# wing02/MyLdpcCppApi

Measured on AMD Instinct MI355X. Metric: decoded Mbit/s (info bits), DVB-S2 N=64800 rate-1/2, 50 iters, higher is better.
Workload: dtype f32; 1 GPU; DVB-S2-profile (64800,32400) rate-1/2 (seeded IRA table with the standard's structure, E=226799), batch 4096 frames per GPU, 50 iterations, sum-product fp32 (probability domain), all-zero codeword + AWGN sigma=0.95 (no frame converges), early termination on, inputs resident in HBM; global_batch=4096, frames_per_gpu=4096, algo=sp, frames_per_launch=4096, parallelism=frames sharded over 1 GPU(s), all-gather of decoded bytes, frames_converged=0

## Files before the change

### include/ldpc_hip.h

```cpp
#ifndef LDPC_HIP_H_
#define LDPC_HIP_H_

#include <stddef.h>
#include <stdint.h>

#ifdef __cplusplus
extern "C" {
#endif

#define LDPC_HIP_ABI_VERSION 3

enum ldpc_status {
    LDPC_OK = 0,
    LDPC_ERR_ARG = 1,
    LDPC_ERR_HIP = 2,
    LDPC_ERR_NOMEM = 3,
    LDPC_ERR_UNSUPPORTED = 4,
    LDPC_ERR_STATE = 5
};

enum ldpc_algo {
    LDPC_ALGO_SP = 0,
    LDPC_ALGO_MS = 1,
    LDPC_ALGO_LAYERED = 2,
    LDPC_ALGO_MS_FUSED = 3,
    LDPC_ALGO_LAYERED_HOST = 4
};

enum ldpc_msg_dtype { LDPC_MSG_F32 = 0, LDPC_MSG_F16 = 1 };

enum ldpc_host_input { LDPC_HOST_INPUT_AUTO = 0, LDPC_HOST_INPUT_STAGED = 1, LDPC_HOST_INPUT_LOCK_PAGES = 2 };

enum ldpc_pack_mode {
    LDPC_PACK_BYTES = 0,
    LDPC_PACK_BITS = 1
};

typedef struct ldpc_graph ldpc_graph;
typedef struct ldpc_decoder ldpc_decoder;

typedef struct ldpc_decoder_config {
    uint32_t struct_size;
    int32_t K;
    int32_t max_batch;
    int32_t algo;
    int32_t msg_dtype;
    int32_t max_iter;
    float llr_scale;
    int32_t early_term;
    int32_t device;
    int32_t layer_rows;
    int32_t pack_mode;
    int32_t frames_per_lane;
    int32_t poll_interval;
    int32_t tune_flags;
    int32_t tune_rows_per_wave;
    int32_t tune_cols_per_wave;
    int32_t tune_link_rows;
    int32_t tune_compact;
    int32_t tune_ldsp_grid;
    int32_t tune_ldsp_shape;
    int32_t tune_place;
    int32_t host_input;
    int32_t host_copy_threads;
    int32_t tune_q_order;
    float ms_scale;
    float ms_offset;
} ldpc_decoder_config;

enum ldpc_tune_field {
    LDPC_TUNE_FUSED = 0,
    LDPC_TUNE_LDSP = 2,
    LDPC_TUNE_LDSP_EXT = 4,
    LDPC_TUNE_LDSP_PACK = 6,
    LDPC_TUNE_LINK_NARROW = 8,
    LDPC_TUNE_CHECK_WIDE = 10,
    LDPC_TUNE_SYN_XCD = 12,
    LDPC_TUNE_FUSED_PACK = 14,
    LDPC_TUNE_FUSED_LOOP = 16,
    LDPC_TUNE_DEVICE_TAIL = 18,
    LDPC_TUNE_MERGE = 20,
    LDPC_TUNE_LINK_DEEP = 22,
    LDPC_TUNE_LINK_HALF = 24,
    LDPC_TUNE_LINK_GUIDED = 26,
    LDPC_TUNE_TILES_FIRST = 28
};
#define LDPC_TUNE_ON(field) (1 << (field))
#define LDPC_TUNE_OFF(field) (2 << (field))

typedef struct ldpc_decode_stats {
    int32_t iterations_launched;
    int32_t batch_time;
    int64_t frames;
    int64_t frames_converged;
    float ms_total;
    float ms_check;
    float ms_var;
    float ms_other;
    int32_t launches_check;
    int32_t launches_var;
    int64_t frame_rounds;
} ldpc_decode_stats;

int ldpc_abi_version(void);
const char *ldpc_last_error(void);
int ldpc_device_count(int *count);

int ldpc_graph_create(const int32_t *rows, const int32_t *cols, int64_t E, int32_t M, int32_t N,
                      ldpc_graph **out);
int ldpc_graph_destroy(ldpc_graph *g);
int ldpc_graph_info(const ldpc_graph *g, int32_t *M, int32_t *N, int64_t *E, int32_t *max_row_deg,
                    int32_t *max_col_deg);

void ldpc_decoder_config_init(ldpc_decoder_config *cfg);
int ldpc_decoder_create(const ldpc_graph *g, const ldpc_decoder_config *cfg, ldpc_decoder **out);
int ldpc_decoder_create_multi(const ldpc_graph *g, const ldpc_decoder_config *cfg, const int32_t *devices,
                              int32_t n_devices, ldpc_decoder **out);
int ldpc_decoder_destroy(ldpc_decoder *d);
int ldpc_shard_range(int64_t frames, int32_t part, int32_t parts, int32_t unit, int64_t *lo, int64_t *hi);

int ldpc_decode(ldpc_decoder *d, const float *llr_host, int64_t frames, uint8_t *out_host,
                int64_t out_bytes, int32_t *iters);

int ldpc_decode_device(ldpc_decoder *d, const float *llr_dev, int64_t frames, uint8_t *out_dev,
                       int64_t out_bytes, int32_t *iters_dev, void *stream);

int64_t ldpc_out_bytes(int32_t K, int64_t frames, int32_t pack_mode);

int ldpc_decoder_set_timing(ldpc_decoder *d, int enable);
int ldpc_decoder_stats(ldpc_decoder *d, ldpc_decode_stats *stats);

typedef struct ldpc_kernel_time {
    int32_t phase;
    int32_t degree;
    int32_t launches;
    float ms_total;
    int64_t bytes_total;
    char name[64];
    int64_t bytes_moved;
} ldpc_kernel_time;
int ldpc_decoder_kernel_times(ldpc_decoder *d, ldpc_kernel_time *out, int32_t capacity,
                              int32_t *count);

int ldpc_decoder_link_form(ldpc_decoder *d, int32_t *form, int32_t *calibrated, float ms[3]);

int ldpc_decoder_placement(ldpc_decoder *d, int32_t *candidates, int32_t *kept, float ms[16]);
int ldpc_decoder_array_addresses(ldpc_decoder *d, uint64_t out[4]);

int ldpc_decoder_set_tap(ldpc_decoder *d, int32_t iter);
int ldpc_decoder_dump(ldpc_decoder *d, int32_t which, float *host_out, int64_t count);

int ldpc_awgn_device(float *llr_dev, int64_t frames, int32_t N, const uint8_t *bits_dev, float sd,
                     uint64_t seed, int64_t first_frame, int32_t device, void *stream);
int ldpc_count_errors_device(const uint8_t *out_dev, const uint8_t *ref_dev, int64_t frames,
                             int64_t bytes_per_frame, int64_t errors[3], int32_t device, void *stream);

typedef struct ldpc_encoder ldpc_encoder;
enum ldpc_code_format {
    LDPC_CODE_PACKED = 0,
    LDPC_CODE_BITS = 1
};
enum ldpc_parity_kind { LDPC_PARITY_DUAL_DIAGONAL = 1, LDPC_PARITY_STAIRCASE = 2 };
int ldpc_parity_structure(const ldpc_graph *g, int32_t K, int32_t block_rows, int32_t out[8]);
int ldpc_encoder_create(const ldpc_graph *g, int32_t K, int32_t block_rows, int32_t max_frames, int32_t device,
                        ldpc_encoder **out);
int ldpc_encoder_destroy(ldpc_encoder *e);
int ldpc_encode_device(ldpc_encoder *e, const uint8_t *src_dev, int64_t src_bytes, int64_t frames, uint8_t *code_dev,
                       int64_t code_bytes, int32_t format, void *stream);
int ldpc_encode(ldpc_encoder *e, const uint8_t *src_host, int64_t src_bytes, uint8_t *code_host, int64_t code_bytes);
int64_t ldpc_code_bytes(int32_t N, int64_t frames, int32_t format);

typedef struct ldpc_rate_spec {
    uint32_t struct_size;
    int32_t  N;
    int32_t  punctured;
    int32_t  filler_lo, filler_hi;
    float    fill_llr;
    float    erasure_llr;
} ldpc_rate_spec;
void ldpc_rate_spec_init(ldpc_rate_spec *spec, int32_t N);
int ldpc_rate_lengths(const ldpc_rate_spec *spec, int32_t *Ncb, int32_t *L);
int ldpc_rate_index(const ldpc_rate_spec *spec, int32_t k0, int32_t E, int32_t *index_out);
int ldpc_rate_match_device(const ldpc_rate_spec *spec, const uint8_t *code_dev, int32_t code_format, int64_t frames, int32_t k0,
                           int32_t E, uint8_t *tx_dev, int64_t tx_bytes, int32_t tx_format, int32_t device, void *stream);
int ldpc_rate_recover_device(const ldpc_rate_spec *spec, const float *rx_dev, int64_t frames, int32_t k0, int32_t E, float *soft_dev,
                             int32_t accumulate, float *y_dev, int32_t device, void *stream);
int ldpc_rate_match(const ldpc_rate_spec *spec, const uint8_t *code_host, int32_t code_format, int64_t frames, int32_t k0, int32_t E,
                    uint8_t *tx_host, int64_t tx_bytes, int32_t tx_format, int32_t device);
int ldpc_rate_recover(const ldpc_rate_spec *spec, const float *rx_host, int64_t frames, int32_t k0, int32_t E, float *soft_host,
                      int32_t accumulate, float *y_host, int32_t device);

typedef struct ldpc_modem_spec {
    uint32_t struct_size;
    int32_t  Qm;
    int32_t  interleave;
} ldpc_modem_spec;
void ldpc_modem_spec_init(ldpc_modem_spec *spec, int32_t Qm);
int64_t ldpc_modem_symbol_floats(const ldpc_modem_spec *spec, int32_t E);
int ldpc_modem_index(const ldpc_modem_spec *spec, int32_t E, int32_t *index_out);
int ldpc_modem_points(int32_t Qm, float *iq);
int ldpc_modem_transmit_device(const ldpc_modem_spec *spec, const uint8_t *tx_dev, int32_t tx_format, int64_t frames, int32_t E,
                               float sd, uint64_t seed, int64_t first_frame, float *sym_dev, int64_t sym_floats, int32_t device,
                               void *stream);
int ldpc_modem_demap_device(const ldpc_modem_spec *spec, const float *sym_dev, int64_t frames, int32_t E, float *rx_dev,
                            int32_t device, void *stream);
int ldpc_modem_transmit(const ldpc_modem_spec *spec, const uint8_t *tx_host, int32_t tx_format, int64_t frames, int32_t E, float sd,
                        uint64_t seed, int64_t first_frame, float *sym_host, int64_t sym_floats, int32_t device);
int ldpc_modem_demap(const ldpc_modem_spec *spec, const float *sym_host, int64_t frames, int32_t E, float *rx_host, int32_t device);

int ldpc_hbm_probe_device(int32_t device, int64_t bytes, int32_t reps, double *copy_gbs, double *by_policy);
int ldpc_hbm_sustained_device(int32_t device, int64_t bytes, int32_t milliseconds, double *copy_gbs);

int ldpc_host_block_plan(uint64_t base, int64_t frames, int32_t N, int32_t max_batch, int64_t group, uint64_t out[6]);
int ldpc_host_locked_ranges(int64_t *live, int64_t *stale);

#ifdef __cplusplus
}
#endif
#endif
```

### myldpccppapi_amd/capi.py

```python
import ctypes

import numpy as np

from . import _lib
from ._lib import DecoderConfig, DecodeStats, LdpcError

ALGO_SP, ALGO_MS, ALGO_LAYERED, ALGO_MS_FUSED, ALGO_LAYERED_HOST = 0, 1, 2, 3, 4
MSG_F32, MSG_F16 = 0, 1
PACK_BYTES, PACK_BITS = 0, 1
CODE_PACKED, CODE_BITS = 0, 1
CODE_FORMATS = {"packed": CODE_PACKED, "bits": CODE_BITS}
PARITY_KINDS = {1: "dual_diagonal", 2: "staircase"}
HOST_INPUT = {"auto": 0, "staged": 1, "lock_pages": 2}
ALGOS = {"sp": ALGO_SP, "ms": ALGO_MS, "layered": ALGO_LAYERED, "ms_fused": ALGO_MS_FUSED,
         "layered_host": ALGO_LAYERED_HOST}

TUNE_FIELDS = {"fused": 0, "ldsp": 2, "ldsp_ext": 4, "ldsp_pack": 6, "link_narrow": 8, "check_wide": 10,
               "syn_xcd": 12, "fused_pack": 14, "fused_loop": 16, "device_tail": 18, "merge": 20, "link_deep": 22, "link_half": 24,
               "link_guided": 26, "tiles_first": 28}
TUNE_INTS = ("rows_per_wave", "cols_per_wave", "link_rows", "compact", "ldsp_grid", "ldsp_per_cu", "ldsp_waves", "place", "q_order")


def apply_tune(cfg, tune):
    flags, shape = 0, 0
    for k, v in (tune or {}).items():
        if k in TUNE_FIELDS:
            if v is not None:
                flags |= (1 if v else 2) << TUNE_FIELDS[k]
        elif k == "ldsp_per_cu":
            shape |= int(v) & 255
        elif k == "ldsp_waves":
            shape |= (int(v) & 255) << 8
        elif k in TUNE_INTS:
            setattr(cfg, "tune_" + k, int(v))
        else:
            raise KeyError("unknown tuning field %r" % k)
    cfg.tune_flags, cfg.tune_ldsp_shape = flags, shape


def hbm_probe(device=0, nbytes=1 << 30, reps=5, by_policy=False):
    g = ctypes.c_double(0.0)
    two = (ctypes.c_double * 2)(0.0, 0.0)
    _lib.check(_lib.load().ldpc_hbm_probe_device(int(device), int(nbytes), int(reps), ctypes.byref(g), two))
    return (g.value, two[0], two[1]) if by_policy else g.value


def hbm_sustained(device=0, nbytes=1 << 30, milliseconds=300):
    g = ctypes.c_double(0.0)
    _lib.check(_lib.load().ldpc_hbm_sustained_device(int(device), int(nbytes), int(milliseconds), ctypes.byref(g)))
    return g.value


def tune_from_env(env=None):
    import os
    env = os.environ if env is None else env
    t = {}
    for name, key in (("FUSED", "fused"), ("LDSP", "ldsp"), ("LDSP_EXT", "ldsp_ext"), ("LDSP_PACK", "ldsp_pack"),
                      ("LINK_NARROW", "link_narrow"), ("CHECK_WIDE", "check_wide"), ("SYN_XCD", "syn_xcd"),
                      ("FUSED_LOOP", "fused_loop"), ("DEVICE_TAIL", "device_tail"), ("MERGE", "merge"), ("LINK_DEEP", "link_deep"), ("LINK_HALF", "link_half"),
                      ("LINK_GUIDED", "link_guided"), ("TILES_FIRST", "tiles_first")):
        if "LDPC_TUNE_" + name in env:
            t[key] = int(env["LDPC_TUNE_" + name]) != 0
    if "LDPC_TUNE_NO_PACK" in env:
        t["fused_pack"] = False
    for name, key in (("RPW", "rows_per_wave"), ("CPW", "cols_per_wave"), ("LDSP_GRID", "ldsp_grid"),
                      ("LDSP_PER_CU", "ldsp_per_cu"), ("LDSP_WAVES", "ldsp_waves")):
        if "LDPC_TUNE_" + name in env:
            t[key] = int(env["LDPC_TUNE_" + name])
    for name, key in (("LINK_RPW", "link_rows"), ("COMPACT", "compact")):
        if "LDPC_TUNE_" + name in env:
            v = int(env["LDPC_TUNE_" + name])
            t[key] = v if v > 0 else -1
    return t


def shard_range(frames, part, parts, unit=1):
    lo, hi = ctypes.c_int64(), ctypes.c_int64()
    _lib.check(_lib.load().ldpc_shard_range(int(frames), int(part), int(parts), int(unit),
                                            ctypes.byref(lo), ctypes.byref(hi)))
    return lo.value, hi.value


def host_block_plan(base, frames, N, max_batch, group):
    out = (ctypes.c_uint64 * 6)()
    _lib.check(_lib.load().ldpc_host_block_plan(int(base), int(frames), int(N), int(max_batch), int(group), out))
    return tuple(int(x) for x in out)


def host_locked_ranges():
    a, b = ctypes.c_int64(-1), ctypes.c_int64(-1)
    _lib.check(_lib.load().ldpc_host_locked_ranges(ctypes.byref(a), ctypes.byref(b)))
    return a.value, b.value


def device_count():
    n = ctypes.c_int(0)
    rc = _lib.load().ldpc_device_count(ctypes.byref(n))
    return n.value if rc == 0 else 0


def out_bytes(K, frames, pack_mode=PACK_BYTES):
    return int(_lib.load().ldpc_out_bytes(K, frames, pack_mode))


def code_bytes(N, frames, fmt="packed"):
    return int(_lib.load().ldpc_code_bytes(int(N), int(frames), CODE_FORMATS.get(fmt, fmt)))


def parity_structure(graph, K, block_rows=0):
    out = (ctypes.c_int32 * 8)()
    _lib.check(_lib.load().ldpc_parity_structure(graph._h, int(K), int(block_rows), out))
    return dict(kind=PARITY_KINDS[out[0]], c=out[1], x=out[2], a=out[3], b=out[4], ext_rows=out[5], z=out[6])


class Graph:

    def __init__(self, rows, cols, M, N):
        L = _lib.load()
        self.rows = np.ascontiguousarray(rows, np.int32)
        self.cols = np.ascontiguousarray(cols, np.int32)
        if self.rows.shape != self.cols.shape or self.rows.ndim != 1:
            raise ValueError("rows and cols must be 1-D arrays of equal length")
        self.M, self.N, self.E = int(M), int(N), int(self.rows.size)
        self._h = ctypes.c_void_p()
        i32p = ctypes.POINTER(ctypes.c_int32)
        _lib.check(L.ldpc_graph_create(self.rows.ctypes.data_as(i32p), self.cols.ctypes.data_as(i32p),
                                       self.E, self.M, self.N, ctypes.byref(self._h)))

    def info(self):
        L = _lib.load()
        M, N, rd, cd = (ctypes.c_int32() for _ in range(4))
        E = ctypes.c_int64()
        _lib.check(L.ldpc_graph_info(self._h, ctypes.byref(M), ctypes.byref(N), ctypes.byref(E),
                                     ctypes.byref(rd), ctypes.byref(cd)))
        return dict(M=M.value, N=N.value, E=E.value, max_row_deg=rd.value, max_col_deg=cd.value)

    def close(self):
        h, self._h = getattr(self, "_h", None), None
        if h and _lib is not None and _lib._lib is not None:
            _lib._lib.ldpc_graph_destroy(h)

    def __del__(self):
        try:
            self.close()
        except Exception:
            pass


class Decoder:

    def __init__(self, graph, K, max_batch, algo="sp", max_iter=40, llr_scale=8.0, early_term=True,
                 device=0, layer_rows=0, pack_mode=PACK_BYTES, frames_per_lane=0, poll_interval=0,
                 msg_dtype=MSG_F32, tune=None, devices=None, host_input="auto", host_copy_threads=0,
                 ms_scale=0.0, ms_offset=0.0):
        L = _lib.load()
        cfg = DecoderConfig()
        L.ldpc_decoder_config_init(ctypes.byref(cfg))
        cfg.K, cfg.max_batch = int(K), int(max_batch)
        cfg.algo = ALGOS[algo] if isinstance(algo, str) else int(algo)
        cfg.msg_dtype = {"f32": MSG_F32, "f16": MSG_F16}.get(msg_dtype, msg_dtype)
        cfg.max_iter, cfg.llr_scale = int(max_iter), float(llr_scale)
        cfg.early_term, cfg.device, cfg.layer_rows = int(bool(early_term)), int(device), int(layer_rows)
        cfg.pack_mode, cfg.frames_per_lane, cfg.poll_interval = int(pack_mode), int(frames_per_lane), int(poll_interval)
        apply_tune(cfg, tune)
        cfg.host_input = HOST_INPUT[host_input] if isinstance(host_input, str) else int(host_input)
        cfg.host_copy_threads = int(host_copy_threads)
        cfg.ms_scale, cfg.ms_offset = float(ms_scale), float(ms_offset)
        self.cfg = cfg
        self.graph = graph
        self.K, self.N, self.E = int(K), graph.N, graph.E
        self._h = ctypes.c_void_p()
        if devices is None:
            _lib.check(L.ldpc_decoder_create(graph._h, ctypes.byref(cfg), ctypes.byref(self._h)))
        else:
            devs = (ctypes.c_int32 * len(devices))(*[int(x) for x in devices])
            _lib.check(L.ldpc_decoder_create_multi(graph._h, ctypes.byref(cfg), devs, len(devices),
                                                   ctypes.byref(self._h)))

    def decode(self, llr, want_iters=True):
        L = _lib.load()
        llr = np.ascontiguousarray(llr, np.float32).reshape(-1, self.N)
        frames = llr.shape[0]
        out = np.zeros(out_bytes(self.K, frames, self.cfg.pack_mode), np.uint8)
        iters = np.zeros(frames, np.int32)
        _lib.check(L.ldpc_decode(self._h, llr.ctypes.data, frames, out.ctypes.data, out.size,
                                 iters.ctypes.data if want_iters else None))
        return out, iters

    def decode_device(self, llr_ptr, frames, out_ptr, out_nbytes, iters_ptr=None, stream=None):
        _lib.check(_lib.load().ldpc_decode_device(self._h, llr_ptr, frames, out_ptr, out_nbytes,
                                                  iters_ptr, stream))

    def set_timing(self, enable=True):
        _lib.check(_lib.load().ldpc_decoder_set_timing(self._h, int(enable)))

    def stats(self):
        st = DecodeStats()
        _lib.check(_lib.load().ldpc_decoder_stats(self._h, ctypes.byref(st)))
        return {f: getattr(st, f) for f, _ in st._fields_}

    def kernel_times(self):
        arr = (_lib.KernelTime * 64)()
        n = ctypes.c_int32(0)
        _lib.check(_lib.load().ldpc_decoder_kernel_times(self._h, arr, 64, ctypes.byref(n)))
        return [dict(name=arr[i].name.decode(), phase=arr[i].phase, degree=arr[i].degree,
                     launches=arr[i].launches, ms_total=arr[i].ms_total, bytes_total=arr[i].bytes_total,
                     bytes_moved=arr[i].bytes_moved)
                for i in range(n.value)]

    def link_form(self):
        form, cal = ctypes.c_int32(-1), ctypes.c_int32(0)
        ms = (ctypes.c_float * 3)()
        _lib.check(_lib.load().ldpc_decoder_link_form(self._h, ctypes.byref(form), ctypes.byref(cal), ms))
# ... 182 lines not shown
```

### myldpccppapi_amd/csrc/decoder.hpp

```cpp
#pragma once

#include <hip/hip_runtime.h>
#include <stdint.h>

#include <memory>
#include <type_traits>
#include <vector>

#include "../../include/ldpc_hip.h"
#include "flood_tables.hpp"
#include "layered_kernels.hpp"
#include "fused_kernels.hpp"
#include "ldsp_kernels.hpp"
#include "engines.hpp"
#include "tune.hpp"
#include "host_stage.hpp"
#include "hip_host.hpp"

#ifndef LDPC_IDLE_FAT
#define LDPC_IDLE_FAT 8
#endif

namespace ldpc {

template <typename Fn> inline int dispatch_v(int V, Fn &&fn)
{
    return V == 1 ? fn(std::integral_constant<int, 1>{})
                  : V == 2 ? fn(std::integral_constant<int, 2>{}) : fn(std::integral_constant<int, 4>{});
}

struct RowClass {
    int degree = 0;
    int count = 0;
    DevBuf<int32_t> e0;
    std::vector<int32_t> h_e0;
    DevBuf<int32_t> link_col, link_pos;
    int linked = 0;
    int n_big = 0, small_rows = 1;
};
struct ColClass {
    int degree = 0;
    int count = 0;
    DevBuf<int32_t> col, edge;
    int64_t q_base = -1;
};

struct ClassGroup {
    int bucket = 0, lo = 0, hi = 0;
    int blocks = 0;
    int blocks_fat = 0;
    std::vector<int> members;
    DevBuf<GroupClass> table, table_fat;
};

constexpr int kIdleFat = LDPC_IDLE_FAT;

struct FloodPlan {
    DevBuf<uint8_t> chan, Q, R;
    int msg_size = 4;
    DevBuf<int32_t> qpos, col_qedge;
    std::vector<int32_t> h_qpos;
    std::vector<RowClass> row_classes;
    std::vector<ColClass> col_classes;
    std::vector<ClassGroup> check_groups, var_groups;
    std::vector<int> check_solo, var_solo;
    DevBuf<int32_t> extra_e0, extra_deg;
    int n_extra = 0;
    int64_t extra_edges = 0;
    FloodFns fns;

    int link_form = 1;
    bool link_deep = false;
    bool syn_xcd = true;
    bool check_wide = false;
    int link_rpw = 16;
    int cus = 256;
    bool link_calibrated = false;
    float link_cal_ms[3] = {0, 0, 0};
    int place_candidates = 0, place_kept = 0;
    float place_ms[16] = {};

    bool tail_enabled = false;
    int TO = 0, TA = 0;
    DevBuf<int32_t> tail_state, tail_map, running;

    std::unique_ptr<ldpc_decoder> child;
    DevBuf<int32_t> cmap;
    DevBuf<int32_t> cinv;
    DevBuf<unsigned long long> cmoved;
    int child_capacity = kCompactCapacity;
    int compact_threshold = kCompactCapacity;
    bool is_child = false;
    ldpc_decoder *handed_to = nullptr;
    HostBuf<int32_t> h_active;

    HostBuf<int32_t> h_summary;
    Event ev_summary;
    bool summary_pending = false;
    int idle_after = 0;

    bool first_round_from_chan = false;
};

struct HostSlot {
    DevBuf<float> llr;
    DevBuf<uint8_t> out;
    DevBuf<int32_t> iters;
    HostBuf<uint8_t> h_out;
    HostBuf<int32_t> h_iters;
    HostBuf<uint8_t> h_head;
    Event h2d_done, all_done;
    bool busy = false;
    int64_t off = 0, n = 0, dst = 0, copy_bytes = 0;
    HostBuf<int32_t> h_sum;
    int g_iterations = 0, g_tiles = 0, g_children = 0, g_child_f[3] = {0, 0, 0};
};
struct RingChunk { HostBuf<uint8_t> h; Event ev; bool used = false; };
struct CallCounts { bool valid = false; int32_t iterations = 0, batch_time = 0; int64_t frames = 0, converged = 0, frame_rounds = 0; };

struct HostPath {
    Stream copy_stream;
    HostSlot slot[3];
    CallCounts call;
    bool suppress_poll = false;
    std::vector<RingChunk> ring;
    size_t ring_next = 0;
    std::unique_ptr<Worker> stager;
    std::vector<std::unique_ptr<Worker>> copy_helpers;
    std::vector<Job> copy_jobs;
    Job stage_job[3];
    bool stage_pending[3] = {false, false, false};
    std::vector<void *> locked_blocks, stuck_blocks;
};

struct TimedSpan {
    Event a, b;
    int kind = 0;
    int degree = 0;
    int64_t bytes = 0;
    int64_t moved = 0;
    int lo = 0;
};

struct Timing {
    bool timing = false;
    int timing_every = 0;
    int64_t timing_calls = 0;
    std::vector<TimedSpan> spans;
    size_t spans_used = 0;
    Event ev_begin, ev_end;
    hipStream_t last_stream = nullptr;
    bool have_last = false;
    int32_t tap_iter = 0;
};

}

struct ldpc_decoder {
    ldpc::Stream stream;
    ldpc_decoder_config cfg{};
    int32_t M = 0, N = 0;
    int64_t E = 0;
    int V = 1, F = 64, T = 0;
    std::vector<int32_t> h_cols;
    ldpc::Tune tune;

    ldpc::DevBuf<int32_t> row_ptr, edge_col, col_ptr, col_edge;
    ldpc::DevBuf<uint64_t> hard, failw, done;
    ldpc::DevBuf<int32_t> iters, active;
    ldpc::DevBuf<int32_t> summary;

    ldpc::LayeredPlan layered;
    ldpc::FusedPlan fused;
    bool use_fused = false;
    ldpc::LdspPlan ldsp;
    bool use_ldsp = false;
    bool ms_corr = false;
    float ms_scale = 1.0f, ms_offset = 0.0f;

    int32_t last_iterations = 0;
    int64_t last_frames = 0;
    int32_t last_tiles = 0;

    ldpc::FloodPlan flood;
    ldpc::HostPath host;
    ldpc::Timing tm;

    std::vector<ldpc_decoder *> shards;
    std::vector<std::unique_ptr<ldpc::Worker>> shard_workers;

    void wait_for_own_work()
    {
        if (!stream.s) return;
        if (flood.child) flood.child->wait_for_own_work();
        (void)hipSetDevice(cfg.device);
        if (tm.have_last && tm.ev_end.e) (void)hipEventSynchronize(tm.ev_end.e);
        (void)hipStreamSynchronize(stream.s);
        if (host.copy_stream.s) (void)hipStreamSynchronize(host.copy_stream.s);
    }

    ~ldpc_decoder()
    {
        for (auto &w : shard_workers) w->stop();
        if (host.stager) host.stager->stop();
        for (auto &w : host.copy_helpers) w->stop();
        for (ldpc_decoder *sh : shards) (void)ldpc_decoder_destroy(sh);
        wait_for_own_work();
    }
};

namespace ldpc {

inline hipError_t span_begin(ldpc_decoder *d, hipStream_t s, int kind, int degree = 0, int64_t bytes = 0, int64_t moved = -1,
                             int lo = 0)
{
    Timing &t = d->tm;
    if (!t.timing) return hipSuccess;
    if (t.spans_used == t.spans.size()) {
        TimedSpan sp;
        hipError_t e = sp.a.create();
        if (e == hipSuccess) e = sp.b.create();
        if (e != hipSuccess) return e;
        t.spans.push_back(std::move(sp));
    }
    TimedSpan &sp = t.spans[t.spans_used];
    sp.kind = kind;
    sp.degree = degree;
    sp.bytes = bytes;
    sp.moved = moved < 0 ? bytes : moved;
    sp.lo = lo;
    return hipEventRecord(sp.a.e, s);
}

inline hipError_t span_end(ldpc_decoder *d, hipStream_t s)
{
    if (!d->tm.timing) return hipSuccess;
    return hipEventRecord(d->tm.spans[d->tm.spans_used++].b.e, s);
}

}
```

### myldpccppapi_amd/csrc/engine_flood.hip

```cpp
#include <hip/hip_runtime.h>

#include <algorithm>
#include <map>
#include <vector>

#include "flood_kernels.hpp"
#include "decoder.hpp"
#include "graph.hpp"

using ldpc::set_error;

namespace {

using ldpc::DevBuf;
using ldpc::RowClass;
using ldpc::ColClass;
using ldpc::ClassGroup;
using ldpc::kIdleFat;
using ldpc::dispatch_v;
using ldpc::span_begin;
using ldpc::span_end;
using ldpc::kVarBuckets;
using ldpc::kCheckBuckets;
using ldpc::kVarBucketLo;
using ldpc::kVarBucketHi;
using ldpc::kCheckBucketLo;
using ldpc::kCheckBucketHi;

template <int V>
__global__ void summary_kernel(const int32_t *iters, const uint64_t *done, const uint64_t *fail,
                               int64_t frames, int32_t freeze, int32_t *summary)
{
    constexpr int F = 64 * V;
    const int64_t f = (int64_t)blockIdx.x * blockDim.x + threadIdx.x;
    if (f >= frames) return;
    const int64_t tile = f / F;
    const int fi = (int)(f % F);
    const int l = fi / V, v = fi % V;
    atomicMax(&summary[0], iters[f]);
    const uint64_t ok = freeze ? done[tile * V + v] : ~fail[tile * V + v];
    if ((ok >> l) & 1ull) atomicAdd(&summary[1], 1);
}

static inline dim3 flood_grid(const ldpc_decoder *d, unsigned blocks, unsigned tiles, int32_t *tiles_first, bool linked = false)
{
    const bool want = d->tune.tiles_first == 1 || (d->tune.tiles_first == 0 && linked);
    *tiles_first = (blocks <= 65535u && want) ? 1 : 0;
    return *tiles_first ? dim3(tiles, blocks) : dim3(blocks, tiles);
}

template <int V> int run_flooding(ldpc_decoder *d, const float *llr_dev, int64_t frames,
                                  uint8_t *out_dev, int64_t out_bytes, int32_t *iters_dev,
                                  hipStream_t s, int start_round = 1);

template <int V> int enqueue_check_phase(ldpc_decoder *d, hipStream_t s, int tiles, int64_t frames, int it, int max_iter,
                                         bool fat, const ldpc::TailRef &tr)
{
    using namespace ldpc;
    const int64_t msz = d->flood.msg_size;
    for (auto &rc : d->flood.row_classes) {
        if (!rc.linked) continue;
        LDPC_HIP_TRY(span_begin(d, s, 4, rc.degree,
                           (2 * msz * rc.degree * rc.count + msz * 5 * rc.linked + 2 * msz * d->flood.extra_edges) * frames,
                           msz * ((int64_t)rc.degree * rc.count + rc.linked +
                                  ((int64_t)rc.degree * rc.count - 2 * rc.linked) +
                                  (it < max_iter ? 2 * rc.linked : 0) + 2 * d->flood.extra_edges) * frames));
        CheckArgs a{d->flood.Q.p, d->flood.R.p, rc.e0.p, d->done.p, d->E, rc.count, 1, rc.degree, d->ms_scale, tr};
        a.ms_offset = d->ms_offset;
        a.qpos = d->flood.qpos.p;
        LinkArgs lk{rc.link_col.p, rc.link_pos.p, d->flood.chan.p, d->flood.Q.p, d->hard.p, d->N,
                    (it < max_iter) ? 1 : 0, d->tm.tap_iter ? 1 : 0, d->flood.extra_e0.p, d->flood.extra_deg.p, d->flood.n_extra, 0,
                    rc.n_big, rc.small_rows};
        a.rows_per_wave = d->flood.link_rpw;
        const int variant = (d->flood.link_form == 2 && !d->flood.fns.link_half[rc.degree]) ? 1 : d->flood.link_form;
        const int waves = link_chunk_count(d->flood.link_rpw, rc.n_big, rc.small_rows, rc.count) * (variant == 1 ? V : variant == 2 ? V / 2 : 1);
        lk.link_blocks = (waves + kWavesPerBlock - 1) / kWavesPerBlock;
        const dim3 grid = flood_grid(d, lk.link_blocks + (d->flood.n_extra + kWavesPerBlock - 1) / kWavesPerBlock, tiles, &a.tiles_first, true);
        (variant == 2 ? d->flood.fns.link_half : variant == 1 ? (d->flood.link_deep ? d->flood.fns.link_deep : d->flood.fns.link_narrow) : d->flood.fns.link)
            [rc.degree]<<<grid, kBlock, 0, s>>>(a, lk);
        LDPC_HIP_TRY(span_end(d, s));
    }
    for (auto &g : d->flood.check_groups) {
        int64_t edges = 0;
        for (int i : g.members) edges += (int64_t)d->flood.row_classes[i].degree * d->flood.row_classes[i].count;
        LDPC_HIP_TRY(span_begin(d, s, 5, g.hi, 2 * msz * edges * frames, -1, g.lo));
        CheckArgs a{d->flood.Q.p, d->flood.R.p, nullptr, d->done.p, d->E, 0, (d->tune.rows_per_wave ? d->tune.rows_per_wave : 2) * (fat ? kIdleFat : 1), 0, d->ms_scale, tr};
        a.ms_offset = d->ms_offset;
        a.qpos = d->flood.qpos.p;
        if (it == 1 && d->flood.first_round_from_chan) { a.first_chan = d->flood.chan.p; a.edge_col = d->edge_col.p; a.N = d->N; }
        const dim3 grid = flood_grid(d, fat ? g.blocks_fat : g.blocks, tiles, &a.tiles_first);
        d->flood.fns.check_group[g.bucket]<<<grid, kBlock, 0, s>>>(a, fat ? g.table_fat.p : g.table.p, (int)g.members.size());
        LDPC_HIP_TRY(span_end(d, s));
    }
    for (int ci : d->flood.check_solo) {
        RowClass &rc = d->flood.row_classes[ci];
        LDPC_HIP_TRY(span_begin(d, s, 0, rc.degree, 2 * msz * rc.degree * rc.count * frames));
        CheckArgs a{d->flood.Q.p, d->flood.R.p, rc.e0.p, d->done.p, d->E, rc.count, 1, rc.degree, d->ms_scale, tr};
        a.ms_offset = d->ms_offset;
        a.qpos = d->flood.qpos.p;
        if (it == 1 && d->flood.first_round_from_chan) { a.first_chan = d->flood.chan.p; a.edge_col = d->edge_col.p; a.N = d->N; }
        const int slotk = rc.degree <= d->flood.fns.max_check_unrolled ? rc.degree : 0;
        const bool narrow = slotk && (!d->flood.check_wide || rc.degree > kMaxUnrolledDegree);
        const int rpw = (d->tune.rows_per_wave ? d->tune.rows_per_wave : (narrow ? 2 : 1)) * (fat ? kIdleFat : 1);
        a.rows_per_wave = rpw;
        const int waves = ((rc.count + rpw - 1) / rpw) * (narrow ? V : 1);
        const dim3 grid = flood_grid(d, (waves + kWavesPerBlock - 1) / kWavesPerBlock, tiles, &a.tiles_first);
        (narrow ? d->flood.fns.check : d->flood.fns.check_wide)[slotk]<<<grid, kBlock, 0, s>>>(a);
        LDPC_HIP_TRY(span_end(d, s));
    }
    return LDPC_OK;
}

template <int V> int enqueue_var_phase(ldpc_decoder *d, hipStream_t s, int tiles, int64_t frames, int it, int max_iter,
                                       bool fat, const ldpc::TailRef &tr)
{
    using namespace ldpc;
    const int64_t msz = d->flood.msg_size;
    const int wq = (it < max_iter) ? 1 : 0;
    for (auto &g : d->flood.var_groups) {
        int64_t units = 0;
        for (int i : g.members) units += (int64_t)((wq ? 2 : 1) * d->flood.col_classes[i].degree + 1) * d->flood.col_classes[i].count;
        LDPC_HIP_TRY(span_begin(d, s, 6, g.hi, msz * units * frames, -1, g.lo));
        VarArgs a{d->flood.R.p, d->flood.Q.p, d->flood.chan.p, d->hard.p, d->done.p, nullptr, nullptr,
                  d->E, d->N, 0, (d->tune.cols_per_wave ? d->tune.cols_per_wave : 1) * (fat ? kIdleFat : 1), wq, 0, tr};
        const dim3 grid = flood_grid(d, fat ? g.blocks_fat : g.blocks, tiles, &a.tiles_first);
        d->flood.fns.var_group[g.bucket]<<<grid, kBlock, 0, s>>>(a, fat ? g.table_fat.p : g.table.p, (int)g.members.size());
        LDPC_HIP_TRY(span_end(d, s));
    }
    for (int ci : d->flood.var_solo) {
        ColClass &cc = d->flood.col_classes[ci];
        LDPC_HIP_TRY(span_begin(d, s, 1, cc.degree, msz * ((wq ? 2 : 1) * cc.degree + 1) * cc.count * frames));
        VarArgs a{d->flood.R.p, d->flood.Q.p, d->flood.chan.p, d->hard.p, d->done.p, cc.col.p, cc.edge.p,
                  d->E, d->N, cc.count, 1, wq, cc.degree, tr};
        const int cpw = (d->tune.cols_per_wave ? d->tune.cols_per_wave : 1) * (fat ? kIdleFat : 1);
        a.cols_per_wave = cpw;
        a.q_base = cc.q_base;
        const int slotk = cc.degree <= kMaxUnrolledDegree ? cc.degree : 0;
        const int waves = (cc.count + cpw - 1) / cpw;
        const dim3 grid = flood_grid(d, (waves + kWavesPerBlock - 1) / kWavesPerBlock, tiles, &a.tiles_first);
        d->flood.fns.var[slotk]<<<grid, kBlock, 0, s>>>(a);
        LDPC_HIP_TRY(span_end(d, s));
    }
    return LDPC_OK;
}

template <int V> int compact_and_finish(ldpc_decoder *d, int64_t frames, int count, int it, hipStream_t s)
{
    using namespace ldpc;
    ldpc_decoder *c = d->flood.child.get();
    while (c->flood.child && count <= c->flood.child->cfg.max_batch) c = c->flood.child.get();
    const int cv = c->V, cf = 64 * cv;
    const unsigned ct = (unsigned)((count + cf - 1) / cf);
    const unsigned cg = ct * (unsigned)cv;
    if (cg > (unsigned)kBackWords) return set_error(LDPC_ERR_STATE, "hand-over of %d frames: more than %d mask words per column", count, kBackWords);
    LDPC_HIP_TRY(hipMemsetAsync(d->active.p, 0, sizeof(int32_t), s));
    compact_list_kernel<V><<<(unsigned)((frames + kBlock - 1) / kBlock), kBlock, 0, s>>>(d->done.p, frames, d->flood.cmap.p,
                                                                                         d->active.p, d->flood.child_capacity);
    const dim3 ge((unsigned)((d->E + kWavesPerBlock - 1) / kWavesPerBlock), cg);
    const dim3 gn((unsigned)((d->N + kWavesPerBlock - 1) / kWavesPerBlock), cg);
    const bool rowwise = count >= 128;
    const int ptiles = (int)((frames + 64 * V - 1) / (64 * V));
    if (d->flood.msg_size == 2) {
        if (rowwise) {
            compact_gather_rows_kernel<V, _Float16><<<(unsigned)((d->E + gather_rows_per_block<_Float16>() - 1) / gather_rows_per_block<_Float16>()), kBlock, 0, s>>>((const _Float16 *)d->flood.Q.p, (_Float16 *)c->flood.Q.p, d->flood.cmap.p, count, d->E, ptiles, cf, d->flood.qpos.p, c->flood.qpos.p);
            compact_gather_rows_kernel<V, _Float16><<<(unsigned)((d->N + gather_rows_per_block<_Float16>() - 1) / gather_rows_per_block<_Float16>()), kBlock, 0, s>>>((const _Float16 *)d->flood.chan.p, (_Float16 *)c->flood.chan.p, d->flood.cmap.p, count, d->N, ptiles, cf);
        } else {
            compact_gather_kernel<V, _Float16><<<ge, kBlock, 0, s>>>((const _Float16 *)d->flood.Q.p, (_Float16 *)c->flood.Q.p, d->flood.cmap.p, count, d->E, cf, d->flood.qpos.p, c->flood.qpos.p);
            compact_gather_kernel<V, _Float16><<<gn, kBlock, 0, s>>>((const _Float16 *)d->flood.chan.p, (_Float16 *)c->flood.chan.p, d->flood.cmap.p, count, d->N, cf);
        }
    } else {
        if (rowwise) {
            compact_gather_rows_kernel<V, float><<<(unsigned)((d->E + gather_rows_per_block<float>() - 1) / gather_rows_per_block<float>()), kBlock, 0, s>>>((const float *)d->flood.Q.p, (float *)c->flood.Q.p, d->flood.cmap.p, count, d->E, ptiles, cf, d->flood.qpos.p, c->flood.qpos.p);
            compact_gather_rows_kernel<V, float><<<(unsigned)((d->N + gather_rows_per_block<float>() - 1) / gather_rows_per_block<float>()), kBlock, 0, s>>>((const float *)d->flood.chan.p, (float *)c->flood.chan.p, d->flood.cmap.p, count, d->N, ptiles, cf);
        } else {
            compact_gather_kernel<V, float><<<ge, kBlock, 0, s>>>((const float *)d->flood.Q.p, (float *)c->flood.Q.p, d->flood.cmap.p, count, d->E, cf, d->flood.qpos.p, c->flood.qpos.p);
            compact_gather_kernel<V, float><<<gn, kBlock, 0, s>>>((const float *)d->flood.chan.p, (float *)c->flood.chan.p, d->flood.cmap.p, count, d->N, cf);
        }
    }
    LDPC_HIP_TRY(hipMemsetAsync(c->hard.p, 0, (size_t)ct * d->N * cv * sizeof(uint64_t), s));
    if (d->cfg.algo == LDPC_ALGO_SP) {
        if (ptiles * V <= kGatherParentWords && count <= 2 * kCompactCapacity)
            compact_hard_lds_kernel<V><<<(unsigned)((d->N + 63) / 64), kBlock, 0, s>>>(d->hard.p, c->hard.p, d->flood.cmap.p, count, d->N, cv, ptiles, (int)cg);
        else
            compact_hard_kernel<V><<<gn, kBlock, 0, s>>>(d->hard.p, c->hard.p, d->flood.cmap.p, count, d->N, cv);
    }
    compact_child_state_kernel<0><<<ct, 64, 0, s>>>(c->done.p, c->iters.p, count, d->cfg.max_iter, cv);
    LDPC_HIP_TRY(hipGetLastError());
    c->tm.timing = false;
    c->tm.tap_iter = 0;
    const int rc = dispatch_v(cv, [&](auto v) { return run_flooding<decltype(v)::value>(c, nullptr, count, nullptr, 0, nullptr, s, it + 1); });
    if (rc) return rc;
    d->flood.handed_to = c;
    LDPC_HIP_TRY(hipMemsetAsync(d->flood.cmoved.p, 0, d->flood.cmoved.n * sizeof(unsigned long long), s));
    compact_inverse_kernel<V><<<(unsigned)((count + 255) / 256), 256, 0, s>>>(d->flood.cmap.p, count, d->flood.cinv.p, d->flood.cmoved.p, cv);
    compact_hard_back_kernel<V><<<dim3((unsigned)((d->N + kBlock - 1) / kBlock), (unsigned)ptiles), kBlock, 0, s>>>(
        d->hard.p, c->hard.p, d->flood.cinv.p, d->flood.cmoved.p, d->N, cv, (int)cg);
    compact_finish_kernel<V><<<(unsigned)((count + 63) / 64), 64, 0, s>>>(d->done.p, d->iters.p, c->done.p, c->iters.p, d->flood.cmap.p, count, cv);
    LDPC_HIP_TRY(hipGetLastError());
    return LDPC_OK;
}

template <int V> int run_flooding(ldpc_decoder *d, const float *llr_dev, int64_t frames,
                                  uint8_t *out_dev, int64_t out_bytes, int32_t *iters_dev,
                                  hipStream_t s, int start_round)
{
    using namespace ldpc;
    const int F = 64 * V;
    const int tiles = (int)((frames + F - 1) / F);
    const int64_t msz = d->flood.msg_size;
    const int max_iter = d->cfg.max_iter;
    const int rounds = d->tm.tap_iter ? std::min(d->tm.tap_iter, max_iter) : max_iter;
    const bool freeze = d->cfg.early_term != 0;
    const size_t slot = (size_t)d->flood.TA * V;

    const bool resume = start_round > 1;
    LDPC_HIP_TRY(hipMemsetAsync(d->failw.p, 0, d->failw.n * sizeof(uint64_t), s));
    LDPC_HIP_TRY(hipMemsetAsync(d->summary.p, 0, 4 * sizeof(int32_t), s));
    d->flood.handed_to = nullptr;
    if (!resume && d->flood.summary_pending) {
        if (hipEventQuery(d->flood.ev_summary.e) == hipSuccess) {
            d->flood.summary_pending = false;
            d->flood.idle_after = (d->flood.h_summary.p[0] > 0 && d->flood.h_summary.p[0] < max_iter) ? d->flood.h_summary.p[0] + 1 : 0;
        } else {
            (void)hipGetLastError();
        }
    }
    const int idle_after = (freeze && !resume && !d->tm.tap_iter && d->cfg.poll_interval == 0) ? d->flood.idle_after : 0;
    const bool use_tail = d->flood.tail_enabled && freeze && !resume && !d->tm.tap_iter && tiles >= 4 * d->flood.TO;
    const TailRef tr{use_tail ? d->flood.tail_state.p : nullptr, d->T, d->flood.TO};
    TailArgs ta{};
    if (use_tail) {
        LDPC_HIP_TRY(hipMemsetAsync(d->flood.tail_state.p, 0, 4 * sizeof(int32_t), s));
        LDPC_HIP_TRY(hipMemsetAsync(d->flood.running.p, 0, d->flood.running.n * sizeof(int32_t), s));
        ta = TailArgs{d->flood.tail_state.p, d->flood.tail_map.p, d->flood.running.p, d->done.p, d->iters.p, d->flood.Q.p, d->flood.chan.p, d->hard.p,
                      d->E, frames, d->N, tiles, d->T, d->flood.TO * F, std::min(d->flood.compact_threshold, d->flood.TO * F), 0, max_iter};
    }

    bool q_less = d->cfg.algo == LDPC_ALGO_MS && !resume && !d->tm.tap_iter && max_iter > 1 && d->flood.n_extra == 0;
    for (auto &rc : d->flood.row_classes) if (rc.linked) q_less = false;
    for (int ci : d->flood.check_solo) if (d->flood.row_classes[ci].degree > d->flood.fns.max_check_unrolled) q_less = false;
    d->flood.first_round_from_chan = q_less;
    if (!resume) {
        LDPC_HIP_TRY(span_begin(d, s, 3));
        InitArgs a{llr_dev, d->flood.chan.p, q_less ? nullptr : d->flood.Q.p, d->hard.p, d->col_ptr.p, d->flood.col_qedge.p,
                   d->E, frames, d->N, d->cfg.llr_scale};
        dim3 grid((d->N + kInitCols - 1) / kInitCols, tiles);
        d->flood.fns.init<<<grid, kBlock, 0, s>>>(a);
        StateArgs st{d->done.p, nullptr, d->iters.p, nullptr, frames, 0, max_iter, freeze ? 1 : 0};
        state_kernel<V><<<use_tail ? d->flood.TA : tiles, 64, 0, s>>>(st);
        LDPC_HIP_TRY(span_end(d, s));
    }

    int launched = start_round - 1;
    bool poll_dense = false;
    for (int it = start_round; it <= rounds; ++it) {
        const bool fat = idle_after > 0 && it > idle_after;
        {
            const int rcp = enqueue_check_phase<V>(d, s, tiles, frames, it, max_iter, fat, tr);
            if (rcp) return rcp;
        }
        {
            const int rcv = enqueue_var_phase<V>(d, s, tiles, frames, it, max_iter, fat, tr);
            if (rcv) return rcv;
        }
        launched = it;
        if (freeze || it == rounds) {
            LDPC_HIP_TRY(span_begin(d, s, 3));
            uint64_t *fw = d->failw.p + (size_t)it * slot;
            const int rbk = (d->M + kBlock - 1) / kBlock;
            SyndromeArgs sa{d->row_ptr.p, d->edge_col.p, d->hard.p, fw, d->done.p, d->M, d->N,
                            d->flood.syn_xcd ? tiles : 0, rbk, tr};
            dim3 sgrid = d->flood.syn_xcd ? dim3(8 * rbk * ((tiles + 7) / 8)) : dim3(rbk, tiles);
            syndrome_kernel<V><<<sgrid, kBlock, 0, s>>>(sa);
            StateArgs st{d->done.p, fw, d->iters.p, nullptr, frames, it, max_iter, 1, tr, use_tail ? d->flood.running.p : nullptr,
                         d->summary.p + 2};
            const bool poll = freeze && it < rounds && d->cfg.poll_interval > 0 && !d->host.suppress_poll &&
                              ((it % d->cfg.poll_interval) == 0 || poll_dense);
            if (poll) {
                LDPC_HIP_TRY(hipMemsetAsync(d->active.p, 0, sizeof(int32_t), s));
                st.active = d->active.p;
            }
            state_kernel<V><<<tiles, 64, 0, s>>>(st);
            if (use_tail && it < rounds) {
                ta.iter = it;
                const unsigned tg = (unsigned)std::min<int64_t>(1024, d->E + 2 * (int64_t)d->N);
                if (d->flood.msg_size == 2) tail_gather_kernel<V, _Float16><<<tg, kBlock, 0, s>>>(ta);
                else tail_gather_kernel<V, float><<<tg, kBlock, 0, s>>>(ta);
            }
            LDPC_HIP_TRY(span_end(d, s));
            if (poll) {
                LDPC_HIP_TRY(hipMemcpyAsync(d->flood.h_active.p, d->active.p, sizeof(int32_t),
                                       hipMemcpyDeviceToHost, s));
                LDPC_HIP_TRY(hipStreamSynchronize(s));
                const int running = *d->flood.h_active.p;
                if (running == 0) break;
                if ((int64_t)running * 10 <= frames * 9 && d->flood.child && tiles > 1 &&
                    (double)d->E * (double)frames * 4.0 * (double)msz > 1.5e9) poll_dense = true;
                if (d->flood.child && running <= d->flood.compact_threshold && (int64_t)running * 4 <= frames && tiles > 1 && !d->tm.tap_iter) {
                    const int rc = compact_and_finish<V>(d, frames, running, it, s);
                    if (rc) return rc;
                    launched = d->flood.handed_to->last_iterations;
                    break;
                }
            }
        }
    }
    d->last_iterations = launched;
    d->last_tiles = tiles;
    if (resume) return LDPC_OK;

    LDPC_HIP_TRY(span_begin(d, s, 3));
    if (use_tail) tail_scatter_kernel<V><<<2048, kBlock, 0, s>>>(ta);
    {
        PackArgs pa{d->hard.p, out_dev, d->iters.p, iters_dev, frames, out_bytes, d->N, d->cfg.K,
                    d->cfg.pack_mode};
        const bool pack = (out_dev || iters_dev) && frames;
        if (d->cfg.pack_mode == LDPC_PACK_BYTES) {
            if (pack) pack_kernel<V><<<pack_grid<V>(d->cfg.K, tiles), kBlock, 0, s>>>(pa);
        } else {
            const int64_t n = std::max<int64_t>(out_bytes, frames);
            dim3 grid((unsigned)((n + kBlock - 1) / kBlock));
            if (pack) pack_kernel<V><<<grid, kBlock, 0, s>>>(pa);
        }
        summary_kernel<V><<<(unsigned)((frames + 255) / 256), 256, 0, s>>>(
            d->iters.p, d->done.p, d->failw.p, frames, 1, d->summary.p);
        if (!d->flood.is_child && d->cfg.poll_interval == 0 && freeze && !d->flood.summary_pending) {
            LDPC_HIP_TRY(hipMemcpyAsync(d->flood.h_summary.p, d->summary.p, 2 * sizeof(int32_t), hipMemcpyDeviceToHost, s));
            LDPC_HIP_TRY(hipEventRecord(d->flood.ev_summary.e, s));
            d->flood.summary_pending = true;
        }
    }
    LDPC_HIP_TRY(span_end(d, s));
    LDPC_HIP_TRY(hipGetLastError());
    return LDPC_OK;
}

int build_classes(ldpc_decoder *d, const ldpc_graph *g)
{
    std::map<int, std::vector<int32_t>> rows_by_deg, cols_by_deg, rowids_by_deg;
    for (int32_t m = 0; m < g->M; ++m) {
        const int deg = g->row_ptr[m + 1] - g->row_ptr[m];
        if (deg > 0) { rows_by_deg[deg].push_back(g->row_ptr[m]); rowids_by_deg[deg].push_back(m); }
    }
    std::vector<char> fused_col((size_t)g->N, 0);
    d->flood.row_classes.resize(rows_by_deg.size());
    size_t i = 0;
    for (auto &kv : rows_by_deg) {
        RowClass &rc = d->flood.row_classes[i++];
        rc.degree = kv.first;
        rc.count = (int)kv.second.size();
        rc.h_e0 = kv.second;
        LDPC_HIP_TRY(rc.e0.upload(kv.second));
        const std::vector<int32_t> &ids = rowids_by_deg[kv.first];
        const int rpw = d->flood.link_rpw;
        if (rpw >= 2 && rc.degree >= 2 && rc.degree <= ldpc::kMaxUnrolledDegree) {
            rc.n_big = (rc.count + rpw - 1) / rpw;
            rc.small_rows = rpw;
            const int small = std::max(2, rpw / 4);
            const bool forced = ldpc::tune_forced_on(d->tune.link_guided);
            if ((d->T >= 4 || forced) && small < rpw && !ldpc::tune_forced_off(d->tune.link_guided)) {
                const int64_t last_generation = (int64_t)d->flood.cus * 16 / d->T;
                int64_t big = (int64_t)rc.n_big - last_generation;
                if (big <= 0 && forced) big = rc.n_big - std::max(1, rc.n_big / 3);
                if (big > 0) { rc.n_big = (int)big; rc.small_rows = small; }
            }
            std::vector<char> chunk_end((size_t)rc.count, 0);
            for (int c = 0, nc = ldpc::link_chunk_count(rpw, rc.n_big, rc.small_rows, rc.count); c < nc; ++c) {
                int rb, re;
                ldpc::link_chunk_rows(c, rpw, rc.n_big, rc.small_rows, rc.count, &rb, &re);
                if (re > rb) chunk_end[(size_t)re - 1] = 1;
            }
            std::vector<int32_t> lcol((size_t)rc.count, -1), lpos((size_t)rc.count, 0);
            for (int idx = 0; idx + 1 < rc.count; ++idx) {
                if (chunk_end[idx]) continue;
                const int32_t m = ids[idx], m2 = ids[idx + 1];
                for (int32_t p = g->row_ptr[m]; p < g->row_ptr[m + 1]; ++p) {
                    const int32_t c = g->cols[p];
                    if (g->col_ptr[c + 1] - g->col_ptr[c] != 2 || fused_col[c]) continue;
                    const int32_t ea = g->col_edge[g->col_ptr[c]], eb = g->col_edge[g->col_ptr[c] + 1];
                    if (ea != p || g->rows[eb] != m2) continue;
                    lcol[idx] = c;
                    lpos[idx] = (p - g->row_ptr[m]) | ((eb - g->row_ptr[m2]) << 8);
                    fused_col[c] = 1;
                    ++rc.linked;
                    break;
                }
            }
            if (rc.linked * 4 >= rc.count) {
                LDPC_HIP_TRY(rc.link_col.upload(lcol));
                LDPC_HIP_TRY(rc.link_pos.upload(lpos));
            } else {
                for (int idx = 0; idx < rc.count; ++idx)
                    if (lcol[idx] >= 0) fused_col[lcol[idx]] = 0;
                rc.linked = 0;
            }
        }
    }
    for (int32_t n = 0; n < g->N; ++n) {
        const int deg = g->col_ptr[n + 1] - g->col_ptr[n];
        if (!fused_col[n]) cols_by_deg[deg].push_back(n);
    }
    d->flood.col_classes.resize(cols_by_deg.size());
    i = 0;
    for (auto &kv : cols_by_deg) {
        ColClass &cc = d->flood.col_classes[i++];
        cc.degree = kv.first;
        cc.count = (int)kv.second.size();
        std::vector<int32_t> edges;
        edges.reserve((size_t)cc.count * std::max(cc.degree, 1));
        for (int32_t n : kv.second)
            for (int32_t p = g->col_ptr[n]; p < g->col_ptr[n + 1]; ++p) edges.push_back(g->col_edge[p]);
        if (edges.empty()) edges.push_back(0);
        LDPC_HIP_TRY(cc.col.upload(kv.second));
        LDPC_HIP_TRY(cc.edge.upload(edges));
    }
    {
        d->flood.h_qpos.assign((size_t)g->E, -1);
        int64_t slot = 0;
        if (d->tune.q_order >= 0)
            for (ColClass &cc : d->flood.col_classes) {
                cc.q_base = slot;
                const std::vector<int32_t> &members = cols_by_deg[cc.degree];
                for (size_t ci = 0; ci < members.size(); ++ci)
                    for (int k = 0; k < cc.degree; ++k)
                        d->flood.h_qpos[(size_t)g->col_edge[(size_t)g->col_ptr[members[ci]] + k]] = (int32_t)(slot + (int64_t)k * cc.count + (int64_t)ci);
                slot += (int64_t)cc.degree * cc.count;
            }
        for (int64_t e = 0; e < g->E; ++e)
            if (d->flood.h_qpos[(size_t)e] < 0) d->flood.h_qpos[(size_t)e] = d->tune.q_order >= 0 ? (int32_t)slot++ : (int32_t)e;
        std::vector<int32_t> cq((size_t)g->E);
        for (int64_t p = 0; p < g->E; ++p) cq[(size_t)p] = d->flood.h_qpos[(size_t)g->col_edge[(size_t)p]];
        LDPC_HIP_TRY(d->flood.qpos.upload(d->flood.h_qpos));
        LDPC_HIP_TRY(d->flood.col_qedge.upload(cq));
    }
    return LDPC_OK;
}

int plan_launches(ldpc_decoder *d)
{
    using ldpc::GroupClass;
    const int V = d->V;
    const bool merge = ldpc::tune_pick(d->tune.merge, true) && !d->flood.check_wide;
    d->flood.check_groups.clear(); d->flood.var_groups.clear(); d->flood.check_solo.clear(); d->flood.var_solo.clear();
    d->flood.n_extra = 0; d->flood.extra_edges = 0;
    int linked_classes = 0;
    int64_t unlinked_rows = 0;
    for (auto &rc : d->flood.row_classes) { if (rc.linked) ++linked_classes; else unlinked_rows += rc.count; }
    const bool as_extra = merge && linked_classes == 1 && unlinked_rows > 0 && unlinked_rows <= 64;
    std::vector<int> cb[kCheckBuckets], vb[kVarBuckets];
    std::vector<int32_t> xe0, xdeg;
    for (int i = 0; i < (int)d->flood.row_classes.size(); ++i) {
        RowClass &rc = d->flood.row_classes[i];
        if (rc.linked) continue;
        if (as_extra) {
            for (int32_t e : rc.h_e0) { xe0.push_back(e); xdeg.push_back(rc.degree); d->flood.extra_edges += rc.degree; }
            continue;
        }
        int b = -1;
        for (int k = 0; k < kCheckBuckets; ++k)
            if (rc.degree >= kCheckBucketLo[k] && rc.degree <= kCheckBucketHi[k] && rc.degree <= d->flood.fns.max_check_unrolled &&
                d->flood.fns.check_group[k]) b = k;
        if (merge && b >= 0) cb[b].push_back(i); else d->flood.check_solo.push_back(i);
    }
    if (as_extra) {
        d->flood.n_extra = (int)xe0.size();
        LDPC_HIP_TRY(d->flood.extra_e0.upload(xe0));
        LDPC_HIP_TRY(d->flood.extra_deg.upload(xdeg));
    }
    for (int i = 0; i < (int)d->flood.col_classes.size(); ++i) {
        const ColClass &cc = d->flood.col_classes[i];
        int b = -1;
        for (int k = 0; k < kVarBuckets; ++k)
            if (cc.degree >= kVarBucketLo[k] && cc.degree <= kVarBucketHi[k] && d->flood.fns.var_group[k]) b = k;
        if (merge && b >= 0) vb[b].push_back(i); else d->flood.var_solo.push_back(i);
    }
    const int rpw = d->tune.rows_per_wave ? d->tune.rows_per_wave : 2, cpw = d->tune.cols_per_wave ? d->tune.cols_per_wave : 1;
    auto make = [&](std::vector<ClassGroup> &groups, std::vector<int> &solo, const std::vector<int> &members, int bucket,
                    int lo, int hi, bool rows) -> hipError_t {
        if (members.size() < 2) { for (int i : members) solo.push_back(i); return hipSuccess; }
        groups.emplace_back();
        ClassGroup &g = groups.back();
        g.bucket = bucket; g.lo = lo; g.hi = hi; g.members = members;
        std::vector<GroupClass> tab, tabf;
        constexpr int fatk = kIdleFat;
        for (int i : members) {
            GroupClass gc{};
            if (rows) {
                const RowClass &rc = d->flood.row_classes[i];
                gc.degree = rc.degree; gc.count = rc.count; gc.ids = rc.e0.p; gc.edges = nullptr; gc.q_base = -1;
            } else {
                const ColClass &cc = d->flood.col_classes[i];
                gc.degree = cc.degree; gc.count = cc.count; gc.ids = cc.col.p; gc.edges = cc.edge.p; gc.q_base = cc.q_base;
            }
            auto blocks_of = [&](int per_wave) {
                const int waves = ((gc.count + per_wave - 1) / per_wave) * (rows ? V / d->flood.fns.check_group_width : 1);
                return (waves + ldpc::kWavesPerBlock - 1) / ldpc::kWavesPerBlock;
            };
            gc.block_begin = g.blocks;
            tab.push_back(gc);
            g.blocks += blocks_of(rows ? rpw : cpw);
            gc.block_begin = g.blocks_fat;
            tabf.push_back(gc);
            g.blocks_fat += blocks_of((rows ? rpw : cpw) * fatk);
        }
        const hipError_t e = g.table.upload(tab);
        return e != hipSuccess ? e : g.table_fat.upload(tabf);
    };
    for (int k = 0; k < kCheckBuckets; ++k) LDPC_HIP_TRY(make(d->flood.check_groups, d->flood.check_solo, cb[k], k, kCheckBucketLo[k], kCheckBucketHi[k], true));
    for (int k = 0; k < kVarBuckets; ++k) LDPC_HIP_TRY(make(d->flood.var_groups, d->flood.var_solo, vb[k], k, kVarBucketLo[k], kVarBucketHi[k], false));
    return LDPC_OK;
}

int setup_flooding(ldpc_decoder *d, const ldpc_graph *g, size_t TF)
{
    const ldpc_decoder_config *cfg = &d->cfg;
    d->flood.msg_size = cfg->msg_dtype == LDPC_MSG_F16 ? 2 : 4;
    LDPC_HIP_TRY(d->flood.chan.alloc(TF * d->N * d->flood.msg_size));
    LDPC_HIP_TRY(d->flood.Q.alloc(TF * (size_t)d->E * d->flood.msg_size));
    LDPC_HIP_TRY(d->flood.R.alloc(TF * (size_t)d->E * d->flood.msg_size));
    int rc = build_classes(d, g);
    if (rc) return rc;
    ldpc::FloodFns *fns = &d->flood.fns;
    if (cfg->algo == LDPC_ALGO_SP) ldpc::fill_flood_sp(d->V, fns);
    else if (d->ms_corr && cfg->msg_dtype == LDPC_MSG_F16) ldpc::fill_flood_msc16(d->V, fns);
    else if (d->ms_corr) ldpc::fill_flood_msc(d->V, fns);
    else if (cfg->msg_dtype == LDPC_MSG_F16) ldpc::fill_flood_ms16(d->V, fns);
    else ldpc::fill_flood_ms(d->V, fns);
    return plan_launches(d);
}

template <int V> int calibrate_link(ldpc_decoder *d)
{
    using namespace ldpc;
    RowClass *rcp = nullptr;
    for (auto &rc : d->flood.row_classes) if (rc.linked) rcp = &rc;
    if (!rcp || !d->flood.fns.link[rcp->degree] || !d->flood.fns.link_narrow[rcp->degree]) return LDPC_OK;
    RowClass &rc = *rcp;
    const int tiles = d->T;
    hipStream_t s = d->stream.s;
    LDPC_HIP_TRY(hipMemsetAsync(d->flood.Q.p, 0, d->flood.Q.n, s));
    LDPC_HIP_TRY(hipMemsetAsync(d->flood.chan.p, 0, d->flood.chan.n, s));
    LDPC_HIP_TRY(hipMemsetAsync(d->done.p, 0, d->done.n * sizeof(uint64_t), s));
    ldpc::Event ev[2];
    LDPC_HIP_TRY(ev[0].create());
    LDPC_HIP_TRY(ev[1].create());
    float best[3] = {1e30f, 1e30f, 1e30f};
    const int candidates = d->flood.fns.link_half[rc.degree] ? 3 : 2;
    hipError_t err = hipSuccess;
    for (int rep = 0; rep < 4 && err == hipSuccess; ++rep) {
        for (int nar = 0; nar < candidates && err == hipSuccess; ++nar) {
            CheckArgs a{d->flood.Q.p, d->flood.R.p, rc.e0.p, d->done.p, d->E, rc.count, d->flood.link_rpw, rc.degree, d->ms_scale,
                        TailRef{nullptr, 0, 0}};
            a.ms_offset = d->ms_offset;
            a.qpos = d->flood.qpos.p;
            LinkArgs lk{rc.link_col.p, rc.link_pos.p, d->flood.chan.p, d->flood.Q.p, d->hard.p, d->N, 1, 0, nullptr, nullptr, 0, 0,
                        rc.n_big, rc.small_rows};
            const int waves = link_chunk_count(d->flood.link_rpw, rc.n_big, rc.small_rows, rc.count) * (nar == 1 ? V : nar == 2 ? V / 2 : 1);
            lk.link_blocks = (waves + kWavesPerBlock - 1) / kWavesPerBlock;
            const dim3 grid = flood_grid(d, lk.link_blocks, tiles, &a.tiles_first, true);
            err = hipEventRecord(ev[0].e, s);
            (nar == 2 ? d->flood.fns.link_half : nar == 1 ? d->flood.fns.link_narrow : d->flood.fns.link)[rc.degree]<<<grid, kBlock, 0, s>>>(a, lk);
            if (err == hipSuccess) err = hipEventRecord(ev[1].e, s);
            if (err == hipSuccess) err = hipEventSynchronize(ev[1].e);
            float ms = 0;
            if (err == hipSuccess) err = hipEventElapsedTime(&ms, ev[0].e, ev[1].e);
            if (err == hipSuccess && rep > 0 && ms < best[nar]) best[nar] = ms;
        }
    }
    if (err != hipSuccess) return set_error(LDPC_ERR_HIP, "link calibration: %s", hipGetErrorString(err));
    LDPC_HIP_TRY(hipGetLastError());
    int pick = 0;
    for (int k = 0; k < candidates; ++k) { d->flood.link_cal_ms[k] = best[k]; if (best[k] < best[pick]) pick = k; }
    d->flood.link_form = pick;
    d->flood.link_calibrated = true;
    return LDPC_OK;
}

template <int V> int time_check_phase(ldpc_decoder *d, float *ms_out)
{
    hipStream_t s = d->stream.s;
    LDPC_HIP_TRY(hipMemsetAsync(d->flood.Q.p, 0, d->flood.Q.n, s));
    LDPC_HIP_TRY(hipMemsetAsync(d->flood.chan.p, 0, d->flood.chan.n, s));
    LDPC_HIP_TRY(hipMemsetAsync(d->done.p, 0, d->done.n * sizeof(uint64_t), s));
    ldpc::Event ev[2];
    LDPC_HIP_TRY(ev[0].create());
    LDPC_HIP_TRY(ev[1].create());
    float best = 1e30f;
    hipError_t err = hipSuccess;
    int rc = LDPC_OK;
    for (int rep = 0; rep < 4 && err == hipSuccess && rc == LDPC_OK; ++rep) {
        err = hipEventRecord(ev[0].e, s);
        rc = enqueue_check_phase<V>(d, s, d->T, (int64_t)d->T * d->F, 1, d->cfg.max_iter, false, ldpc::TailRef{nullptr, 0, 0});
        if (rc == LDPC_OK)
            rc = enqueue_var_phase<V>(d, s, d->T, (int64_t)d->T * d->F, 1, d->cfg.max_iter, false, ldpc::TailRef{nullptr, 0, 0});
        if (err == hipSuccess) err = hipEventRecord(ev[1].e, s);
        if (err == hipSuccess) err = hipEventSynchronize(ev[1].e);
        float ms = 0;
        if (err == hipSuccess) err = hipEventElapsedTime(&ms, ev[0].e, ev[1].e);
        if (err == hipSuccess && rep > 0 && ms < best) best = ms;
    }
    if (rc) return rc;
    if (err != hipSuccess) return set_error(LDPC_ERR_HIP, "placement search: %s", hipGetErrorString(err));
    *ms_out = best;
    return LDPC_OK;
}

template <int V> int placement_search(ldpc_decoder *d, size_t TF)
{
    const size_t bq = TF * (size_t)d->E * d->flood.msg_size, bc = TF * d->N * d->flood.msg_size;
    const int want = d->tune.place == 0 ? (2 * bq + bc >= ((size_t)256 << 20) ? 6 : 1) : d->tune.place;
    if (want <= 1) return LDPC_OK;
    float best_ms = 0.0f;
    int rc = time_check_phase<V>(d, &best_ms);
    if (rc) return rc;
    std::vector<DevBuf<uint8_t>> held;
    d->flood.place_ms[0] = best_ms;
    d->flood.place_candidates = 1;
    d->flood.place_kept = 0;
    float lo = best_ms, hi = best_ms;
    for (int stage = 0; stage < 2; ++stage) {
        DevBuf<uint8_t> &arr = stage == 0 ? d->flood.R : d->flood.Q;
        for (int c = 1; c < want; ++c) {
            if (lo < 0.91f * hi && best_ms <= lo && d->flood.place_candidates >= 4) break;
            size_t free_b = 0, total_b = 0;
            if (hipMemGetInfo(&free_b, &total_b) != hipSuccess || free_b < 2 * bq + ((size_t)2 << 30)) break;
            DevBuf<uint8_t> cand, spacer;
            const size_t period = (size_t)16 << 30;
            if (c == 1 && arr.n < period && free_b > period + 2 * bq + ((size_t)2 << 30)) {
                if (spacer.alloc(period - arr.n) != hipSuccess) (void)hipGetLastError();
            }
            if (cand.alloc(arr.n) != hipSuccess) { (void)hipGetLastError(); break; }
            spacer.release();
            std::swap(arr, cand);
            float ms = 0.0f;
            rc = time_check_phase<V>(d, &ms);
            if (rc) return rc;
            if (d->flood.place_candidates < 16) d->flood.place_ms[d->flood.place_candidates] = ms;
            lo = std::min(lo, ms); hi = std::max(hi, ms);
            if (ms < best_ms) {
                best_ms = ms;
                d->flood.place_kept = d->flood.place_candidates;
            } else {
                std::swap(arr, cand);
            }
            ++d->flood.place_candidates;
            held.push_back(std::move(cand));
        }
    }
    return LDPC_OK;
}

}

int ldpc::engine_flood_setup(ldpc_decoder *d, const ldpc_graph *g, size_t TF, bool top_level)
{
    int rc = setup_flooding(d, g, TF);
    if (rc || !top_level) return rc;
    const ldpc::Tune &tune = d->tune;
    if (tune.link_narrow == 0 && tune.link_half == 0 && !tune.link_deep && d->V >= 2) {
        rc = dispatch_v(d->V, [&](auto v) { return calibrate_link<decltype(v)::value>(d); });
        if (rc) return rc;
    }
// ... 9 lines not shown
```

### myldpccppapi_amd/csrc/flood_kernels.hpp

```cpp
#pragma once

#include <hip/hip_runtime.h>
#include <stdint.h>

#include "ldpc_expf.h"

namespace ldpc {

constexpr int kAlgoSP = 0;
constexpr int kAlgoMS = 1;
constexpr int kAlgoMSC = 2;
constexpr int kCompactCapacity = 512;
constexpr int kLastCapacity = 64;
constexpr int kBlock = 256;
constexpr int kWavesPerBlock = 4;
constexpr int kMaxUnrolledDegree = 16;
constexpr int kMaxUnrolledCheckDegreeMS = 32;

#ifndef LDPC_NT_LOAD
#define LDPC_NT_LOAD 1
#endif
#ifndef LDPC_NT_STORE
#define LDPC_NT_STORE 1
#endif
typedef float vf2 __attribute__((ext_vector_type(2)));
typedef float vf4 __attribute__((ext_vector_type(4)));

template <typename T> __device__ __forceinline__ T ld_stream(const T *p)
{
#if LDPC_NT_LOAD
    return __builtin_nontemporal_load(p);
#else
    return *p;
#endif
}
template <typename T> __device__ __forceinline__ void st_stream(T *p, T v)
{
#if LDPC_NT_STORE
    __builtin_nontemporal_store(v, p);
#else
    *p = v;
#endif
}

template <int V> __device__ __forceinline__ void vload(float (&d)[V], const float *p);
template <> __device__ __forceinline__ void vload<1>(float (&d)[1], const float *p) { d[0] = ld_stream(p); }
template <> __device__ __forceinline__ void vload<2>(float (&d)[2], const float *p)
{
    const vf2 t = ld_stream(reinterpret_cast<const vf2 *>(p));
    d[0] = t.x; d[1] = t.y;
}
template <> __device__ __forceinline__ void vload<4>(float (&d)[4], const float *p)
{
    const vf4 t = ld_stream(reinterpret_cast<const vf4 *>(p));
    d[0] = t.x; d[1] = t.y; d[2] = t.z; d[3] = t.w;
}
template <int V> __device__ __forceinline__ void vstore(float *p, const float (&s)[V]);
template <> __device__ __forceinline__ void vstore<1>(float *p, const float (&s)[1]) { st_stream(p, s[0]); }
template <> __device__ __forceinline__ void vstore<2>(float *p, const float (&s)[2])
{
    vf2 t; t.x = s[0]; t.y = s[1];
    st_stream(reinterpret_cast<vf2 *>(p), t);
}
template <> __device__ __forceinline__ void vstore<4>(float *p, const float (&s)[4])
{
    vf4 t; t.x = s[0]; t.y = s[1]; t.z = s[2]; t.w = s[3];
    st_stream(reinterpret_cast<vf4 *>(p), t);
}

typedef _Float16 hf;
typedef _Float16 vh2 __attribute__((ext_vector_type(2)));
typedef _Float16 vh4 __attribute__((ext_vector_type(4)));

template <int V> __device__ __forceinline__ void vload(float (&d)[V], const hf *p);
template <> __device__ __forceinline__ void vload<1>(float (&d)[1], const hf *p) { d[0] = (float)ld_stream(p); }
template <> __device__ __forceinline__ void vload<2>(float (&d)[2], const hf *p)
{
    const vh2 t = ld_stream(reinterpret_cast<const vh2 *>(p));
    d[0] = (float)t.x; d[1] = (float)t.y;
}
template <> __device__ __forceinline__ void vload<4>(float (&d)[4], const hf *p)
{
    const vh4 t = ld_stream(reinterpret_cast<const vh4 *>(p));
    d[0] = (float)t.x; d[1] = (float)t.y; d[2] = (float)t.z; d[3] = (float)t.w;
}
template <int V> __device__ __forceinline__ void vstore(hf *p, const float (&s)[V]);
template <> __device__ __forceinline__ void vstore<1>(hf *p, const float (&s)[1]) { st_stream(p, (hf)s[0]); }
template <> __device__ __forceinline__ void vstore<2>(hf *p, const float (&s)[2])
{
    vh2 t; t.x = (hf)s[0]; t.y = (hf)s[1];
    st_stream(reinterpret_cast<vh2 *>(p), t);
}
template <> __device__ __forceinline__ void vstore<4>(hf *p, const float (&s)[4])
{
    vh4 t; t.x = (hf)s[0]; t.y = (hf)s[1]; t.z = (hf)s[2]; t.w = (hf)s[3];
    st_stream(reinterpret_cast<vh4 *>(p), t);
}

__device__ __forceinline__ int wave_id_in_block()
{
    return __builtin_amdgcn_readfirstlane((int)(threadIdx.x >> 6));
}

template <int V> __device__ __forceinline__ bool tile_finished(const uint64_t *done, int tile)
{
    bool all = true;
#pragma unroll
    for (int v = 0; v < V; ++v) all = all && (done[(size_t)tile * V + v] == ~0ull);
    return all;
}

struct TailRef {
    const int32_t *state;
    int32_t base_tile;
    int32_t n_tiles;
};

template <int V> __device__ __forceinline__ int tile_select(const TailRef &t, const uint64_t *done, int row)
{
    int tile = row;
    if (t.state && __builtin_amdgcn_readfirstlane(t.state[0])) {
        if (row >= t.n_tiles) return -1;
        tile = t.base_tile + row;
    }
    return tile_finished<V>(done, tile) ? -1 : tile;
}


struct CheckArgs {
    const void *__restrict__ Q;
    void *__restrict__ R;
    const int32_t *__restrict__ cls_e0;
    const uint64_t *__restrict__ done;
    int64_t E;
    int32_t n_rows;
    int32_t rows_per_wave;
    int32_t degree;
    float ms_scale = 1.0f;
    TailRef tail;
    int32_t tiles_first = 0;
    float ms_offset = 0.0f;
    const void *__restrict__ first_chan = nullptr;
    const int32_t *__restrict__ edge_col = nullptr;
    int32_t N = 0;
    const int32_t *__restrict__ qpos = nullptr;
};

template <int D> __device__ __forceinline__ void row_slots(const int32_t *__restrict__ qpos, int e0, int lane, int (&slot)[D])
{
    static_assert(D <= 64, "one lane per edge");
    const int mine = qpos[e0 + (lane < D ? lane : D - 1)];
#pragma unroll
    for (int k = 0; k < D; ++k) slot[k] = __builtin_amdgcn_readlane(mine, k);
}
__device__ __forceinline__ int edge_slot(const int32_t *__restrict__ qpos, int e)
{
    return __builtin_amdgcn_readfirstlane(qpos[e]);
}

struct GridPos { int row, block; };
__device__ __forceinline__ GridPos grid_pos(int tiles_first)
{
    return tiles_first ? GridPos{(int)blockIdx.x, (int)blockIdx.y} : GridPos{(int)blockIdx.y, (int)blockIdx.x};
}

template <int D, int V>
__device__ __forceinline__ void check_sp(const float (&x)[D][V], float (&out)[D][V])
{
#pragma unroll
    for (int v = 0; v < V; ++v) {
        if (D == 1) { out[0][v] = 1.0f; continue; }
        {
            float p = x[1][v];
#pragma unroll
            for (int j = 2; j < D; ++j) p *= x[j][v];
            out[0][v] = p;
        }
        float pre = x[0][v];
#pragma unroll
        for (int k = 1; k < D; ++k) {
            float p = pre;
#pragma unroll
            for (int j = k + 1; j < D; ++j) p *= x[j][v];
            out[k][v] = p;
            pre *= x[k][v];
        }
    }
}

struct MsCorr {
    float scale, offset;
};
template <typename T> __device__ __forceinline__ float ms_corr(float m, const MsCorr &c)
{
    const float r = fmaxf(m - c.offset, 0.0f) * c.scale;
    return sizeof(T) == 2 ? (float)(hf)r : r;
}

template <int D, int V, bool CORR = false, typename T = float>
__device__ __forceinline__ void check_ms(const float (&x)[D][V], float (&out)[D][V], MsCorr c = MsCorr{1.0f, 0.0f})
{
#pragma unroll
    for (int v = 0; v < V; ++v) {
        float m1 = 1000.0f, m2 = 1000.0f;
        int idx = -1;
        unsigned par = 0;
#pragma unroll
        for (int j = 0; j < D; ++j) {
            const float a = __builtin_fabsf(x[j][v]);
            par ^= (x[j][v] < 0.0f) ? 1u : 0u;
            if (a < m1) { m2 = m1; m1 = a; idx = j; }
            else if (a < m2) { m2 = a; }
        }
        if (CORR) { m1 = ms_corr<T>(m1, c); m2 = ms_corr<T>(m2, c); }
#pragma unroll
        for (int k = 0; k < D; ++k) {
            const float b = (k == idx) ? m2 : m1;
            const unsigned s = par ^ ((x[k][v] < 0.0f) ? 1u : 0u);
            out[k][v] = s ? -b : b;
        }
    }
}

__device__ __forceinline__ MsCorr ms_corr_of(const CheckArgs &a) { return MsCorr{a.ms_scale, a.ms_offset}; }

template <int ALGO, int D, int V, int W, typename T>
__global__ __launch_bounds__(kBlock) void check_kernel(const CheckArgs a)
{
    constexpr size_t F = 64 * V;
    constexpr int SUB = V / W;
    const int lane = threadIdx.x & 63;
    const GridPos gp = grid_pos(a.tiles_first);
    const int tile = tile_select<V>(a.tail, a.done, gp.row);
    if (tile < 0) return;
    const int wave = gp.block * kWavesPerBlock + wave_id_in_block();
    const int sub = wave % SUB;
    const int r_begin = (wave / SUB) * a.rows_per_wave;
    const int r_end = min(r_begin + a.rows_per_wave, a.n_rows);
    const unsigned lane_off = (unsigned)sub * 64 * W + (unsigned)lane * W;
    const T *Qu = static_cast<const T *>(a.Q) + (size_t)tile * (size_t)a.E * F;
    T *Rt = static_cast<T *>(a.R) + (size_t)tile * (size_t)a.E * F + lane_off;

    const T *Ct = (ALGO != kAlgoSP && a.first_chan)
                      ? static_cast<const T *>(a.first_chan) + (size_t)tile * (size_t)a.N * F + lane_off : nullptr;
    for (int r = r_begin; r < r_end; ++r) {
        const int e0 = a.cls_e0[r];
        float x[D][W], out[D][W];
        if (ALGO != kAlgoSP && Ct) {
#pragma unroll
            for (int k = 0; k < D; ++k) vload<W>(x[k], Ct + (size_t)a.edge_col[e0 + k] * F);
        } else {
            int sl[D];
            row_slots<D>(a.qpos, e0, lane, sl);
#pragma unroll
            for (int k = 0; k < D; ++k) vload<W>(x[k], Qu + (size_t)sl[k] * F + lane_off);
        }
        if (ALGO == kAlgoSP) check_sp<D, W>(x, out); else if (ALGO == kAlgoMS) check_ms<D, W>(x, out); else check_ms<D, W, true, T>(x, out, ms_corr_of(a));
#pragma unroll
        for (int k = 0; k < D; ++k) vstore<W>(Rt + (size_t)(e0 + k) * F, out[k]);
    }
}

template <int ALGO, int V, typename T>
__device__ __forceinline__ void check_row_generic(const T *Qu, unsigned lane_off, T *Rt, int e0, int D,
                                                  const int32_t *__restrict__ qpos, const MsCorr &c)
{
    constexpr size_t F = 64 * V;
    if (ALGO != kAlgoSP) {
        float m1[V], m2[V];
        int idx[V];
        unsigned par[V];
#pragma unroll
        for (int v = 0; v < V; ++v) { m1[v] = 1000.0f; m2[v] = 1000.0f; idx[v] = -1; par[v] = 0; }
        for (int j = 0; j < D; ++j) {
            float xj[V];
            vload<V>(xj, Qu + (size_t)edge_slot(qpos, e0 + j) * F + lane_off);
#pragma unroll
            for (int v = 0; v < V; ++v) {
                const float m = __builtin_fabsf(xj[v]);
                par[v] ^= (xj[v] < 0.0f) ? 1u : 0u;
                if (m < m1[v]) { m2[v] = m1[v]; m1[v] = m; idx[v] = j; }
                else if (m < m2[v]) { m2[v] = m; }
            }
        }
        if (ALGO == kAlgoMSC) {
#pragma unroll
            for (int v = 0; v < V; ++v) { m1[v] = ms_corr<T>(m1[v], c); m2[v] = ms_corr<T>(m2[v], c); }
        }
        for (int k = 0; k < D; ++k) {
            float xk[V], o[V];
            vload<V>(xk, Qu + (size_t)edge_slot(qpos, e0 + k) * F + lane_off);
#pragma unroll
            for (int v = 0; v < V; ++v) {
                const float b = (k == idx[v]) ? m2[v] : m1[v];
                const unsigned sg = par[v] ^ ((xk[v] < 0.0f) ? 1u : 0u);
                o[v] = sg ? -b : b;
            }
            vstore<V>(Rt + (size_t)(e0 + k) * F, o);
        }
        return;
    }
    for (int k = 0; k < D; ++k) {
        float o[V];
        float p[V];
#pragma unroll
        for (int v = 0; v < V; ++v) p[v] = 1.0f;
        for (int j = 0; j < D; ++j) {
            if (j == k) continue;
            float xj[V];
            vload<V>(xj, Qu + (size_t)edge_slot(qpos, e0 + j) * F + lane_off);
#pragma unroll
            for (int v = 0; v < V; ++v) p[v] *= xj[v];
        }
#pragma unroll
        for (int v = 0; v < V; ++v) o[v] = p[v];
        vstore<V>(Rt + (size_t)(e0 + k) * F, o);
    }
}

template <int ALGO, int V, typename T>
__global__ __launch_bounds__(kBlock) void check_kernel_generic(const CheckArgs a)
{
    constexpr size_t F = 64 * V;
    const int lane = threadIdx.x & 63;
    const GridPos gp = grid_pos(a.tiles_first);
    const int tile = tile_select<V>(a.tail, a.done, gp.row);
    if (tile < 0) return;
    const int wave = gp.block * kWavesPerBlock + wave_id_in_block();
    const int r_begin = wave * a.rows_per_wave;
    const int r_end = min(r_begin + a.rows_per_wave, a.n_rows);
    const T *Qu = static_cast<const T *>(a.Q) + (size_t)tile * (size_t)a.E * F;
    T *Rt = static_cast<T *>(a.R) + (size_t)tile * (size_t)a.E * F + (size_t)lane * V;
    for (int r = r_begin; r < r_end; ++r) check_row_generic<ALGO, V, T>(Qu, (unsigned)lane * V, Rt, a.cls_e0[r], a.degree, a.qpos, ms_corr_of(a));
}

struct GroupClass {
    int32_t block_begin;
    int32_t degree;
    int32_t count;
    int32_t pad;
    const int32_t *ids;
    const int32_t *edges;
    int64_t q_base;
};

template <int ALGO, int D, int V, int W, typename T>
__device__ __forceinline__ void check_rows(const T *Qu, unsigned lane_off, T *Rt, const int32_t *__restrict__ e0s, int r_begin, int r_end,
                                           const T *Ct, const int32_t *__restrict__ edge_col,
                                           const int32_t *__restrict__ qpos, const MsCorr &c)
{
    const int lane = threadIdx.x & 63;
    constexpr size_t F = 64 * V;
    for (int r = r_begin; r < r_end; ++r) {
        const int e0 = e0s[r];
        float x[D][W], out[D][W];
        if (ALGO != kAlgoSP && Ct) {
#pragma unroll
            for (int k = 0; k < D; ++k) vload<W>(x[k], Ct + (size_t)edge_col[e0 + k] * F);
        } else {
            int sl[D];
            row_slots<D>(qpos, e0, lane, sl);
#pragma unroll
            for (int k = 0; k < D; ++k) vload<W>(x[k], Qu + (size_t)sl[k] * F + lane_off);
        }
        if (ALGO == kAlgoSP) check_sp<D, W>(x, out); else if (ALGO == kAlgoMS) check_ms<D, W>(x, out); else check_ms<D, W, true, T>(x, out, c);
#pragma unroll
        for (int k = 0; k < D; ++k) vstore<W>(Rt + (size_t)(e0 + k) * F, out[k]);
    }
}

template <int ALGO, int V, typename T, int D, int DLO, int W = 1> struct CheckDispatch {
    static __device__ __forceinline__ void run(int deg, const T *Qu, unsigned lane_off, T *Rt, const int32_t *e0s, int rb, int re,
                                               const T *Ct, const int32_t *edge_col, const int32_t *qpos, const MsCorr &c)
    {
        if (deg == D) check_rows<ALGO, D, V, W, T>(Qu, lane_off, Rt, e0s, rb, re, Ct, edge_col, qpos, c);
        else CheckDispatch<ALGO, V, T, D - 1, DLO, W>::run(deg, Qu, lane_off, Rt, e0s, rb, re, Ct, edge_col, qpos, c);
    }
};
template <int ALGO, int V, typename T, int DLO, int W> struct CheckDispatch<ALGO, V, T, DLO, DLO, W> {
    static __device__ __forceinline__ void run(int, const T *Qu, unsigned lane_off, T *Rt, const int32_t *e0s, int rb, int re,
                                               const T *Ct, const int32_t *edge_col, const int32_t *qpos, const MsCorr &c)
    {
        check_rows<ALGO, DLO, V, W, T>(Qu, lane_off, Rt, e0s, rb, re, Ct, edge_col, qpos, c);
    }
};

template <int ALGO, int V, typename T, int DLO, int DHI, int W = 1>
__global__ __launch_bounds__(kBlock) void check_group_kernel(const CheckArgs a, const GroupClass *__restrict__ cls, int n_classes)
{
    constexpr size_t F = 64 * V;
    constexpr int SUB = V / W;
    const int lane = threadIdx.x & 63;
    const GridPos gp = grid_pos(a.tiles_first);
    const int tile = tile_select<V>(a.tail, a.done, gp.row);
    if (tile < 0) return;
    int c = 0;
    while (c + 1 < n_classes && gp.block >= cls[c + 1].block_begin) ++c;
    const int wave = (gp.block - cls[c].block_begin) * kWavesPerBlock + wave_id_in_block();
    const int sub = wave % SUB;
    const int r_begin = (wave / SUB) * a.rows_per_wave;
    const int r_end = min(r_begin + a.rows_per_wave, cls[c].count);
    const unsigned lane_off = (unsigned)sub * 64 * W + (unsigned)lane * W;
    const T *Qu = static_cast<const T *>(a.Q) + (size_t)tile * (size_t)a.E * F;
    T *Rt = static_cast<T *>(a.R) + (size_t)tile * (size_t)a.E * F + lane_off;
    const T *Ct = (ALGO != kAlgoSP && a.first_chan)
                      ? static_cast<const T *>(a.first_chan) + (size_t)tile * (size_t)a.N * F + lane_off : nullptr;
    CheckDispatch<ALGO, V, T, DHI, DLO, W>::run(cls[c].degree, Qu, lane_off, Rt, cls[c].ids, r_begin, r_end, Ct, a.edge_col, a.qpos, ms_corr_of(a));
}

struct SyndromeArgs {
    const int32_t *__restrict__ row_ptr;
    const int32_t *__restrict__ edge_col;
    const uint64_t *__restrict__ hard;
    uint64_t *__restrict__ fail;
    const uint64_t *__restrict__ done;
    int32_t M, N;
    int32_t tiles;
    int32_t row_blocks;
    TailRef tail;
};

template <int V> __global__ __launch_bounds__(kBlock) void syndrome_kernel(const SyndromeArgs a)
{
    int tile, rb;
    if (a.tiles > 0) {
        const int xcd = blockIdx.x & 7, j = blockIdx.x >> 3;
        tile = xcd + 8 * (j / a.row_blocks);
        rb = j % a.row_blocks;
        if (tile >= a.tiles) return;
    } else {
        tile = blockIdx.y;
        rb = blockIdx.x;
    }
    tile = tile_select<V>(a.tail, a.done, tile);
    if (tile < 0) return;
    const int m = rb * kBlock + threadIdx.x;
    const uint64_t *hard_t = a.hard + (size_t)tile * (size_t)a.N * V;
    uint64_t s[V];
#pragma unroll
    for (int v = 0; v < V; ++v) s[v] = 0;
    if (m < a.M) {
        for (int p = a.row_ptr[m]; p < a.row_ptr[m + 1]; ++p) {
            const int c = a.edge_col[p];
#pragma unroll
            for (int v = 0; v < V; ++v) s[v] ^= hard_t[(size_t)c * V + v];
        }
    }
    __shared__ uint64_t part[kWavesPerBlock][V];
#pragma unroll
    for (int v = 0; v < V; ++v) {
        uint64_t x = s[v];
#pragma unroll
        for (int off = 32; off >= 1; off >>= 1) {
            const uint32_t lo = __shfl_xor((uint32_t)x, off);
            const uint32_t hi = __shfl_xor((uint32_t)(x >> 32), off);
            x |= ((uint64_t)hi << 32) | lo;
        }
        if ((threadIdx.x & 63) == 0) part[threadIdx.x >> 6][v] = x;
    }
    __syncthreads();
    if (threadIdx.x < V) {
        uint64_t x = 0;
#pragma unroll
        for (int w = 0; w < kWavesPerBlock; ++w) x |= part[w][threadIdx.x];
        unsigned long long *dst = reinterpret_cast<unsigned long long *>(&a.fail[(size_t)tile * V + threadIdx.x]);
        const uint64_t seen = __hip_atomic_load(dst, __ATOMIC_RELAXED, __HIP_MEMORY_SCOPE_AGENT);
        if (x & ~seen) atomicOr(dst, (unsigned long long)x);
    }
}


struct VarArgs {
    const void *__restrict__ R;
    void *__restrict__ Q;
    const void *__restrict__ chan;
    uint64_t *hard;
    const uint64_t *__restrict__ done;
    const int32_t *__restrict__ cls_col;
    const int32_t *__restrict__ cls_edge;
    int64_t E;
    int32_t N;
    int32_t n_cols;
    int32_t cols_per_wave;
    int32_t write_q;
    int32_t degree;
    TailRef tail;
    int32_t tiles_first = 0;
    int64_t q_base = -1;
};

template <int D, int V>
__device__ __forceinline__ void var_sp(const float (&t)[V], const float (&d)[D][V],
                                       float (&outq)[D][V], float (&full0)[V], float (&full1)[V])
{
#pragma unroll
    for (int v = 0; v < V; ++v) {
        const float den = 1.0f + t[v];
        float pre0 = t[v] / den;
        float pre1 = 1.0f / den;
        float r0[D], r1[D];
#pragma unroll
        for (int k = 0; k < D; ++k) {
            r0[k] = (1.0f + d[k][v]) * 0.5f;
            r1[k] = (1.0f - d[k][v]) * 0.5f;
        }
#pragma unroll
        for (int k = 0; k < D; ++k) {
            float t0 = pre0, t1 = pre1;
#pragma unroll
            for (int j = k + 1; j < D; ++j) { t0 *= r0[j]; t1 *= r1[j]; }
            const float s = t0 + t1;
            const float q0 = t0 / s;
            const float q1 = t1 / s;
            outq[k][v] = q0 - q1;
            pre0 *= r0[k];
            pre1 *= r1[k];
        }
        full0[v] = pre0;
        full1[v] = pre1;
    }
}

struct LinkArgs {
    const int32_t *__restrict__ link_col;
    const int32_t *__restrict__ link_pos;
    const void *__restrict__ chan;
    void *Qw;
    uint64_t *hard;
    int32_t N;
    int32_t write_q;
    int32_t store_all;
    const int32_t *__restrict__ extra_e0;
    const int32_t *__restrict__ extra_deg;
    int32_t n_extra;
    int32_t link_blocks;
    int32_t n_big, small_rows;
};

__host__ __device__ inline void link_chunk_rows(int c, int rows_per_wave, int n_big, int small_rows, int n_rows,
                                               int *rb, int *re)
{
    int b, e;
    if (c < n_big) { b = c * rows_per_wave; e = b + rows_per_wave; }
    else { b = n_big * rows_per_wave + (c - n_big) * small_rows; e = b + small_rows; }
    *rb = b < n_rows ? b : n_rows;
    *re = e < n_rows ? e : n_rows;
}
__host__ __device__ inline int link_chunk_count(int rows_per_wave, int n_big, int small_rows, int n_rows)
{
    const int rest = n_rows - n_big * rows_per_wave;
    return n_big + (rest > 0 ? (rest + small_rows - 1) / small_rows : 0);
}

template <int ALGO, int V, typename T>
__device__ __forceinline__ void link_extra_rows(const CheckArgs &a, const LinkArgs &g, int tile, int block)
{
    constexpr size_t F = 64 * V;
    const int lane = threadIdx.x & 63;
    const int w = (block - g.link_blocks) * kWavesPerBlock + wave_id_in_block();
    if (w >= g.n_extra) return;
    const T *Qu = static_cast<const T *>(a.Q) + (size_t)tile * (size_t)a.E * F;
    T *Rt = static_cast<T *>(a.R) + (size_t)tile * (size_t)a.E * F + (size_t)lane * V;
    check_row_generic<ALGO, V, T>(Qu, (unsigned)lane * V, Rt, g.extra_e0[w], g.extra_deg[w], a.qpos, ms_corr_of(a));
}

#ifdef LDPC_LINK_WIDE_WAVES
#define LDPC_LINK_WIDE_ATTR __attribute__((amdgpu_waves_per_eu(LDPC_LINK_WIDE_WAVES, LDPC_LINK_WIDE_WAVES)))
#else
#define LDPC_LINK_WIDE_ATTR
#endif
template <int ALGO, int D, int V, typename T>
__global__ __launch_bounds__(kBlock) LDPC_LINK_WIDE_ATTR void check_link_kernel(const CheckArgs a, const LinkArgs g)
{
    constexpr size_t F = 64 * V;
    const int lane = threadIdx.x & 63;
    const GridPos gp = grid_pos(a.tiles_first);
    const int tile = tile_select<V>(a.tail, a.done, gp.row);
    if (tile < 0) return;
    if (gp.block >= g.link_blocks) { link_extra_rows<ALGO, V, T>(a, g, tile, gp.block); return; }
    const int wave = gp.block * kWavesPerBlock + wave_id_in_block();
    int r_begin, r_end;
    link_chunk_rows(wave, a.rows_per_wave, g.n_big, g.small_rows, a.n_rows, &r_begin, &r_end);
    const size_t lane_off = (size_t)lane * V;
    const unsigned lane_q = (unsigned)lane * V;
    const T *Qt = static_cast<const T *>(a.Q) + (size_t)tile * (size_t)a.E * F;
    T *Qwt = static_cast<T *>(g.Qw) + (size_t)tile * (size_t)a.E * F;
    T *Rt = static_cast<T *>(a.R) + (size_t)tile * (size_t)a.E * F + lane_off;
    const T *chan_t = static_cast<const T *>(g.chan) + (size_t)tile * (size_t)g.N * F + lane_off;
    uint64_t *hard_t = g.hard + (size_t)tile * (size_t)g.N * V;
    uint64_t frozen[V];
#pragma unroll
    for (int v = 0; v < V; ++v) frozen[v] = a.done[(size_t)tile * V + v];

    int pend_col = -1, pend_edge = 0, pend_kb = 0;
    float pend_r[V];
#pragma unroll
    for (int v = 0; v < V; ++v) pend_r[v] = 0.0f;

    float x[D][V];
    int qc[D], qn[D];
#pragma unroll
    for (int k = 0; k < D; ++k) qc[k] = qn[k] = 0;
    if (r_begin < r_end) {
        row_slots<D>(a.qpos, a.cls_e0[r_begin], lane, qc);
#pragma unroll
        for (int k = 0; k < D; ++k) vload<V>(x[k], Qt + (size_t)qc[k] * F + lane_q);
    }
    for (int r = r_begin; r < r_end; ++r) {
        const int e0 = a.cls_e0[r];
        const int next_col = (r + 1 < r_end) ? g.link_col[r] : -1;
        const int pos = g.link_pos[r];
        const int ka = next_col >= 0 ? (pos & 255) : -1;
        const int kb = pend_col >= 0 ? pend_kb : -1;
        if (r + 1 < r_end) row_slots<D>(a.qpos, a.cls_e0[r + 1], lane, qn);
        float ch[V];
        uint64_t old_w[V];
        if (pend_col >= 0) {
            vload<V>(ch, chan_t + (size_t)pend_col * F);
#pragma unroll
            for (int v = 0; v < V; ++v) old_w[v] = hard_t[(size_t)pend_col * V + v];
        }
        float out[D][V];
        if (ALGO == kAlgoSP) check_sp<D, V>(x, out); else if (ALGO == kAlgoMS) check_ms<D, V>(x, out); else check_ms<D, V, true, T>(x, out, ms_corr_of(a));
        if (r + 1 < r_end) {
#pragma unroll
            for (int k = 0; k < D; ++k) vload<V>(x[k], Qt + (size_t)qn[k] * F + lane_q);
        }
#pragma unroll
        for (int k = 0; k < D; ++k)
            if ((k != ka && k != kb) || g.store_all) vstore<V>(Rt + (size_t)(e0 + k) * F, out[k]);

        if (pend_col >= 0) {
            float rr[2][V], q[2][V];
#pragma unroll
            for (int v = 0; v < V; ++v) {
                rr[0][v] = pend_r[v];
                float t = out[0][v];
#pragma unroll
                for (int k = 1; k < D; ++k) t = (k == kb) ? out[k][v] : t;
                rr[1][v] = t;
            }
            uint64_t new_w[V];
            if (ALGO == kAlgoSP) {
                float f0[V], f1[V];
                var_sp<2, V>(ch, rr, q, f0, f1);
#pragma unroll
                for (int v = 0; v < V; ++v) {
                    const bool oldb = (old_w[v] >> lane) & 1ull;
                    const bool b = (f0[v] > f1[v]) ? false : ((f0[v] < f1[v]) ? true : oldb);
                    new_w[v] = __ballot(b);
                }
            } else {
#pragma unroll
                for (int v = 0; v < V; ++v) {
                    float p = ch[v];
                    p += rr[0][v];
                    p += rr[1][v];
                    q[0][v] = p - rr[0][v];
                    q[1][v] = p - rr[1][v];
                    new_w[v] = __ballot(!(p > 0.0f));
                }
            }
            if (lane == 0) {
#pragma unroll
                for (int v = 0; v < V; ++v)
                    hard_t[(size_t)pend_col * V + v] = (old_w[v] & frozen[v]) | (new_w[v] & ~frozen[v]);
            }
            if (g.write_q) {
                int qw1 = qc[0];
#pragma unroll
                for (int k = 1; k < D; ++k) qw1 = (k == kb) ? qc[k] : qw1;
                vstore<V>(Qwt + (size_t)pend_edge * F + lane_q, q[0]);
                vstore<V>(Qwt + (size_t)qw1 * F + lane_q, q[1]);
            }
        }
        pend_col = next_col;
        if (next_col >= 0) {
            pend_edge = qc[0];
#pragma unroll
            for (int k = 1; k < D; ++k) pend_edge = (k == ka) ? qc[k] : pend_edge;
            pend_kb = (pos >> 8) & 255;
#pragma unroll
            for (int v = 0; v < V; ++v) {
                float t = out[0][v];
#pragma unroll
                for (int k = 1; k < D; ++k) t = (k == ka) ? out[k][v] : t;
                pend_r[v] = t;
            }
        }
#pragma unroll
        for (int k = 0; k < D; ++k) qc[k] = qn[k];
    }
}

template <int V> __device__ __forceinline__ uint64_t compress_stride(uint64_t x)
{
    if (V == 1) return x;
    if (V == 2) {
        x &= 0x5555555555555555ull;
        x = (x | (x >> 1)) & 0x3333333333333333ull;
        x = (x | (x >> 2)) & 0x0f0f0f0f0f0f0f0full;
        x = (x | (x >> 4)) & 0x00ff00ff00ff00ffull;
        x = (x | (x >> 8)) & 0x0000ffff0000ffffull;
        x = (x | (x >> 16)) & 0x00000000ffffffffull;
        return x;
    }
    x &= 0x1111111111111111ull;
    x = (x | (x >> 3)) & 0x0303030303030303ull;
    x = (x | (x >> 6)) & 0x000f000f000f000full;
    x = (x | (x >> 12)) & 0x000000ff000000ffull;
    x = (x | (x >> 24)) & 0x000000000000ffffull;
    return x;
}

template <int ALGO, int D, int V, typename T, int W = 1>
__global__ __launch_bounds__(kBlock) void check_link_narrow_kernel(const CheckArgs a, const LinkArgs g)
{
    constexpr size_t F = 64 * V;
    constexpr int SUBS = V / W;
    constexpr int FB = 64 / SUBS;
    const int lane = threadIdx.x & 63;
    const GridPos gp = grid_pos(a.tiles_first);
    const int tile = tile_select<V>(a.tail, a.done, gp.row);
    if (tile < 0) return;
    if (gp.block >= g.link_blocks) { link_extra_rows<ALGO, V, T>(a, g, tile, gp.block); return; }
    const int wave = gp.block * kWavesPerBlock + wave_id_in_block();
    const int sub = wave % SUBS;
    int r_begin, r_end;
    link_chunk_rows(wave / SUBS, a.rows_per_wave, g.n_big, g.small_rows, a.n_rows, &r_begin, &r_end);
    const size_t lane_off = (size_t)sub * 64 * W + (size_t)lane * W;
    const unsigned lane_q = (unsigned)lane_off;
    const T *Qt = static_cast<const T *>(a.Q) + (size_t)tile * (size_t)a.E * F;
    T *Qwt = static_cast<T *>(g.Qw) + (size_t)tile * (size_t)a.E * F;
    T *Rt = static_cast<T *>(a.R) + (size_t)tile * (size_t)a.E * F + lane_off;
    const T *chan_t = static_cast<const T *>(g.chan) + (size_t)tile * (size_t)g.N * F + lane_off;
    uint8_t *hard_b = reinterpret_cast<uint8_t *>(g.hard + (size_t)tile * (size_t)g.N * V) + (size_t)sub * (FB / 8);
    const uint64_t frozen_field = (a.done[(size_t)tile * V + (lane < V ? lane : 0)] >> (sub * FB)) &
                                  (FB == 64 ? ~0ull : ((1ull << (FB & 63)) - 1ull));

    auto load_field = [&](int col, int word) -> uint64_t {
        const uint8_t *p = hard_b + ((size_t)col * V + word) * 8;
        if (FB == 64) return *reinterpret_cast<const uint64_t *>(p);
        if (FB == 32) return *reinterpret_cast<const uint32_t *>(p);
        return *reinterpret_cast<const uint16_t *>(p);
    };

    int pend_col = -1, pend_edge = 0, pend_kb = 0;
    float pend_r[W];
#pragma unroll
    for (int w = 0; w < W; ++w) pend_r[w] = 0.0f;
    float x[D][W];
    int qc[D], qn[D];
#pragma unroll
    for (int k = 0; k < D; ++k) qc[k] = qn[k] = 0;
    if (r_begin < r_end) {
        row_slots<D>(a.qpos, a.cls_e0[r_begin], lane, qc);
#pragma unroll
        for (int k = 0; k < D; ++k) vload<W>(x[k], Qt + (size_t)qc[k] * F + lane_q);
    }
    for (int r = r_begin; r < r_end; ++r) {
        const int e0 = a.cls_e0[r];
        const int next_col = (r + 1 < r_end) ? g.link_col[r] : -1;
        const int pos = g.link_pos[r];
        const int ka = next_col >= 0 ? (pos & 255) : -1;
        const int kb = pend_col >= 0 ? pend_kb : -1;
        if (r + 1 < r_end) row_slots<D>(a.qpos, a.cls_e0[r + 1], lane, qn);
        float ch[W];
        uint64_t old_mine[W];
#pragma unroll
        for (int w = 0; w < W; ++w) { ch[w] = 0.0f; old_mine[w] = 0; }
        if (pend_col >= 0) {
            vload<W>(ch, chan_t + (size_t)pend_col * F);
#pragma unroll
            for (int w = 0; w < W; ++w) old_mine[w] = load_field(pend_col, (W * lane + w) % V);
        }
        float out[D][W];
        if (ALGO == kAlgoSP) check_sp<D, W>(x, out); else if (ALGO == kAlgoMS) check_ms<D, W>(x, out); else check_ms<D, W, true, T>(x, out, ms_corr_of(a));
        if (r + 1 < r_end) {
#pragma unroll
            for (int k = 0; k < D; ++k) vload<W>(x[k], Qt + (size_t)qn[k] * F + lane_q);
        }
#pragma unroll
        for (int k = 0; k < D; ++k)
            if ((k != ka && k != kb) || g.store_all) vstore<W>(Rt + (size_t)(e0 + k) * F, out[k]);

        if (pend_col >= 0) {
            float rr[2][W], q[2][W];
#pragma unroll
            for (int w = 0; w < W; ++w) {
                rr[0][w] = pend_r[w];
                float t = out[0][w];
#pragma unroll
                for (int k = 1; k < D; ++k) t = (k == kb) ? out[k][w] : t;
                rr[1][w] = t;
            }
            uint64_t ballot[W];
            if (ALGO == kAlgoSP) {
                float f0[W], f1[W];
                var_sp<2, W>(ch, rr, q, f0, f1);
#pragma unroll
                for (int w = 0; w < W; ++w) {
                    const bool oldb = (old_mine[w] >> ((W * lane + w) / V)) & 1ull;
                    const bool bit = (f0[w] > f1[w]) ? false : ((f0[w] < f1[w]) ? true : oldb);
                    ballot[w] = __ballot(bit);
                }
            } else {
#pragma unroll
                for (int w = 0; w < W; ++w) {
                    float p = ch[w];
                    p += rr[0][w];
                    p += rr[1][w];
                    q[0][w] = p - rr[0][w];
                    q[1][w] = p - rr[1][w];
                    ballot[w] = __ballot(!(p > 0.0f));
                }
            }
            if (lane < V) {
                uint64_t bw = ballot[0];
#pragma unroll
                for (int w = 1; w < W; ++w) bw = (lane % W == w) ? ballot[w] : bw;
                const uint64_t nf = compress_stride<SUBS>(bw >> (lane / W));
                const uint64_t of = load_field(pend_col, lane);
                const uint64_t res = (of & frozen_field) | (nf & ~frozen_field);
                uint8_t *p = hard_b + ((size_t)pend_col * V + lane) * 8;
                if (FB == 64) *reinterpret_cast<uint64_t *>(p) = res;
                else if (FB == 32) *reinterpret_cast<uint32_t *>(p) = (uint32_t)res;
                else *reinterpret_cast<uint16_t *>(p) = (uint16_t)res;
            }
            if (g.write_q) {
                int qw1 = qc[0];
#pragma unroll
                for (int k = 1; k < D; ++k) qw1 = (k == kb) ? qc[k] : qw1;
                vstore<W>(Qwt + (size_t)pend_edge * F + lane_q, q[0]);
                vstore<W>(Qwt + (size_t)qw1 * F + lane_q, q[1]);
            }
        }
        pend_col = next_col;
        if (next_col >= 0) {
            pend_edge = qc[0];
#pragma unroll
            for (int k = 1; k < D; ++k) pend_edge = (k == ka) ? qc[k] : pend_edge;
            pend_kb = (pos >> 8) & 255;
#pragma unroll
            for (int w = 0; w < W; ++w) {
                float t = out[0][w];
#pragma unroll
                for (int k = 1; k < D; ++k) t = (k == ka) ? out[k][w] : t;
                pend_r[w] = t;
            }
        }
#pragma unroll
        for (int k = 0; k < D; ++k) qc[k] = qn[k];
    }
}

template <int ALGO, int D, int V, typename T>
__global__ __launch_bounds__(kBlock) void check_link_narrow2_kernel(const CheckArgs a, const LinkArgs g)
{
    constexpr size_t F = 64 * V;
    constexpr int FB = 64 / V;
    const int lane = threadIdx.x & 63;
    const GridPos gp = grid_pos(a.tiles_first);
    const int tile = tile_select<V>(a.tail, a.done, gp.row);
    if (tile < 0) return;
    if (gp.block >= g.link_blocks) { link_extra_rows<ALGO, V, T>(a, g, tile, gp.block); return; }
    const int wave = gp.block * kWavesPerBlock + wave_id_in_block();
    const int sub = wave % V;
    int r_begin, r_end;
    link_chunk_rows(wave / V, a.rows_per_wave, g.n_big, g.small_rows, a.n_rows, &r_begin, &r_end);
    const size_t lane_off = (size_t)sub * 64 + lane;
    const T *Qt = static_cast<const T *>(a.Q) + (size_t)tile * (size_t)a.E * F + lane_off;
    T *Qwt = static_cast<T *>(g.Qw) + (size_t)tile * (size_t)a.E * F + lane_off;
    T *Rt = static_cast<T *>(a.R) + (size_t)tile * (size_t)a.E * F + lane_off;
    const T *chan_t = static_cast<const T *>(g.chan) + (size_t)tile * (size_t)g.N * F + lane_off;
    const int my_word = lane % V, my_bit = lane / V;
    uint8_t *hard_b = reinterpret_cast<uint8_t *>(g.hard + (size_t)tile * (size_t)g.N * V) + (size_t)sub * (FB / 8);
    const uint64_t frozen_field = (a.done[(size_t)tile * V + (lane < V ? lane : 0)] >> (sub * FB)) &
                                  (FB == 64 ? ~0ull : ((1ull << FB) - 1ull));

    auto load_field = [&](int col, int word) -> uint64_t {
        const uint8_t *p = hard_b + ((size_t)col * V + word) * 8;
        if (V == 1) return *reinterpret_cast<const uint64_t *>(p);
        if (V == 2) return *reinterpret_cast<const uint32_t *>(p);
        return *reinterpret_cast<const uint16_t *>(p);
    };

    int pend_col = -1, pend_edge = 0, pend_kb = 0;
    float pend_r = 0.0f;
    float b0[D], b1[D], b2[D];
    auto load_row = [&](float (&dst)[D], int r) {
        const int e = a.cls_e0[r];
#pragma unroll
        for (int k = 0; k < D; ++k) { float t[1]; vload<1>(t, Qt + (size_t)edge_slot(a.qpos, e + k) * F); dst[k] = t[0]; }
    };
    if (r_begin < r_end) load_row(b0, r_begin);
    if (r_begin + 1 < r_end) load_row(b1, r_begin + 1);
    auto step = [&](int r, float (&x)[D], float (&pre)[D]) {
        const int e0 = a.cls_e0[r];
        const int next_col = (r + 1 < r_end) ? g.link_col[r] : -1;
        const int pos = g.link_pos[r];
        const int ka = next_col >= 0 ? (pos & 255) : -1;
        const int kb = pend_col >= 0 ? pend_kb : -1;
        float ch[1] = {0.0f};
        uint64_t old_mine = 0;
        if (pend_col >= 0) {
            vload<1>(ch, chan_t + (size_t)pend_col * F);
            old_mine = load_field(pend_col, my_word);
        }
        if (r + 2 < r_end) load_row(pre, r + 2);
        float xx[D][1], out[D][1];
#pragma unroll
        for (int k = 0; k < D; ++k) xx[k][0] = x[k];
        if (ALGO == kAlgoSP) check_sp<D, 1>(xx, out); else if (ALGO == kAlgoMS) check_ms<D, 1>(xx, out); else check_ms<D, 1, true, T>(xx, out, ms_corr_of(a));
#pragma unroll
        for (int k = 0; k < D; ++k)
            if ((k != ka && k != kb) || g.store_all) vstore<1>(Rt + (size_t)(e0 + k) * F, out[k]);

        if (pend_col >= 0) {
            float rr[2][1], q[2][1];
            rr[0][0] = pend_r;
            float t = out[0][0];
#pragma unroll
            for (int k = 1; k < D; ++k) t = (k == kb) ? out[k][0] : t;
            rr[1][0] = t;
            bool bit;
            if (ALGO == kAlgoSP) {
                float f0[1], f1[1];
                var_sp<2, 1>(ch, rr, q, f0, f1);
                const bool oldb = (old_mine >> my_bit) & 1ull;
                bit = (f0[0] > f1[0]) ? false : ((f0[0] < f1[0]) ? true : oldb);
            } else {
                float p = ch[0];
                p += rr[0][0];
                p += rr[1][0];
                q[0][0] = p - rr[0][0];
                q[1][0] = p - rr[1][0];
                bit = !(p > 0.0f);
            }
            const uint64_t ballot = __ballot(bit);
            if (lane < V) {
                const uint64_t nf = compress_stride<V>(ballot >> lane);
                const uint64_t of = load_field(pend_col, lane);
                const uint64_t res = (of & frozen_field) | (nf & ~frozen_field);
                uint8_t *p = hard_b + ((size_t)pend_col * V + lane) * 8;
                if (V == 1) *reinterpret_cast<uint64_t *>(p) = res;
                else if (V == 2) *reinterpret_cast<uint32_t *>(p) = (uint32_t)res;
                else *reinterpret_cast<uint16_t *>(p) = (uint16_t)res;
            }
            if (g.write_q) {
                vstore<1>(Qwt + (size_t)edge_slot(a.qpos, pend_edge) * F, q[0]);
                vstore<1>(Qwt + (size_t)edge_slot(a.qpos, e0 + kb) * F, q[1]);
            }
        }
        pend_col = next_col;
        if (next_col >= 0) {
            pend_edge = e0 + ka;
            pend_kb = (pos >> 8) & 255;
            float t = out[0][0];
#pragma unroll
            for (int k = 1; k < D; ++k) t = (k == ka) ? out[k][0] : t;
            pend_r = t;
        }
    };
    for (int r = r_begin; r < r_end; r += 3) {
        step(r, b0, b2);
        if (r + 1 < r_end) step(r + 1, b1, b0);
        if (r + 2 < r_end) step(r + 2, b2, b1);
    }
}

template <int ALGO, int D, int V, typename T>
__device__ __forceinline__ void var_columns(const T *Rt, T *Qt, const T *chan_t, uint64_t *hard_t, const uint64_t (&frozen)[V],
                                            const int32_t *__restrict__ cls_col, const int32_t *__restrict__ cls_edge,
                                            int c_begin, int c_end, int write_q, int lane, int64_t q_base, int n_cls)
{
    constexpr size_t F = 64 * V;
    for (int ci = c_begin; ci < c_end; ++ci) {
        const int n = cls_col[ci];
        int e[D];
#pragma unroll
        for (int k = 0; k < D; ++k) e[k] = cls_edge[(size_t)ci * D + k];
        float ch[V], r[D][V], q[D][V];
        vload<V>(ch, chan_t + (size_t)n * F);
#pragma unroll
        for (int k = 0; k < D; ++k) vload<V>(r[k], Rt + (size_t)e[k] * F);
        uint64_t old_w[V], new_w[V];
#pragma unroll
        for (int v = 0; v < V; ++v) old_w[v] = hard_t[(size_t)n * V + v];

        if (ALGO == kAlgoSP) {
            float f0[V], f1[V];
            var_sp<D, V>(ch, r, q, f0, f1);
#pragma unroll
            for (int v = 0; v < V; ++v) {
                const bool oldb = (old_w[v] >> lane) & 1ull;
                const bool b = (f0[v] > f1[v]) ? false : ((f0[v] < f1[v]) ? true : oldb);
                new_w[v] = __ballot(b);
            }
        } else {
#pragma unroll
            for (int v = 0; v < V; ++v) {
                float p = ch[v];
#pragma unroll
                for (int k = 0; k < D; ++k) p += r[k][v];
#pragma unroll
                for (int k = 0; k < D; ++k) q[k][v] = p - r[k][v];
                new_w[v] = __ballot(!(p > 0.0f));
            }
        }
        if (lane == 0) {
#pragma unroll
            for (int v = 0; v < V; ++v)
                hard_t[(size_t)n * V + v] = (old_w[v] & frozen[v]) | (new_w[v] & ~frozen[v]);
        }
        if (write_q) {
            if (q_base >= 0) {
                T *Qc = Qt + ((size_t)q_base + (size_t)ci) * F;
#pragma unroll
                for (int k = 0; k < D; ++k) vstore<V>(Qc + (size_t)k * (size_t)n_cls * F, q[k]);
            } else {
#pragma unroll
                for (int k = 0; k < D; ++k) vstore<V>(Qt + (size_t)e[k] * F, q[k]);
            }
        }
    }
}

#ifdef LDPC_VAR_WAVES
#define LDPC_VAR_ATTR __attribute__((amdgpu_waves_per_eu(LDPC_VAR_WAVES, LDPC_VAR_WAVES)))
#else
#define LDPC_VAR_ATTR
#endif
template <int ALGO, int D, int V, typename T>
__global__ __launch_bounds__(kBlock) LDPC_VAR_ATTR void var_kernel(const VarArgs a)
{
    constexpr size_t F = 64 * V;
    const int lane = threadIdx.x & 63;
    const GridPos gp = grid_pos(a.tiles_first);
    const int tile = tile_select<V>(a.tail, a.done, gp.row);
    if (tile < 0) return;
    const int wave = gp.block * kWavesPerBlock + wave_id_in_block();
    const int c_begin = wave * a.cols_per_wave;
    const int c_end = min(c_begin + a.cols_per_wave, a.n_cols);
    const T *Rt = static_cast<const T *>(a.R) + (size_t)tile * (size_t)a.E * F + (size_t)lane * V;
    T *Qt = static_cast<T *>(a.Q) + (size_t)tile * (size_t)a.E * F + (size_t)lane * V;
    const T *chan_t = static_cast<const T *>(a.chan) + (size_t)tile * (size_t)a.N * F + (size_t)lane * V;
    uint64_t *hard_t = a.hard + (size_t)tile * (size_t)a.N * V;
    uint64_t frozen[V];
#pragma unroll
    for (int v = 0; v < V; ++v) frozen[v] = a.done[(size_t)tile * V + v];
    var_columns<ALGO, D, V, T>(Rt, Qt, chan_t, hard_t, frozen, a.cls_col, a.cls_edge, c_begin, c_end, a.write_q, lane, a.q_base, a.n_cols);
}

template <int ALGO, int V, typename T, int D, int DLO> struct VarDispatch {
    static __device__ __forceinline__ void run(int deg, const T *Rt, T *Qt, const T *chan_t, uint64_t *hard_t,
                                               const uint64_t (&frozen)[V], const int32_t *col, const int32_t *edge,
                                               int cb, int ce, int write_q, int lane, int64_t q_base, int n_cls)
    {
        if (deg == D) var_columns<ALGO, D, V, T>(Rt, Qt, chan_t, hard_t, frozen, col, edge, cb, ce, write_q, lane, q_base, n_cls);
        else VarDispatch<ALGO, V, T, D - 1, DLO>::run(deg, Rt, Qt, chan_t, hard_t, frozen, col, edge, cb, ce, write_q, lane, q_base, n_cls);
    }
};
template <int ALGO, int V, typename T, int DLO> struct VarDispatch<ALGO, V, T, DLO, DLO> {
    static __device__ __forceinline__ void run(int, const T *Rt, T *Qt, const T *chan_t, uint64_t *hard_t,
                                               const uint64_t (&frozen)[V], const int32_t *col, const int32_t *edge,
// ... 713 lines not shown
```

### myldpccppapi_amd/csrc/flood_tables.hpp

```cpp
#pragma once

#include "flood_kernels.hpp"

namespace ldpc {

using CheckFn = void (*)(const CheckArgs);
using VarFn = void (*)(const VarArgs);
using LinkFn = void (*)(const CheckArgs, const LinkArgs);
using CheckGroupFn = void (*)(const CheckArgs, const GroupClass *, int);
using VarGroupFn = void (*)(const VarArgs, const GroupClass *, int);
using InitFn = void (*)(const InitArgs);

constexpr int kVarBuckets = 3, kCheckBuckets = 4;
constexpr int kVarBucketLo[kVarBuckets] = {1, 5, 9}, kVarBucketHi[kVarBuckets] = {4, 8, 16};
constexpr int kCheckBucketLo[kCheckBuckets] = {1, 9, 17, 25}, kCheckBucketHi[kCheckBuckets] = {8, 16, 24, 32};

struct FloodFns {
    CheckFn check[kMaxUnrolledCheckDegreeMS + 1] = {};
    CheckFn check_wide[kMaxUnrolledCheckDegreeMS + 1] = {};
    LinkFn link[kMaxUnrolledDegree + 1] = {};
    LinkFn link_narrow[kMaxUnrolledDegree + 1] = {};
    LinkFn link_deep[kMaxUnrolledDegree + 1] = {};
    LinkFn link_half[kMaxUnrolledDegree + 1] = {};
    VarFn var[kMaxUnrolledDegree + 1] = {};
    CheckGroupFn check_group[kCheckBuckets] = {};
    int check_group_width = 1;
    VarGroupFn var_group[kVarBuckets] = {};
    InitFn init = nullptr;
    int max_check_unrolled = kMaxUnrolledDegree;
};

void fill_flood_sp(int V, FloodFns *f);
void fill_flood_ms(int V, FloodFns *f);
void fill_flood_ms16(int V, FloodFns *f);
void fill_flood_msc(int V, FloodFns *f);
void fill_flood_msc16(int V, FloodFns *f);

}
```

### myldpccppapi_amd/csrc/flood_tables_impl.hpp

```cpp
#pragma once

#include "flood_tables.hpp"

namespace ldpc {
namespace tables {

template <int ALGO, int V, typename T, int D> struct FloodTable {
    static void fill(CheckFn *c, CheckFn *cw, VarFn *v)
    {
        c[D] = check_kernel<ALGO, D, V, 1, T>;
        cw[D] = check_kernel<ALGO, D, V, V, T>;
        v[D] = var_kernel<ALGO, D, V, T>;
        FloodTable<ALGO, V, T, D - 1>::fill(c, cw, v);
    }
};
template <int ALGO, int V, typename T> struct FloodTable<ALGO, V, T, 0> {
    static void fill(CheckFn *c, CheckFn *cw, VarFn *v)
    {
        c[0] = cw[0] = check_kernel_generic<ALGO, V, T>;
        v[0] = var_kernel_generic<ALGO, V, T>;
    }
};

template <int ALGO, int V, typename T, int D> struct CheckTableMS {
    static void fill(CheckFn *c, CheckFn *cw)
    {
        c[D] = cw[D] = check_kernel<ALGO, D, V, 1, T>;
        CheckTableMS<ALGO, V, T, D - 1>::fill(c, cw);
    }
};
template <int ALGO, int V, typename T> struct CheckTableMS<ALGO, V, T, kMaxUnrolledDegree> {
    static void fill(CheckFn *, CheckFn *) {}
};

template <int ALGO, int V, typename T, int D> struct LinkHalf {
    static LinkFn get() { return nullptr; }
};
template <int ALGO, typename T, int D> struct LinkHalf<ALGO, 4, T, D> {
    static LinkFn get() { return check_link_narrow_kernel<ALGO, D, 4, T, 2>; }
};
template <int ALGO, int V, typename T, int D> struct LinkTable {
    static void fill(LinkFn *t, LinkFn *tn, LinkFn *td, LinkFn *th)
    {
        t[D] = check_link_kernel<ALGO, D, V, T>;
        tn[D] = check_link_narrow_kernel<ALGO, D, V, T>;
        td[D] = check_link_narrow2_kernel<ALGO, D, V, T>;
        th[D] = LinkHalf<ALGO, V, T, D>::get();
        LinkTable<ALGO, V, T, D - 1>::fill(t, tn, td, th);
    }
};
template <int ALGO, int V, typename T> struct LinkTable<ALGO, V, T, 1> {
    static void fill(LinkFn *, LinkFn *, LinkFn *, LinkFn *) {}
};

template <int ALGO, int V, typename T> void fill_v(FloodFns *f)
{
    constexpr int DM = kMaxUnrolledDegree;
    FloodTable<ALGO, V, T, DM>::fill(f->check, f->check_wide, f->var);
    LinkTable<ALGO, V, T, DM>::fill(f->link, f->link_narrow, f->link_deep, f->link_half);
    constexpr int GW = (sizeof(T) == 2 && V == 4) ? 2 : 1;
    f->check_group_width = GW;
    f->check_group[0] = check_group_kernel<ALGO, V, T, 1, 8, GW>;
    f->check_group[1] = check_group_kernel<ALGO, V, T, 9, 16, GW>;
    f->check_group[2] = f->check_group[3] = nullptr;
    f->var_group[0] = var_group_kernel<ALGO, V, T, 1, 4>;
    f->var_group[1] = var_group_kernel<ALGO, V, T, 5, 8>;
    f->var_group[2] = var_group_kernel<ALGO, V, T, 9, 16>;
    f->init = init_kernel<ALGO, V, T>;
    f->max_check_unrolled = DM;
    if (ALGO != kAlgoSP) {
        CheckTableMS<ALGO, V, T, kMaxUnrolledCheckDegreeMS>::fill(f->check, f->check_wide);
        f->check_group[2] = check_group_kernel<ALGO, V, T, 17, 24, GW>;
        f->check_group[3] = check_group_kernel<ALGO, V, T, 25, 32, GW>;
        f->max_check_unrolled = kMaxUnrolledCheckDegreeMS;
    }
}

template <int ALGO, typename T> void fill(int V, FloodFns *f)
{
    *f = FloodFns();
    if (V == 1) fill_v<ALGO, 1, T>(f);
    else if (V == 2) fill_v<ALGO, 2, T>(f);
    else fill_v<ALGO, 4, T>(f);
}

}
}
```

### myldpccppapi_amd/csrc/ldpc_hip.hip

```cpp
#include <hip/hip_runtime.h>

#include <algorithm>
#include <cstdarg>
#include <cstdio>
#include <cstdlib>
#include <cstring>
#include <memory>
#include <new>
#include <string>
#include <vector>

#include "decoder.hpp"
#include "graph.hpp"

using ldpc::set_error;

namespace {

thread_local std::string g_err;

int pick_frames_per_lane(const ldpc_decoder_config &cfg, int32_t max_row_deg, int32_t max_col_deg)
{
    if (cfg.frames_per_lane) return cfg.frames_per_lane;
    int deg = cfg.algo == LDPC_ALGO_LAYERED ? max_row_deg : max_col_deg;
// ... 39 lines not shown
    *count = n;
    return LDPC_OK;
}

int64_t ldpc_out_bytes(int32_t K, int64_t frames, int32_t pack_mode)
{
    if (frames <= 0 || K <= 0) return 0;
    if (pack_mode == LDPC_PACK_BYTES) return (frames - 1) * (int64_t)K / 8 + K / 8;
    return (frames * (int64_t)K + 7) / 8;
}

int ldpc_graph_create(const int32_t *rows, const int32_t *cols, int64_t E, int32_t M, int32_t N,
                      ldpc_graph **out)
{
    if (!out) return set_error(LDPC_ERR_ARG, "out is NULL");
    *out = nullptr;
    if (!rows || !cols) return set_error(LDPC_ERR_ARG, "rows/cols is NULL");
    if (M <= 0 || N <= 0 || E <= 0) return set_error(LDPC_ERR_ARG, "M, N, E must be positive");
    if (E > 0x7fffffffLL) return set_error(LDPC_ERR_ARG, "E does not fit int32 edge ids");
    for (int64_t e = 0; e < E; ++e) {
        if (rows[e] < 0 || rows[e] >= M || cols[e] < 0 || cols[e] >= N)
            return set_error(LDPC_ERR_ARG, "edge %lld = (%d, %d) outside %d x %d", (long long)e, rows[e],
                        cols[e], M, N);
        if (e && (rows[e] < rows[e - 1] || (rows[e] == rows[e - 1] && cols[e] <= cols[e - 1])))
            return set_error(LDPC_ERR_ARG, "edges must be in strictly ascending row-major order (edge %lld)",
                        (long long)e);
    }
    ldpc_graph *g = new (std::nothrow) ldpc_graph;
    if (!g) return set_error(LDPC_ERR_NOMEM, "out of memory");
    g->M = M; g->N = N; g->E = E;
    g->rows.assign(rows, rows + E);
    g->cols.assign(cols, cols + E);
    g->row_ptr.assign((size_t)M + 1, 0);
    g->col_ptr.assign((size_t)N + 1, 0);
    for (int64_t e = 0; e < E; ++e) { ++g->row_ptr[rows[e] + 1]; ++g->col_ptr[cols[e] + 1]; }
    for (int32_t m = 0; m < M; ++m) {
        g->max_row_deg = std::max(g->max_row_deg, g->row_ptr[m + 1]);
        g->row_ptr[m + 1] += g->row_ptr[m];
    }
    for (int32_t n = 0; n < N; ++n) {
        g->max_col_deg = std::max(g->max_col_deg, g->col_ptr[n + 1]);
        g->col_ptr[n + 1] += g->col_ptr[n];
    }
    g->col_edge.assign((size_t)E, 0);
    std::vector<int32_t> fill(g->col_ptr.begin(), g->col_ptr.end() - 1);
    for (int64_t e = 0; e < E; ++e) g->col_edge[fill[cols[e]]++] = (int32_t)e;
    *out = g;
    return LDPC_OK;
}

int ldpc_graph_destroy(ldpc_graph *g)
{
    delete g;
    return LDPC_OK;
}

int ldpc_graph_info(const ldpc_graph *g, int32_t *M, int32_t *N, int64_t *E, int32_t *max_row_deg,
                    int32_t *max_col_deg)
{
    if (!g) return set_error(LDPC_ERR_ARG, "graph is NULL");
    if (M) *M = g->M;
    if (N) *N = g->N;
    if (E) *E = g->E;
    if (max_row_deg) *max_row_deg = g->max_row_deg;
    if (max_col_deg) *max_col_deg = g->max_col_deg;
    return LDPC_OK;
}

void ldpc_decoder_config_init(ldpc_decoder_config *cfg)
{
    if (!cfg) return;
    memset(cfg, 0, sizeof *cfg);
    cfg->struct_size = sizeof *cfg;
    cfg->max_batch = 1;
    cfg->algo = LDPC_ALGO_SP;
    cfg->msg_dtype = LDPC_MSG_F32;
    cfg->max_iter = 40;
    cfg->llr_scale = 8.0f;
    cfg->early_term = 1;
    cfg->pack_mode = LDPC_PACK_BYTES;
}

static int config_in(const ldpc_decoder_config *cfg, ldpc_decoder_config *full)
{
    constexpr size_t kSizeBeforeMsCorr = offsetof(ldpc_decoder_config, ms_scale);
    if (cfg->struct_size != sizeof(ldpc_decoder_config) && cfg->struct_size != kSizeBeforeMsCorr)
        return set_error(LDPC_ERR_ARG, "config struct_size %u is neither %zu nor %zu (ABI mismatch)", cfg->struct_size,
                    sizeof(ldpc_decoder_config), kSizeBeforeMsCorr);
    memset(full, 0, sizeof *full);
    memcpy(full, cfg, cfg->struct_size);
    full->struct_size = sizeof *full;
    return LDPC_OK;
}

int ldpc_decoder_create(const ldpc_graph *g, const ldpc_decoder_config *cfg_in, ldpc_decoder **out)
{
    if (!out) return set_error(LDPC_ERR_ARG, "out is NULL");
    *out = nullptr;
    if (!g || !cfg_in) return set_error(LDPC_ERR_ARG, "graph/config is NULL");
    ldpc_decoder_config cfg_full;
    if (int rc = config_in(cfg_in, &cfg_full)) return rc;
    const ldpc_decoder_config *cfg = &cfg_full;
    if (cfg->K <= 0 || cfg->K > g->N) return set_error(LDPC_ERR_ARG, "K=%d out of range", cfg->K);
    if (cfg->max_batch <= 0) return set_error(LDPC_ERR_ARG, "max_batch must be positive");
    if (cfg->max_iter <= 0 || cfg->max_iter > 100000) return set_error(LDPC_ERR_ARG, "max_iter out of range");
    if (cfg->algo != LDPC_ALGO_SP && cfg->algo != LDPC_ALGO_MS && cfg->algo != LDPC_ALGO_LAYERED &&
        cfg->algo != LDPC_ALGO_MS_FUSED && cfg->algo != LDPC_ALGO_LAYERED_HOST)
        return set_error(LDPC_ERR_ARG, "unknown algo %d", cfg->algo);
    if (!(cfg->ms_scale >= 0.0f && cfg->ms_scale <= 1.0f))
        return set_error(LDPC_ERR_ARG, "ms_scale must be 0 (off) or in (0, 1]");
    if (!(cfg->ms_offset >= 0.0f && cfg->ms_offset < 1000.0f))
        return set_error(LDPC_ERR_ARG, "ms_offset must be 0 (off) or in (0, 1000)");
    const bool ms_corr = cfg->ms_scale != 0.0f || cfg->ms_offset != 0.0f;
    if (ms_corr && cfg->algo != LDPC_ALGO_MS && cfg->algo != LDPC_ALGO_LAYERED)
        return set_error(LDPC_ERR_UNSUPPORTED, "ms_scale / ms_offset apply to LDPC_ALGO_MS and LDPC_ALGO_LAYERED only "
                    "(SP has no minimum to correct; MS_FUSED and LAYERED_HOST reproduce reference kernels)");
    if (cfg->algo == LDPC_ALGO_LAYERED_HOST) {
        for (int32_t m = 1; m < g->M; ++m)
            if (g->row_ptr[m + 1] - g->row_ptr[m] != g->row_ptr[1] - g->row_ptr[0])
                return set_error(LDPC_ERR_UNSUPPORTED, "LAYERED_HOST follows the reference's host-layered path, which sizes its "
                            "layers correctly only when every row of H has the same weight (MyLdpc.cpp:907,958)");
        if (g->max_row_deg > ldpc::kMaxUnrolledLayerDegree)
            return set_error(LDPC_ERR_UNSUPPORTED, "LAYERED_HOST: row weight %d > %d", g->max_row_deg, ldpc::kMaxUnrolledLayerDegree);
    }
    if (cfg->pack_mode != LDPC_PACK_BYTES && cfg->pack_mode != LDPC_PACK_BITS)
        return set_error(LDPC_ERR_ARG, "unknown pack_mode %d", cfg->pack_mode);
    if (cfg->frames_per_lane != 0 && cfg->frames_per_lane != 1 && cfg->frames_per_lane != 2 &&
        cfg->frames_per_lane != 4)
        return set_error(LDPC_ERR_ARG, "frames_per_lane must be 0, 1, 2 or 4");
    if (cfg->msg_dtype != LDPC_MSG_F32 && cfg->msg_dtype != LDPC_MSG_F16)
        return set_error(LDPC_ERR_ARG, "unknown msg_dtype %d", cfg->msg_dtype);
    if (cfg->msg_dtype == LDPC_MSG_F16 && cfg->algo != LDPC_ALGO_MS)
        return set_error(LDPC_ERR_UNSUPPORTED, "fp16 messages are built for flooding min-sum only "
                    "(the probability-domain SP needs fp32 range; layered: not yet)");
    if (!ldpc::tune_valid(*cfg)) return set_error(LDPC_ERR_ARG, "tuning / streams config fields out of range");

    int ndev = 0;
    LDPC_HIP_TRY(hipGetDeviceCount(&ndev));
    if (cfg->device < 0 || cfg->device >= ndev)
        return set_error(LDPC_ERR_HIP, "device %d not present (%d HIP devices)", cfg->device, ndev);
    LDPC_HIP_TRY(hipSetDevice(cfg->device));

    ldpc_decoder *d = new (std::nothrow) ldpc_decoder;
    if (!d) return set_error(LDPC_ERR_NOMEM, "out of memory");
    std::unique_ptr<ldpc_decoder> guard(d);
    d->cfg = *cfg;
    d->ms_corr = ms_corr;
    d->ms_scale = cfg->ms_scale != 0.0f ? cfg->ms_scale : 1.0f;
    d->ms_offset = cfg->ms_offset;
    d->M = g->M; d->N = g->N; d->E = g->E;
    d->h_cols = g->cols;
    const ldpc::Tune tune = d->tune = ldpc::tune_from_config(*cfg);
    d->flood.syn_xcd = ldpc::tune_pick(tune.syn_xcd, true);
    d->flood.check_wide = ldpc::tune_pick(tune.check_wide, false);
    d->flood.link_form = ldpc::tune_pick(tune.link_half, false) ? 2 : (ldpc::tune_pick(tune.link_narrow, true) ? 1 : 0);
    d->flood.link_deep = ldpc::tune_pick(tune.link_deep, false);
    if (tune.link_rows) d->flood.link_rpw = tune.link_rows < 0 ? 0 : tune.link_rows;
    LDPC_HIP_TRY(hipDeviceGetAttribute(&d->flood.cus, hipDeviceAttributeMultiprocessorCount, cfg->device));
    d->V = pick_frames_per_lane(*cfg, g->max_row_deg, g->max_col_deg);
    d->F = 64 * d->V;
    d->T = (cfg->max_batch + d->F - 1) / d->F;
    if (d->T == 1 && !tune.link_rows) d->flood.link_rpw = 4;

    LDPC_HIP_TRY(d->stream.create());
    LDPC_HIP_TRY(d->tm.ev_begin.create());
    LDPC_HIP_TRY(d->tm.ev_end.create());
    LDPC_HIP_TRY(d->flood.h_active.alloc(1));
    LDPC_HIP_TRY(d->flood.h_summary.alloc(2));
    LDPC_HIP_TRY(d->flood.ev_summary.create(false));
    LDPC_HIP_TRY(d->row_ptr.upload(g->row_ptr));
    LDPC_HIP_TRY(d->edge_col.upload(g->cols));
    LDPC_HIP_TRY(d->col_ptr.upload(g->col_ptr));
    LDPC_HIP_TRY(d->col_edge.upload(g->col_edge));
    d->flood.TO = (ldpc::kCompactCapacity + d->F - 1) / d->F;
    d->flood.tail_enabled = cfg->early_term && cfg->poll_interval == 0 && ldpc::tune_pick(tune.device_tail, true) &&
                      (cfg->algo == LDPC_ALGO_SP || cfg->algo == LDPC_ALGO_MS) && d->T >= 4 * d->flood.TO && t_child_depth == 0;
    if (!d->flood.tail_enabled) d->flood.TO = 0;
    d->flood.TA = d->T + d->flood.TO;
    const size_t TF = (size_t)d->flood.TA * d->F;
    LDPC_HIP_TRY(d->hard.alloc((size_t)d->flood.TA * d->N * d->V));
    LDPC_HIP_TRY(d->failw.alloc((size_t)(cfg->max_iter + 2) * d->flood.TA * d->V));
    LDPC_HIP_TRY(d->done.alloc((size_t)d->flood.TA * d->V));
    LDPC_HIP_TRY(d->iters.alloc(TF));
    LDPC_HIP_TRY(d->active.alloc(1));
    LDPC_HIP_TRY(d->summary.alloc(4));

    if (cfg->algo == LDPC_ALGO_MS_FUSED) {
        if (cfg->pack_mode != LDPC_PACK_BYTES && cfg->K % 8)
            return set_error(LDPC_ERR_UNSUPPORTED, "MS_FUSED packs whole bytes per frame only");
        if (!ldpc::tune_forced_off(tune.ldsp)) {
            LDPC_HIP_TRY(ldpc::engine_ldsp_plan_create(&d->ldsp, g->M, g->N, g->E, g->row_ptr, g->cols, cfg->layer_rows, cfg->K,
                                           cfg->max_batch, cfg->device, tune, 2));
            if (d->ldsp.eligible && (ldpc::tune_forced_on(tune.ldsp) || d->ldsp.lds_bytes <= 80 * 1024)) d->use_ldsp = true;
            else d->ldsp = ldpc::LdspPlan();
        }
        if (!d->use_ldsp) {
            LDPC_HIP_TRY(ldpc::fused_plan_create(&d->fused, g->M, g->N, g->E, g->row_ptr, g->cols, cfg->layer_rows));
            if (!d->fused.eligible)
                return set_error(LDPC_ERR_UNSUPPORTED, "MS_FUSED needs a quasi-cyclic H (circulant size = layer_rows) whose "
                            "posteriors fit in LDS");
        }
        d->use_fused = true;
    } else if (cfg->algo == LDPC_ALGO_LAYERED_HOST) {
        d->layered.host_arith = 1;
        int rc = ldpc::layered_plan_create(&d->layered, g->M, g->N, g->E, g->row_ptr, g->cols, cfg->layer_rows, d->T, d->V);
        if (rc == -1) return set_error(LDPC_ERR_ARG, "layer_rows=%d must divide M=%d and rows of a layer "
                                  "must not share a column", cfg->layer_rows, g->M);
        if (rc) return set_error(LDPC_ERR_HIP, "layered plan allocation failed: %s", hipGetErrorString(hipGetLastError()));
    } else if (cfg->algo == LDPC_ALGO_LAYERED) {
        if (d->ms_corr && ldpc::tune_forced_on(tune.fused) && ldpc::tune_forced_off(tune.ldsp))
            return set_error(LDPC_ERR_UNSUPPORTED, "ms_scale / ms_offset: the LDS-resident layered kernel (LDPC_TUNE_FUSED on, "
                        "LDPC_TUNE_LDSP off) carries no correction; the record or the streaming kernels do");
        if (!ldpc::tune_forced_off(tune.fused) && (cfg->pack_mode == LDPC_PACK_BYTES || cfg->K % 8 == 0)) {
            if (!d->ms_corr) {
                LDPC_HIP_TRY(ldpc::fused_plan_create(&d->fused, g->M, g->N, g->E, g->row_ptr, g->cols, cfg->layer_rows));
                d->use_fused = d->fused.eligible;
            }
            if (!ldpc::tune_forced_off(tune.ldsp)) {
                d->ldsp.corr = d->ms_corr;
                d->ldsp.mc = ldpc::MsCorr{d->ms_scale, d->ms_offset};
                LDPC_HIP_TRY(ldpc::engine_ldsp_plan_create(&d->ldsp, g->M, g->N, g->E, g->row_ptr, g->cols, cfg->layer_rows,
                                               cfg->K, cfg->max_batch, cfg->device, tune, 0));
                if (d->ldsp.eligible) d->use_fused = d->use_ldsp = true;
            }
        }
        d->layered.corr = d->ms_corr;
        d->layered.ms_scale = d->ms_scale;
        d->layered.ms_offset = d->ms_offset;
        int rc = d->use_fused ? 0 : ldpc::layered_plan_create(&d->layered, g->M, g->N, g->E, g->row_ptr, g->cols,
                                                              cfg->layer_rows, d->T, d->V);
        if (rc == -1) return set_error(LDPC_ERR_ARG, "layer_rows=%d must divide M=%d and rows of a layer "
                                  "must not share a column", cfg->layer_rows, g->M);
        if (rc) return set_error(LDPC_ERR_HIP, "layered plan allocation failed: %s",
                            hipGetErrorString(hipGetLastError()));
    } else {
        if (d->ms_corr && ldpc::tune_forced_on(tune.fused) && ldpc::tune_forced_off(tune.ldsp))
            return set_error(LDPC_ERR_UNSUPPORTED, "ms_scale / ms_offset: the LDS-resident flooding kernel (LDPC_TUNE_FUSED on, "
                        "LDPC_TUNE_LDSP off) carries no correction; the record or the streaming kernels do");
        if (cfg->msg_dtype == LDPC_MSG_F32 && cfg->layer_rows > 0 && cfg->frames_per_lane == 0 &&
            (cfg->pack_mode == LDPC_PACK_BYTES || cfg->K % 8 == 0)) {
            const bool small = (int64_t)cfg->max_batch * g->E <= (int64_t)1 << 23;
            if (!d->ms_corr && ldpc::tune_pick(tune.fused, small)) {
                LDPC_HIP_TRY(ldpc::fused_plan_create(&d->fused, g->M, g->N, g->E, g->row_ptr, g->cols, cfg->layer_rows));
                d->use_fused = d->fused.eligible && (cfg->algo == LDPC_ALGO_MS || d->fused.eligible_sp);
            }
            if (cfg->algo == LDPC_ALGO_MS && !ldpc::tune_forced_off(tune.fused) && !ldpc::tune_forced_off(tune.ldsp)) {
                d->ldsp.corr = d->ms_corr;
                d->ldsp.mc = ldpc::MsCorr{d->ms_scale, d->ms_offset};
                LDPC_HIP_TRY(ldpc::engine_ldsp_plan_create(&d->ldsp, g->M, g->N, g->E, g->row_ptr, g->cols, cfg->layer_rows,
                                               cfg->K, cfg->max_batch, cfg->device, tune, 1));
                if (d->ldsp.eligible && (ldpc::tune_forced_on(tune.ldsp) || d->ldsp.lds_bytes <= 80 * 1024))
                    d->use_fused = d->use_ldsp = true;
                else
                    d->ldsp = ldpc::LdspPlan();
            }
        }
        if (!d->use_fused) {
            int rc = ldpc::engine_flood_setup(d, g, TF, t_child_depth == 0);
            if (rc) return rc;
            if (d->flood.tail_enabled) {
                LDPC_HIP_TRY(d->flood.tail_state.alloc(4));
                LDPC_HIP_TRY(d->flood.tail_map.alloc((size_t)d->flood.TO * d->F));
                LDPC_HIP_TRY(d->flood.running.alloc((size_t)cfg->max_iter + 2));
            }
            if (t_child_depth == 0) d->flood.child_capacity = cfg->max_batch >= 4096 ? 2 * ldpc::kCompactCapacity : ldpc::kCompactCapacity;
            else d->flood.child_capacity = cfg->max_batch > ldpc::kCompactCapacity ? ldpc::kCompactCapacity : ldpc::kLastCapacity;
            d->flood.compact_threshold = d->flood.child_capacity;
            if (tune.compact) d->flood.compact_threshold = tune.compact < 0 ? 0 : std::min(d->flood.child_capacity, tune.compact);
            const bool may_have_child = t_child_depth == 0 || cfg->max_batch > ldpc::kLastCapacity;
            if (cfg->early_term && cfg->poll_interval > 0 && d->T > 1 && d->flood.compact_threshold > 0 && may_have_child) {
                ldpc_decoder_config cc = *cfg;
                cc.max_batch = d->flood.child_capacity;
                cc.frames_per_lane = (d->flood.child_capacity > ldpc::kCompactCapacity && d->V == 4) ? 4 : 1;
                cc.layer_rows = 0;
                cc.tune_compact = d->flood.child_capacity > ldpc::kLastCapacity ? 0 : -1;
                ++t_child_depth;
                ldpc_decoder *child = nullptr;
                rc = ldpc_decoder_create(g, &cc, &child);
                --t_child_depth;
                if (rc) return rc;
                d->flood.child.reset(child);
                d->flood.child->flood.is_child = true;
                LDPC_HIP_TRY(hipSetDevice(cfg->device));
                LDPC_HIP_TRY(d->flood.cmap.alloc((size_t)d->flood.child_capacity));
                LDPC_HIP_TRY(d->flood.cinv.alloc((size_t)d->T * d->F));
                LDPC_HIP_TRY(d->flood.cmoved.alloc((size_t)d->T * d->V));
            }
        }
    }
    *out = guard.release();
    return LDPC_OK;
}

int ldpc_decoder_destroy(ldpc_decoder *d)
{
    if (!d) return LDPC_OK;
    size_t stuck = d->host.stuck_blocks.size() + d->host.locked_blocks.size();
    for (ldpc_decoder *sh : d->shards) stuck += sh->host.stuck_blocks.size() + sh->host.locked_blocks.size();
    delete d;
    if (stuck) {
        fprintf(stderr, "ldpc_decoder_destroy: %zu page-locked block(s) of caller memory were never released\n", stuck);
        return set_error(LDPC_ERR_STATE, "%zu page-locked block(s) of caller memory could not be released "
                    "(hipHostUnregister failed in an earlier ldpc_decode)", stuck);
    }
    return LDPC_OK;
}

int ldpc_shard_range(int64_t frames, int32_t part, int32_t parts, int32_t unit, int64_t *lo, int64_t *hi)
{
    if (!lo || !hi) return set_error(LDPC_ERR_ARG, "lo/hi is NULL");
    if (frames < 0 || parts <= 0 || part < 0 || part >= parts || unit <= 0)
        return set_error(LDPC_ERR_ARG, "shard_range(frames=%lld, part=%d, parts=%d, unit=%d)", (long long)frames, part, parts, unit);
    const int64_t nu = (frames + unit - 1) / unit, base = nu / parts, rem = nu % parts;
    const int64_t lo_u = part * base + std::min<int64_t>(part, rem);
    const int64_t hi_u = lo_u + base + (part < rem ? 1 : 0);
    *lo = std::min(lo_u * unit, frames);
    *hi = std::min(hi_u * unit, frames);
    return LDPC_OK;
}

int ldpc_decoder_create_multi(const ldpc_graph *g, const ldpc_decoder_config *cfg, const int32_t *devices,
                              int32_t n_devices, ldpc_decoder **out)
{
    if (!out) return set_error(LDPC_ERR_ARG, "out is NULL");
    *out = nullptr;
    if (!g || !cfg) return set_error(LDPC_ERR_ARG, "graph/config is NULL");
    if (!devices || n_devices <= 0 || n_devices > 64) return set_error(LDPC_ERR_ARG, "devices[] must hold 1..64 ordinals");
    ldpc_decoder_config cfg_full;
    if (int rc = config_in(cfg, &cfg_full)) return rc;
    cfg = &cfg_full;
    ldpc_decoder *grp = new (std::nothrow) ldpc_decoder;
    if (!grp) return set_error(LDPC_ERR_NOMEM, "out of memory");
    std::unique_ptr<ldpc_decoder> guard(grp);
    for (int32_t i = 0; i < n_devices; ++i) {
// ... 82 lines not shown
```

### myldpccppapi_amd/csrc/tune.hpp

```cpp
#pragma once

#include "../../include/ldpc_hip.h"

namespace ldpc {

struct Tune {
    int fused = 0, ldsp = 0, ldsp_ext = 0, ldsp_pack = 0, link_narrow = 0, check_wide = 0, syn_xcd = 0,
        fused_pack = 0, fused_loop = 0, device_tail = 0, merge = 0, link_deep = 0, link_half = 0, link_guided = 0, tiles_first = 0;
    int rows_per_wave = 0, cols_per_wave = 0;
    int link_rows = 0;
    int compact = 0;
    int ldsp_grid = 0, ldsp_per_cu = 0, ldsp_waves = 0;
    int place = 0;
    int q_order = 0;
};

inline Tune tune_from_config(const ldpc_decoder_config &c)
{
    Tune t;
    auto f = [&](int field) { return (c.tune_flags >> field) & 3; };
    t.fused = f(LDPC_TUNE_FUSED);
    t.ldsp = f(LDPC_TUNE_LDSP);
    t.ldsp_ext = f(LDPC_TUNE_LDSP_EXT);
    t.ldsp_pack = f(LDPC_TUNE_LDSP_PACK);
    t.link_narrow = f(LDPC_TUNE_LINK_NARROW);
    t.check_wide = f(LDPC_TUNE_CHECK_WIDE);
    t.syn_xcd = f(LDPC_TUNE_SYN_XCD);
    t.fused_pack = f(LDPC_TUNE_FUSED_PACK);
    t.fused_loop = f(LDPC_TUNE_FUSED_LOOP);
    t.device_tail = f(LDPC_TUNE_DEVICE_TAIL);
    t.merge = f(LDPC_TUNE_MERGE);
    t.link_deep = f(LDPC_TUNE_LINK_DEEP);
    t.link_half = f(LDPC_TUNE_LINK_HALF);
    t.link_guided = f(LDPC_TUNE_LINK_GUIDED);
    t.tiles_first = f(LDPC_TUNE_TILES_FIRST);
    t.rows_per_wave = c.tune_rows_per_wave;
    t.cols_per_wave = c.tune_cols_per_wave;
    t.link_rows = c.tune_link_rows;
    t.compact = c.tune_compact;
    t.ldsp_grid = c.tune_ldsp_grid;
    t.ldsp_per_cu = c.tune_ldsp_shape & 255;
    t.ldsp_waves = (c.tune_ldsp_shape >> 8) & 255;
    t.place = c.tune_place;
    t.q_order = c.tune_q_order;
    return t;
}

inline bool tune_pick(int tri, bool dflt) { return tri == 1 ? true : (tri == 2 ? false : dflt); }
inline bool tune_forced_on(int tri) { return tri == 1; }
inline bool tune_forced_off(int tri) { return tri == 2; }

inline bool tune_valid(const ldpc_decoder_config &c)
{
    for (int field = 0; field <= LDPC_TUNE_TILES_FIRST; field += 2)
        if (((c.tune_flags >> field) & 3) == 3) return false;
    if (c.tune_flags >> (LDPC_TUNE_TILES_FIRST + 2)) return false;
    return c.tune_rows_per_wave >= 0 && c.tune_rows_per_wave <= 4096 && c.tune_cols_per_wave >= 0 &&
           c.tune_cols_per_wave <= 4096 && c.tune_link_rows >= -1 && c.tune_link_rows <= 4096 &&
           c.tune_compact >= -1 && c.tune_ldsp_grid >= 0 && c.tune_ldsp_shape >= 0 && c.tune_ldsp_shape < 65536 &&
           c.tune_place >= 0 && c.tune_place <= 8 && c.host_input >= 0 && c.host_input <= 2 && c.host_copy_threads >= 0 && c.host_copy_threads <= 16 &&
           c.tune_q_order >= -1 && c.tune_q_order <= 1;
}

}
```

Baseline: 1128 Mbit/s.

## Read channel LLRs directly in first round and fuse syndrome with state update

Adds FIRST-templated check and link kernels that read channel values through edge_col and convert them to the sum-product probability form in registers. This lets the first iteration skip the separate Q initialisation pass, and it now also applies to SP and to linked rows. Separately, a lean syndrome kernel driven by a per-row-class table folds the state/termination update into the syndrome launch using per-tile counters. The aim is to cut one full-E memory pass and one kernel launch per checked iteration, at the cost of many more kernel instantiations and a new termination path that can be switched off by a tune flag.

```diff
diff --git a/include/ldpc_hip.h b/include/ldpc_hip.h
--- a/include/ldpc_hip.h
+++ b/include/ldpc_hip.h
@@ -83,10 +83,11 @@
     LDPC_TUNE_LINK_DEEP = 22,
     LDPC_TUNE_LINK_HALF = 24,
     LDPC_TUNE_LINK_GUIDED = 26,
-    LDPC_TUNE_TILES_FIRST = 28
-};
-#define LDPC_TUNE_ON(field) (1 << (field))
-#define LDPC_TUNE_OFF(field) (2 << (field))
+    LDPC_TUNE_TILES_FIRST = 28,
+    LDPC_TUNE_LEAN_ROUNDS = 30
+};
+#define LDPC_TUNE_ON(field) ((int32_t)(1u << (field)))
+#define LDPC_TUNE_OFF(field) ((int32_t)(2u << (field)))
 
 typedef struct ldpc_decode_stats {
     int32_t iterations_launched;
diff --git a/myldpccppapi_amd/capi.py b/myldpccppapi_amd/capi.py
--- a/myldpccppapi_amd/capi.py
+++ b/myldpccppapi_amd/capi.py
@@ -18,6 +18,7 @@
 TUNE_FIELDS = {"fused": 0, "ldsp": 2, "ldsp_ext": 4, "ldsp_pack": 6, "link_narrow": 8, "check_wide": 10,
                "syn_xcd": 12, "fused_pack": 14, "fused_loop": 16, "device_tail": 18, "merge": 20, "link_deep": 22, "link_half": 24,
                "link_guided": 26, "tiles_first": 28}
+TUNE_OFF_ONLY = {"lean_rounds": 30}
 TUNE_INTS = ("rows_per_wave", "cols_per_wave", "link_rows", "compact", "ldsp_grid", "ldsp_per_cu", "ldsp_waves", "place", "q_order")
 
 
@@ -27,6 +28,9 @@
         if k in TUNE_FIELDS:
             if v is not None:
                 flags |= (1 if v else 2) << TUNE_FIELDS[k]
+        elif k in TUNE_OFF_ONLY:
+            if v is not None and not v:
+                flags |= 2 << TUNE_OFF_ONLY[k]
         elif k == "ldsp_per_cu":
             shape |= int(v) & 255
         elif k == "ldsp_waves":
@@ -35,7 +39,7 @@
             setattr(cfg, "tune_" + k, int(v))
         else:
             raise KeyError("unknown tuning field %r" % k)
-    cfg.tune_flags, cfg.tune_ldsp_shape = flags, shape
+    cfg.tune_flags, cfg.tune_ldsp_shape = flags - (1 << 32 if flags >> 31 else 0), shape
 
 
 def hbm_probe(device=0, nbytes=1 << 30, reps=5, by_policy=False):
@@ -58,7 +62,7 @@
     for name, key in (("FUSED", "fused"), ("LDSP", "ldsp"), ("LDSP_EXT", "ldsp_ext"), ("LDSP_PACK", "ldsp_pack"),
                       ("LINK_NARROW", "link_narrow"), ("CHECK_WIDE", "check_wide"), ("SYN_XCD", "syn_xcd"),
                       ("FUSED_LOOP", "fused_loop"), ("DEVICE_TAIL", "device_tail"), ("MERGE", "merge"), ("LINK_DEEP", "link_deep"), ("LINK_HALF", "link_half"),
-                      ("LINK_GUIDED", "link_guided"), ("TILES_FIRST", "tiles_first")):
+                      ("LINK_GUIDED", "link_guided"), ("TILES_FIRST", "tiles_first"), ("LEAN_ROUNDS", "lean_rounds")):
         if "LDPC_TUNE_" + name in env:
             t[key] = int(env["LDPC_TUNE_" + name]) != 0
     if "LDPC_TUNE_NO_PACK" in env:
diff --git a/myldpccppapi_amd/csrc/decoder.hpp b/myldpccppapi_amd/csrc/decoder.hpp
--- a/myldpccppapi_amd/csrc/decoder.hpp
+++ b/myldpccppapi_amd/csrc/decoder.hpp
@@ -98,6 +98,10 @@
     Event ev_summary;
     bool summary_pending = false;
     int idle_after = 0;
+
+    bool lean = true;
+    DevBuf<GroupClass> syn_table;
+    int syn_blocks = 0;
 
     bool first_round_from_chan = false;
 };
diff --git a/myldpccppapi_amd/csrc/engine_flood.hip b/myldpccppapi_amd/csrc/engine_flood.hip
--- a/myldpccppapi_amd/csrc/engine_flood.hip
+++ b/myldpccppapi_amd/csrc/engine_flood.hip
@@ -58,6 +58,8 @@
 {
     using namespace ldpc;
     const int64_t msz = d->flood.msg_size;
+    const bool first = it == 1 && d->flood.first_round_from_chan;
+    const FloodFns &fn = d->flood.fns;
     for (auto &rc : d->flood.row_classes) {
         if (!rc.linked) continue;
         LDPC_HIP_TRY(span_begin(d, s, 4, rc.degree,
@@ -68,6 +70,7 @@
         CheckArgs a{d->flood.Q.p, d->flood.R.p, rc.e0.p, d->done.p, d->E, rc.count, 1, rc.degree, d->ms_scale, tr};
         a.ms_offset = d->ms_offset;
         a.qpos = d->flood.qpos.p;
+        if (first) { a.edge_col = d->edge_col.p; a.N = d->N; }
         LinkArgs lk{rc.link_col.p, rc.link_pos.p, d->flood.chan.p, d->flood.Q.p, d->hard.p, d->N,
                     (it < max_iter) ? 1 : 0, d->tm.tap_iter ? 1 : 0, d->flood.extra_e0.p, d->flood.extra_deg.p, d->flood.n_extra, 0,
                     rc.n_big, rc.small_rows};
@@ -76,8 +79,10 @@
         const int waves = link_chunk_count(d->flood.link_rpw, rc.n_big, rc.small_rows, rc.count) * (variant == 1 ? V : variant == 2 ? V / 2 : 1);
         lk.link_blocks = (waves + kWavesPerBlock - 1) / kWavesPerBlock;
         const dim3 grid = flood_grid(d, lk.link_blocks + (d->flood.n_extra + kWavesPerBlock - 1) / kWavesPerBlock, tiles, &a.tiles_first, true);
-        (variant == 2 ? d->flood.fns.link_half : variant == 1 ? (d->flood.link_deep ? d->flood.fns.link_deep : d->flood.fns.link_narrow) : d->flood.fns.link)
-            [rc.degree]<<<grid, kBlock, 0, s>>>(a, lk);
+        const LinkFn *forms = variant == 2 ? (first ? fn.link_half_first : fn.link_half)
+                              : variant == 1 ? (d->flood.link_deep ? (first ? fn.link_deep_first : fn.link_deep) : (first ? fn.link_narrow_first : fn.link_narrow))
+                                             : (first ? fn.link_first : fn.link);
+        forms[rc.degree]<<<grid, kBlock, 0, s>>>(a, lk);
         LDPC_HIP_TRY(span_end(d, s));
     }
     for (auto &g : d->flood.check_groups) {
@@ -87,9 +92,9 @@
         CheckArgs a{d->flood.Q.p, d->flood.R.p, nullptr, d->done.p, d->E, 0, (d->tune.rows_per_wave ? d->tune.rows_per_wave : 2) * (fat ? kIdleFat : 1), 0, d->ms_scale, tr};
         a.ms_offset = d->ms_offset;
         a.qpos = d->flood.qpos.p;
-        if (it == 1 && d->flood.first_round_from_chan) { a.first_chan = d->flood.chan.p; a.edge_col = d->edge_col.p; a.N = d->N; }
+        if (first) { a.first_chan = d->flood.chan.p; a.edge_col = d->edge_col.p; a.N = d->N; }
         const dim3 grid = flood_grid(d, fat ? g.blocks_fat : g.blocks, tiles, &a.tiles_first);
-        d->flood.fns.check_group[g.bucket]<<<grid, kBlock, 0, s>>>(a, fat ? g.table_fat.p : g.table.p, (int)g.members.size());
+        (first ? fn.check_group_first : fn.check_group)[g.bucket]<<<grid, kBlock, 0, s>>>(a, fat ? g.table_fat.p : g.table.p, (int)g.members.size());
         LDPC_HIP_TRY(span_end(d, s));
     }
     for (int ci : d->flood.check_solo) {
@@ -98,14 +103,14 @@
         CheckArgs a{d->flood.Q.p, d->flood.R.p, rc.e0.p, d->done.p, d->E, rc.count, 1, rc.degree, d->ms_scale, tr};
         a.ms_offset = d->ms_offset;
         a.qpos = d->flood.qpos.p;
-        if (it == 1 && d->flood.first_round_from_chan) { a.first_chan = d->flood.chan.p; a.edge_col = d->edge_col.p; a.N = d->N; }
+        if (first) { a.first_chan = d->flood.chan.p; a.edge_col = d->edge_col.p; a.N = d->N; }
         const int slotk = rc.degree <= d->flood.fns.max_check_unrolled ? rc.degree : 0;
         const bool narrow = slotk && (!d->flood.check_wide || rc.degree > kMaxUnrolledDegree);
         const int rpw = (d->tune.rows_per_wave ? d->tune.rows_per_wave : (narrow ? 2 : 1)) * (fat ? kIdleFat : 1);
         a.rows_per_wave = rpw;
         const int waves = ((rc.count + rpw - 1) / rpw) * (narrow ? V : 1);
         const dim3 grid = flood_grid(d, (waves + kWavesPerBlock - 1) / kWavesPerBlock, tiles, &a.tiles_first);
-        (narrow ? d->flood.fns.check : d->flood.fns.check_wide)[slotk]<<<grid, kBlock, 0, s>>>(a);
+        (narrow ? (first ? fn.check_first : fn.check) : (first ? fn.check_wide_first : fn.check_wide))[slotk]<<<grid, kBlock, 0, s>>>(a);
         LDPC_HIP_TRY(span_end(d, s));
     }
     return LDPC_OK;
@@ -236,9 +241,18 @@
                       d->E, frames, d->N, tiles, d->T, d->flood.TO * F, std::min(d->flood.compact_threshold, d->flood.TO * F), 0, max_iter};
     }
 
-    bool q_less = d->cfg.algo == LDPC_ALGO_MS && !resume && !d->tm.tap_iter && max_iter > 1 && d->flood.n_extra == 0;
-    for (auto &rc : d->flood.row_classes) if (rc.linked) q_less = false;
-    for (int ci : d->flood.check_solo) if (d->flood.row_classes[ci].degree > d->flood.fns.max_check_unrolled) q_less = false;
+    bool q_less = !resume && !d->tm.tap_iter && max_iter > 1;
+    {
+        const FloodFns &fn = d->flood.fns;
+        if (!d->flood.lean && (d->cfg.algo != LDPC_ALGO_MS || d->flood.n_extra != 0)) q_less = false;
+        for (auto &rc : d->flood.row_classes)
+            if (rc.linked && (!d->flood.lean || rc.degree > kMaxUnrolledDegree || !fn.link_first[rc.degree])) q_less = false;
+        for (auto &g : d->flood.check_groups) if (!fn.check_group_first[g.bucket]) q_less = false;
+        for (int ci : d->flood.check_solo) {
+            const int deg = d->flood.row_classes[ci].degree;
+            if (deg > fn.max_check_unrolled || !fn.check_first[deg] || !fn.check_wide_first[deg]) q_less = false;
+        }
+    }
     d->flood.first_round_from_chan = q_less;
     if (!resume) {
         LDPC_HIP_TRY(span_begin(d, s, 3));
@@ -267,20 +281,27 @@
         if (freeze || it == rounds) {
             LDPC_HIP_TRY(span_begin(d, s, 3));
             uint64_t *fw = d->failw.p + (size_t)it * slot;
-            const int rbk = (d->M + kBlock - 1) / kBlock;
-            SyndromeArgs sa{d->row_ptr.p, d->edge_col.p, d->hard.p, fw, d->done.p, d->M, d->N,
-                            d->flood.syn_xcd ? tiles : 0, rbk, tr};
-            dim3 sgrid = d->flood.syn_xcd ? dim3(8 * rbk * ((tiles + 7) / 8)) : dim3(rbk, tiles);
-            syndrome_kernel<V><<<sgrid, kBlock, 0, s>>>(sa);
-            StateArgs st{d->done.p, fw, d->iters.p, nullptr, frames, it, max_iter, 1, tr, use_tail ? d->flood.running.p : nullptr,
-                         d->summary.p + 2};
             const bool poll = freeze && it < rounds && d->cfg.poll_interval > 0 && !d->host.suppress_poll &&
                               ((it % d->cfg.poll_interval) == 0 || poll_dense);
-            if (poll) {
-                LDPC_HIP_TRY(hipMemsetAsync(d->active.p, 0, sizeof(int32_t), s));
-                st.active = d->active.p;
-            }
-            state_kernel<V><<<tiles, 64, 0, s>>>(st);
+            if (poll) LDPC_HIP_TRY(hipMemsetAsync(d->active.p, 0, sizeof(int32_t), s));
+            if (d->flood.lean) {
+                const int rbk = d->flood.syn_blocks;
+                int32_t *counters = reinterpret_cast<int32_t *>(d->failw.p + (size_t)(max_iter + 2) * slot) + (size_t)it * d->flood.TA;
+                SyndromeLeanArgs sa{d->edge_col.p, d->hard.p, fw, d->done.p, d->flood.syn_table.p, (int)d->flood.row_classes.size(), d->N,
+                                    d->flood.syn_xcd ? tiles : 0, rbk, tr, counters, d->iters.p, poll ? d->active.p : nullptr,
+                                    use_tail ? d->flood.running.p : nullptr, d->summary.p + 2, it};
+                dim3 sgrid = d->flood.syn_xcd ? dim3(8 * rbk * ((tiles + 7) / 8)) : dim3(rbk, tiles);
+                syndrome_lean_kernel<V><<<sgrid, kBlock, 0, s>>>(sa);
+            } else {
+                const int rbk = (d->M + kBlock - 1) / kBlock;
+                SyndromeArgs sa{d->row_ptr.p, d->edge_col.p, d->hard.p, fw, d->done.p, d->M, d->N,
+                                d->flood.syn_xcd ? tiles : 0, rbk, tr};
+                dim3 sgrid = d->flood.syn_xcd ? dim3(8 * rbk * ((tiles + 7) / 8)) : dim3(rbk, tiles);
+                syndrome_kernel<V><<<sgrid, kBlock, 0, s>>>(sa);
+                StateArgs st{d->done.p, fw, d->iters.p, poll ? d->active.p : nullptr, frames, it, max_iter, 1, tr,
+                             use_tail ? d->flood.running.p : nullptr, d->summary.p + 2};
+                state_kernel<V><<<tiles, 64, 0, s>>>(st);
+            }
             if (use_tail && it < rounds) {
                 ta.iter = it;
                 const unsigned tg = (unsigned)std::min<int64_t>(1024, d->E + 2 * (int64_t)d->N);
@@ -508,6 +529,18 @@
     };
     for (int k = 0; k < kCheckBuckets; ++k) LDPC_HIP_TRY(make(d->flood.check_groups, d->flood.check_solo, cb[k], k, kCheckBucketLo[k], kCheckBucketHi[k], true));
     for (int k = 0; k < kVarBuckets; ++k) LDPC_HIP_TRY(make(d->flood.var_groups, d->flood.var_solo, vb[k], k, kVarBucketLo[k], kVarBucketHi[k], false));
+    {
+        std::vector<GroupClass> tab;
+        d->flood.syn_blocks = 0;
+        for (const RowClass &rc : d->flood.row_classes) {
+            GroupClass gc{};
+            gc.block_begin = d->flood.syn_blocks; gc.degree = rc.degree; gc.count = rc.count; gc.ids = rc.e0.p; gc.edges = nullptr; gc.q_base = -1;
+            tab.push_back(gc);
+            d->flood.syn_blocks += (rc.count + ldpc::kBlock - 1) / ldpc::kBlock;
+        }
+        if (tab.empty()) d->flood.lean = false;
+        else LDPC_HIP_TRY(d->flood.syn_table.upload(tab));
+    }
     return LDPC_OK;
 }
 
diff --git a/myldpccppapi_amd/csrc/flood_kernels.hpp b/myldpccppapi_amd/csrc/flood_kernels.hpp
--- a/myldpccppapi_amd/csrc/flood_kernels.hpp
+++ b/myldpccppapi_amd/csrc/flood_kernels.hpp
@@ -158,6 +158,19 @@
     return __builtin_amdgcn_readfirstlane(qpos[e]);
 }
 
+template <int ALGO> __device__ __forceinline__ float first_q(float c)
+{
+    if (ALGO == kAlgoSP) return c / (1.0f + c) - 1.0f / (1.0f + c);
+    return c;
+}
+template <int ALGO, int D, int W> __device__ __forceinline__ void first_inputs(float (&x)[D][W])
+{
+#pragma unroll
+    for (int k = 0; k < D; ++k)
+#pragma unroll
+        for (int w = 0; w < W; ++w) x[k][w] = first_q<ALGO>(x[k][w]);
+}
+
 struct GridPos { int row, block; };
 __device__ __forceinline__ GridPos grid_pos(int tiles_first)
 {
@@ -224,7 +237,7 @@
 
 __device__ __forceinline__ MsCorr ms_corr_of(const CheckArgs &a) { return MsCorr{a.ms_scale, a.ms_offset}; }
 
-template <int ALGO, int D, int V, int W, typename T>
+template <int ALGO, int D, int V, int W, typename T, bool FIRST = false>
 __global__ __launch_bounds__(kBlock) void check_kernel(const CheckArgs a)
 {
     constexpr size_t F = 64 * V;
@@ -241,12 +254,16 @@
     const T *Qu = static_cast<const T *>(a.Q) + (size_t)tile * (size_t)a.E * F;
     T *Rt = static_cast<T *>(a.R) + (size_t)tile * (size_t)a.E * F + lane_off;
 
-    const T *Ct = (ALGO != kAlgoSP && a.first_chan)
+    const T *Ct = ((FIRST || ALGO != kAlgoSP) && a.first_chan)
                       ? static_cast<const T *>(a.first_chan) + (size_t)tile * (size_t)a.N * F + lane_off : nullptr;
     for (int r = r_begin; r < r_end; ++r) {
         const int e0 = a.cls_e0[r];
         float x[D][W], out[D][W];
-        if (ALGO != kAlgoSP && Ct) {
+        if (FIRST) {
+#pragma unroll
+            for (int k = 0; k < D; ++k) vload<W>(x[k], Ct + (size_t)a.edge_col[e0 + k] * F);
+            first_inputs<ALGO, D, W>(x);
+        } else if (ALGO != kAlgoSP && Ct) {
 #pragma unroll
             for (int k = 0; k < D; ++k) vload<W>(x[k], Ct + (size_t)a.edge_col[e0 + k] * F);
         } else {
@@ -261,7 +278,7 @@
     }
 }
 
-template <int ALGO, int V, typename T>
+template <int ALGO, int V, typename T, bool FIRST = false>
 __device__ __forceinline__ void check_row_generic(const T *Qu, unsigned lane_off, T *Rt, int e0, int D,
                                                   const int32_t *__restrict__ qpos, const MsCorr &c)
 {
@@ -275,6 +292,10 @@
         for (int j = 0; j < D; ++j) {
             float xj[V];
             vload<V>(xj, Qu + (size_t)edge_slot(qpos, e0 + j) * F + lane_off);
+            if (FIRST) {
+#pragma unroll
+                for (int v = 0; v < V; ++v) xj[v] = first_q<ALGO>(xj[v]);
+            }
 #pragma unroll
             for (int v = 0; v < V; ++v) {
                 const float m = __builtin_fabsf(xj[v]);
@@ -290,6 +311,10 @@
         for (int k = 0; k < D; ++k) {
             float xk[V], o[V];
             vload<V>(xk, Qu + (size_t)edge_slot(qpos, e0 + k) * F + lane_off);
+            if (FIRST) {
+#pragma unroll
+                for (int v = 0; v < V; ++v) xk[v] = first_q<ALGO>(xk[v]);
+            }
 #pragma unroll
             for (int v = 0; v < V; ++v) {
                 const float b = (k == idx[v]) ? m2[v] : m1[v];
@@ -309,6 +334,10 @@
             if (j == k) continue;
             float xj[V];
             vload<V>(xj, Qu + (size_t)edge_slot(qpos, e0 + j) * F + lane_off);
+            if (FIRST) {
+#pragma unroll
+                for (int v = 0; v < V; ++v) xj[v] = first_q<ALGO>(xj[v]);
+            }
 #pragma unroll
             for (int v = 0; v < V; ++v) p[v] *= xj[v];
         }
@@ -344,7 +373,7 @@
     int64_t q_base;
 };
 
-template <int ALGO, int D, int V, int W, typename T>
+template <int ALGO, int D, int V, int W, typename T, bool FIRST = false>
 __device__ __forceinline__ void check_rows(const T *Qu, unsigned lane_off, T *Rt, const int32_t *__restrict__ e0s, int r_begin, int r_end,
                                            const T *Ct, const int32_t *__restrict__ edge_col,
                                            const int32_t *__restrict__ qpos, const MsCorr &c)
@@ -354,7 +383,11 @@
     for (int r = r_begin; r < r_end; ++r) {
         const int e0 = e0s[r];
         float x[D][W], out[D][W];
-        if (ALGO != kAlgoSP && Ct) {
+        if (FIRST) {
+#pragma unroll
+            for (int k = 0; k < D; ++k) vload<W>(x[k], Ct + (size_t)edge_col[e0 + k] * F);
+            first_inputs<ALGO, D, W>(x);
+        } else if (ALGO != kAlgoSP && Ct) {
 #pragma unroll
             for (int k = 0; k < D; ++k) vload<W>(x[k], Ct + (size_t)edge_col[e0 + k] * F);
         } else {
@@ -369,23 +402,23 @@
     }
 }
 
-template <int ALGO, int V, typename T, int D, int DLO, int W = 1> struct CheckDispatch {
+template <int ALGO, int V, typename T, int D, int DLO, int W = 1, bool FIRST = false> struct CheckDispatch {
     static __device__ __forceinline__ void run(int deg, const T *Qu, unsigned lane_off, T *Rt, const int32_t *e0s, int rb, int re,
                                                const T *Ct, const int32_t *edge_col, const int32_t *qpos, const MsCorr &c)
     {
-        if (deg == D) check_rows<ALGO, D, V, W, T>(Qu, lane_off, Rt, e0s, rb, re, Ct, edge_col, qpos, c);
-        else CheckDispatch<ALGO, V, T, D - 1, DLO, W>::run(deg, Qu, lane_off, Rt, e0s, rb, re, Ct, edge_col, qpos, c);
+        if (deg == D) check_rows<ALGO, D, V, W, T, FIRST>(Qu, lane_off, Rt, e0s, rb, re, Ct, edge_col, qpos, c);
+        else CheckDispatch<ALGO, V, T, D - 1, DLO, W, FIRST>::run(deg, Qu, lane_off, Rt, e0s, rb, re, Ct, edge_col, qpos, c);
     }
 };
-template <int ALGO, int V, typename T, int DLO, int W> struct CheckDispatch<ALGO, V, T, DLO, DLO, W> {
+template <int ALGO, int V, typename T, int DLO, int W, bool FIRST> struct CheckDispatch<ALGO, V, T, DLO, DLO, W, FIRST> {
     static __device__ __forceinline__ void run(int, const T *Qu, unsigned lane_off, T *Rt, const int32_t *e0s, int rb, int re,
                                                const T *Ct, const int32_t *edge_col, const int32_t *qpos, const MsCorr &c)
     {
-        check_rows<ALGO, DLO, V, W, T>(Qu, lane_off, Rt, e0s, rb, re, Ct, edge_col, qpos, c);
+        check_rows<ALGO, DLO, V, W, T, FIRST>(Qu, lane_off, Rt, e0s, rb, re, Ct, edge_col, qpos, c);
     }
 };
 
-template <int ALGO, int V, typename T, int DLO, int DHI, int W = 1>
+template <int ALGO, int V, typename T, int DLO, int DHI, int W = 1, bool FIRST = false>
 __global__ __launch_bounds__(kBlock) void check_group_kernel(const CheckArgs a, const GroupClass *__restrict__ cls, int n_classes)
 {
     constexpr size_t F = 64 * V;
@@ -403,9 +436,9 @@
     const unsigned lane_off = (unsigned)sub * 64 * W + (unsigned)lane * W;
     const T *Qu = static_cast<const T *>(a.Q) + (size_t)tile * (size_t)a.E * F;
     T *Rt = static_cast<T *>(a.R) + (size_t)tile * (size_t)a.E * F + lane_off;
-    const T *Ct = (ALGO != kAlgoSP && a.first_chan)
+    const T *Ct = ((FIRST || ALGO != kAlgoSP) && a.first_chan)
                       ? static_cast<const T *>(a.first_chan) + (size_t)tile * (size_t)a.N * F + lane_off : nullptr;
-    CheckDispatch<ALGO, V, T, DHI, DLO, W>::run(cls[c].degree, Qu, lane_off, Rt, cls[c].ids, r_begin, r_end, Ct, a.edge_col, a.qpos, ms_corr_of(a));
+    CheckDispatch<ALGO, V, T, DHI, DLO, W, FIRST>::run(cls[c].degree, Qu, lane_off, Rt, cls[c].ids, r_begin, r_end, Ct, a.edge_col, a.qpos, ms_corr_of(a));
 }
 
 struct SyndromeArgs {
@@ -467,6 +500,160 @@
         const uint64_t seen = __hip_atomic_load(dst, __ATOMIC_RELAXED, __HIP_MEMORY_SCOPE_AGENT);
         if (x & ~seen) atomicOr(dst, (unsigned long long)x);
     }
+}
+
+#ifndef LDPC_SYN_FENCE
+#define LDPC_SYN_FENCE 0
+#endif
+struct SyndromeLeanArgs {
+    const int32_t *__restrict__ edge_col;
+    const uint64_t *__restrict__ hard;
+    uint64_t *fail;
+    uint64_t *done;
+    const GroupClass *__restrict__ cls;
+    int32_t n_classes;
+    int32_t N;
+    int32_t tiles;
+    int32_t row_blocks;
+    TailRef tail;
+    int32_t *counter;
+    int32_t *__restrict__ iters;
+    int32_t *__restrict__ active;
+    int32_t *__restrict__ running;
+    int32_t *__restrict__ tile_rounds;
+    int32_t iter;
+};
+
+typedef unsigned long long vu2 __attribute__((ext_vector_type(2)));
+template <int V> __device__ __forceinline__ void load_words(uint64_t (&w)[V], const uint64_t *p);
+template <> __device__ __forceinline__ void load_words<1>(uint64_t (&w)[1], const uint64_t *p) { w[0] = *p; }
+template <> __device__ __forceinline__ void load_words<2>(uint64_t (&w)[2], const uint64_t *p)
+{
+    const vu2 t = *reinterpret_cast<const vu2 *>(p);
+    w[0] = t.x; w[1] = t.y;
+}
+template <> __device__ __forceinline__ void load_words<4>(uint64_t (&w)[4], const uint64_t *p)
+{
+    const vu2 t = reinterpret_cast<const vu2 *>(p)[0], u = reinterpret_cast<const vu2 *>(p)[1];
+    w[0] = t.x; w[1] = t.y; w[2] = u.x; w[3] = u.y;
+}
+
+template <int D, int V>
+__device__ __forceinline__ void syndrome_row(const int32_t *__restrict__ edge_col, const uint64_t *__restrict__ hard_t, int e0, int deg,
+                                             uint64_t (&s)[V])
+{
+    if (D == 0) {
+        for (int k = 0; k < deg; ++k) {
+            uint64_t w[V];
+            load_words<V>(w, hard_t + (size_t)edge_col[e0 + k] * V);
+#pragma unroll
+            for (int v = 0; v < V; ++v) s[v] ^= w[v];
+        }
+        return;
+    }
+    constexpr int DD = D > 0 ? D : 1;
+    int c[DD];
+    uint64_t w[DD][V];
+#pragma unroll
+    for (int k = 0; k < DD; ++k) c[k] = edge_col[e0 + k];
+#pragma unroll
+    for (int k = 0; k < DD; ++k) load_words<V>(w[k], hard_t + (size_t)c[k] * V);
+#pragma unroll
+    for (int k = 0; k < DD; ++k)
+#pragma unroll
+        for (int v = 0; v < V; ++v) s[v] ^= w[k][v];
+}
+
+template <int V, int D> struct SyndromeDispatch {
+    static __device__ __forceinline__ void run(int deg, const int32_t *edge_col, const uint64_t *hard_t, int e0, uint64_t (&s)[V])
+    {
+        if (deg == D) syndrome_row<D, V>(edge_col, hard_t, e0, deg, s);
+        else SyndromeDispatch<V, D - 1>::run(deg, edge_col, hard_t, e0, s);
+    }
+};
+template <int V> struct SyndromeDispatch<V, 0> {
+    static __device__ __forceinline__ void run(int deg, const int32_t *edge_col, const uint64_t *hard_t, int e0, uint64_t (&s)[V])
+    {
+        syndrome_row<0, V>(edge_col, hard_t, e0, deg, s);
+    }
+};
+
+template <int V> __global__ __launch_bounds__(kBlock) void syndrome_lean_kernel(const SyndromeLeanArgs a)
+{
+    constexpr int F = 64 * V;
+    int tile, rb;
+    if (a.tiles > 0) {
+        const int xcd = blockIdx.x & 7, j = blockIdx.x >> 3;
+        tile = xcd + 8 * (j / a.row_blocks);
+        rb = j % a.row_blocks;
+        if (tile >= a.tiles) return;
+    } else {
+        tile = blockIdx.y;
+        rb = blockIdx.x;
+    }
+    tile = tile_select<V>(a.tail, a.done, tile);
+    if (tile < 0) return;
+    int c = 0;
+    while (c + 1 < a.n_classes && rb >= a.cls[c + 1].block_begin) ++c;
+    const int r = (rb - a.cls[c].block_begin) * kBlock + threadIdx.x;
+    const uint64_t *hard_t = a.hard + (size_t)tile * (size_t)a.N * V;
+    uint64_t s[V];
+#pragma unroll
+    for (int v = 0; v < V; ++v) s[v] = 0;
+    if (r < a.cls[c].count) SyndromeDispatch<V, kMaxUnrolledDegree>::run(a.cls[c].degree, a.edge_col, hard_t, a.cls[c].ids[r], s);
+    __shared__ uint64_t part[kWavesPerBlock][V];
+#pragma unroll
+    for (int v = 0; v < V; ++v) {
+        uint64_t x = s[v];
+#pragma unroll
+        for (int off = 32; off >= 1; off >>= 1) {
+            const uint32_t lo = __shfl_xor((uint32_t)x, off);
+            const uint32_t hi = __shfl_xor((uint32_t)(x >> 32), off);
+            x |= ((uint64_t)hi << 32) | lo;
+        }
+        if ((threadIdx.x & 63) == 0) part[threadIdx.x >> 6][v] = x;
+    }
+    __syncthreads();
+    if (threadIdx.x >= 64) return;
+    if (threadIdx.x < V) {
+        uint64_t x = 0;
+#pragma unroll
+        for (int w = 0; w < kWavesPerBlock; ++w) x |= part[w][threadIdx.x];
+        unsigned long long *dst = reinterpret_cast<unsigned long long *>(&a.fail[(size_t)tile * V + threadIdx.x]);
+        const uint64_t seen = __hip_atomic_load(dst, __ATOMIC_RELAXED, __HIP_MEMORY_SCOPE_AGENT);
+        if (x & ~seen) atomicOr(dst, (unsigned long long)x);
+    }
+#if LDPC_SYN_FENCE == 2
+    __threadfence();
+#elif LDPC_SYN_FENCE == 1
+    __builtin_amdgcn_fence(__ATOMIC_RELEASE, "agent");
+#else
+    __builtin_amdgcn_s_waitcnt(0);
+#endif
+    int last = 0;
+    if (threadIdx.x == 0) last = (atomicAdd(&a.counter[tile], 1) == a.row_blocks - 1);
+    if (!__builtin_amdgcn_readfirstlane(last)) return;
+#if LDPC_SYN_FENCE == 2
+    __threadfence();
+#else
+    __builtin_amdgcn_fence(__ATOMIC_ACQUIRE, "agent");
+#endif
+    const int lane = threadIdx.x;
+    int n_active = 0;
+#pragma unroll
+    for (int v = 0; v < V; ++v) {
+        const uint64_t old = a.done[(size_t)tile * V + v];
+        const uint64_t clean = ~__hip_atomic_load(reinterpret_cast<unsigned long long *>(&a.fail[(size_t)tile * V + v]),
+                                                  __ATOMIC_RELAXED, __HIP_MEMORY_SCOPE_AGENT);
+        const uint64_t newly = clean & ~old;
+        if ((newly >> lane) & 1ull) a.iters[(size_t)tile * F + lane * V + v] = a.iter;
+        const uint64_t d = old | clean;
+        if (lane == 0) a.done[(size_t)tile * V + v] = d;
+        n_active += __popcll(~d);
+    }
+    if (lane == 0 && n_active && a.active) atomicAdd(a.active, n_active);
+    if (lane == 0 && n_active && a.running) atomicAdd(&a.running[a.iter], n_active);
+    if (lane == 0 && a.tile_rounds) atomicAdd(a.tile_rounds, 1);
 }
 
 
@@ -552,16 +739,17 @@
     return n_big + (rest > 0 ? (rest + small_rows - 1) / small_rows : 0);
 }
 
-template <int ALGO, int V, typename T>
+template <int ALGO, int V, typename T, bool FIRST = false>
 __device__ __forceinline__ void link_extra_rows(const CheckArgs &a, const LinkArgs &g, int tile, int block)
 {
     constexpr size_t F = 64 * V;
     const int lane = threadIdx.x & 63;
     const int w = (block - g.link_blocks) * kWavesPerBlock + wave_id_in_block();
     if (w >= g.n_extra) return;
-    const T *Qu = static_cast<const T *>(a.Q) + (size_t)tile * (size_t)a.E * F;
+    const T *Qu = FIRST ? static_cast<const T *>(g.chan) + (size_t)tile * (size_t)g.N * F
+                        : static_cast<const T *>(a.Q) + (size_t)tile * (size_t)a.E * F;
     T *Rt = static_cast<T *>(a.R) + (size_t)tile * (size_t)a.E * F + (size_t)lane * V;
-    check_row_generic<ALGO, V, T>(Qu, (unsigned)lane * V, Rt, g.extra_e0[w], g.extra_deg[w], a.qpos, ms_corr_of(a));
+    check_row_generic<ALGO, V, T, FIRST>(Qu, (unsigned)lane * V, Rt, g.extra_e0[w], g.extra_deg[w], FIRST ? a.edge_col : a.qpos, ms_corr_of(a));
 }
 
 #ifdef LDPC_LINK_WIDE_WAVES
@@ -569,7 +757,7 @@
 #else
 #define LDPC_LINK_WIDE_ATTR
 #endif
-template <int ALGO, int D, int V, typename T>
+template <int ALGO, int D, int V, typename T, bool FIRST = false>
 __global__ __launch_bounds__(kBlock) LDPC_LINK_WIDE_ATTR void check_link_kernel(const CheckArgs a, const LinkArgs g)
 {
     constexpr size_t F = 64 * V;
@@ -577,13 +765,15 @@
     const GridPos gp = grid_pos(a.tiles_first);
     const int tile = tile_select<V>(a.tail, a.done, gp.row);
     if (tile < 0) return;
-    if (gp.block >= g.link_blocks) { link_extra_rows<ALGO, V, T>(a, g, tile, gp.block); return; }
+    if (gp.block >= g.link_blocks) { link_extra_rows<ALGO, V, T, FIRST>(a, g, tile, gp.block); return; }
     const int wave = gp.block * kWavesPerBlock + wave_id_in_block();
     int r_begin, r_end;
     link_chunk_rows(wave, a.rows_per_wave, g.n_big, g.small_rows, a.n_rows, &r_begin, &r_end);
     const size_t lane_off = (size_t)lane * V;
     const unsigned lane_q = (unsigned)lane * V;
-    const T *Qt = static_cast<const T *>(a.Q) + (size_t)tile * (size_t)a.E * F;
+    const T *Qt = FIRST ? static_cast<const T *>(g.chan) + (size_t)tile * (size_t)g.N * F
+                        : static_cast<const T *>(a.Q) + (size_t)tile * (size_t)a.E * F;
+    const int32_t *__restrict__ in_idx = FIRST ? a.edge_col : a.qpos;
     T *Qwt = static_cast<T *>(g.Qw) + (size_t)tile * (size_t)a.E * F;
     T *Rt = static_cast<T *>(a.R) + (size_t)tile * (size_t)a.E * F + lane_off;
     const T *chan_t = static_cast<const T *>(g.chan) + (size_t)tile * (size_t)g.N * F + lane_off;
@@ -602,7 +792,7 @@
 #pragma unroll
     for (int k = 0; k < D; ++k) qc[k] = qn[k] = 0;
     if (r_begin < r_end) {
-        row_slots<D>(a.qpos, a.cls_e0[r_begin], lane, qc);
+        row_slots<D>(in_idx, a.cls_e0[r_begin], lane, qc);
 #pragma unroll
         for (int k = 0; k < D; ++k) vload<V>(x[k], Qt + (size_t)qc[k] * F + lane_q);
     }
@@ -612,7 +802,7 @@
         const int pos = g.link_pos[r];
         const int ka = next_col >= 0 ? (pos & 255) : -1;
         const int kb = pend_col >= 0 ? pend_kb : -1;
-        if (r + 1 < r_end) row_slots<D>(a.qpos, a.cls_e0[r + 1], lane, qn);
+        if (r + 1 < r_end) row_slots<D>(in_idx, a.cls_e0[r + 1], lane, qn);
         float ch[V];
         uint64_t old_w[V];
         if (pend_col >= 0) {
@@ -621,6 +811,7 @@
             for (int v = 0; v < V; ++v) old_w[v] = hard_t[(size_t)pend_col * V + v];
         }
         float out[D][V];
+        if (FIRST) first_inputs<ALGO, D, V>(x);
         if (ALGO == kAlgoSP) check_sp<D, V>(x, out); else if (ALGO == kAlgoMS) check_ms<D, V>(x, out); else check_ms<D, V, true, T>(x, out, ms_corr_of(a));
         if (r + 1 < r_end) {
 #pragma unroll
@@ -670,6 +861,7 @@
                 int qw1 = qc[0];
 #pragma unroll
                 for (int k = 1; k < D; ++k) qw1 = (k == kb) ? qc[k] : qw1;
+                if (FIRST) qw1 = edge_slot(a.qpos, e0 + kb);
                 vstore<V>(Qwt + (size_t)pend_edge * F + lane_q, q[0]);
                 vstore<V>(Qwt + (size_t)qw1 * F + lane_q, q[1]);
             }
@@ -679,6 +871,7 @@
             pend_edge = qc[0];
 #pragma unroll
             for (int k = 1; k < D; ++k) pend_edge = (k == ka) ? qc[k] : pend_edge;
+            if (FIRST) pend_edge = edge_slot(a.qpos, e0 + ka);
             pend_kb = (pos >> 8) & 255;
 #pragma unroll
             for (int v = 0; v < V; ++v) {
@@ -713,7 +906,7 @@
     return x;
 }
 
-template <int ALGO, int D, int V, typename T, int W = 1>
+template <int ALGO, int D, int V, typename T, int W = 1, bool FIRST = false>
 __global__ __launch_bounds__(kBlock) void check_link_narrow_kernel(const CheckArgs a, const LinkArgs g)
 {
     constexpr size_t F = 64 * V;
@@ -723,14 +916,16 @@
     const GridPos gp = grid_pos(a.tiles_first);
     const int tile = tile_select<V>(a.tail, a.done, gp.row);
     if (tile < 0) return;
-    if (gp.block >= g.link_blocks) { link_extra_rows<ALGO, V, T>(a, g, tile, gp.block); return; }
+    if (gp.block >= g.link_blocks) { link_extra_rows<ALGO, V, T, FIRST>(a, g, tile, gp.block); return; }
     const int wave = gp.block * kWavesPerBlock + wave_id_in_block();
     const int sub = wave % SUBS;
     int r_begin, r_end;
     link_chunk_rows(wave / SUBS, a.rows_per_wave, g.n_big, g.small_rows, a.n_rows, &r_begin, &r_end);
     const size_t lane_off = (size_t)sub * 64 * W + (size_t)lane * W;
     const unsigned lane_q = (unsigned)lane_off;
-    const T *Qt = static_cast<const T *>(a.Q) + (size_t)tile * (size_t)a.E * F;
+    const T *Qt = FIRST ? static_cast<const T *>(g.chan) + (size_t)tile * (size_t)g.N * F
+                        : static_cast<const T *>(a.Q) + (size_t)tile * (size_t)a.E * F;
+    const int32_t *__restrict__ in_idx = FIRST ? a.edge_col : a.qpos;
     T *Qwt = static_cast<T *>(g.Qw) + (size_t)tile * (size_t)a.E * F;
     T *Rt = static_cast<T *>(a.R) + (size_t)tile * (size_t)a.E * F + lane_off;
     const T *chan_t = static_cast<const T *>(g.chan) + (size_t)tile * (size_t)g.N * F + lane_off;
@@ -754,7 +949,7 @@
 #pragma unroll
     for (int k = 0; k < D; ++k) qc[k] = qn[k] = 0;
     if (r_begin < r_end) {
-        row_slots<D>(a.qpos, a.cls_e0[r_begin], lane, qc);
+        row_slots<D>(in_idx, a.cls_e0[r_begin], lane, qc);
 #pragma unroll
         for (int k = 0; k < D; ++k) vload<W>(x[k], Qt + (size_t)qc[k] * F + lane_q);
     }
@@ -764,7 +959,7 @@
         const int pos = g.link_pos[r];
         const int ka = next_col >= 0 ? (pos & 255) : -1;
         const int kb = pend_col >= 0 ? pend_kb : -1;
-        if (r + 1 < r_end) row_slots<D>(a.qpos, a.cls_e0[r + 1], lane, qn);
+        if (r + 1 < r_end) row_slots<D>(in_idx, a.cls_e0[r + 1], lane, qn);
         float ch[W];
         uint64_t old_mine[W];
 #pragma unroll
@@ -775,6 +970,7 @@
             for (int w = 0; w < W; ++w) old_mine[w] = load_field(pend_col, (W * lane + w) % V);
         }
         float out[D][W];
+        if (FIRST) first_inputs<ALGO, D, W>(x);
         if (ALGO == kAlgoSP) check_sp<D, W>(x, out); else if (ALGO == kAlgoMS) check_ms<D, W>(x, out); else check_ms<D, W, true, T>(x, out, ms_corr_of(a));
         if (r + 1 < r_end) {
 #pragma unroll
@@ -831,6 +1027,7 @@
                 int qw1 = qc[0];
 #pragma unroll
                 for (int k = 1; k < D; ++k) qw1 = (k == kb) ? qc[k] : qw1;
+                if (FIRST) qw1 = edge_slot(a.qpos, e0 + kb);
                 vstore<W>(Qwt + (size_t)pend_edge * F + lane_q, q[0]);
                 vstore<W>(Qwt + (size_t)qw1 * F + lane_q, q[1]);
             }
@@ -840,6 +1037,7 @@
             pend_edge = qc[0];
 #pragma unroll
             for (int k = 1; k < D; ++k) pend_edge = (k == ka) ? qc[k] : pend_edge;
+            if (FIRST) pend_edge = edge_slot(a.qpos, e0 + ka);
             pend_kb = (pos >> 8) & 255;
 #pragma unroll
             for (int w = 0; w < W; ++w) {
@@ -854,7 +1052,7 @@
     }
 }
 
-template <int ALGO, int D, int V, typename T>
+template <int ALGO, int D, int V, typename T, bool FIRST = false>
 __global__ __launch_bounds__(kBlock) void check_link_narrow2_kernel(const CheckArgs a, const LinkArgs g)
 {
     constexpr size_t F = 64 * V;
@@ -863,13 +1061,15 @@
     const GridPos gp = grid_pos(a.tiles_first);
     const int tile = tile_select<V>(a.tail, a.done, gp.row);
     if (tile < 0) return;
-    if (gp.block >= g.link_blocks) { link_extra_rows<ALGO, V, T>(a, g, tile, gp.block); return; }
+    if (gp.block >= g.link_blocks) { link_extra_rows<ALGO, V, T, FIRST>(a, g, tile, gp.block); return; }
     const int wave = gp.block * kWavesPerBlock + wave_id_in_block();
     const int sub = wave % V;
     int r_begin, r_end;
     link_chunk_rows(wave / V, a.rows_per_wave, g.n_big, g.small_rows, a.n_rows, &r_begin, &r_end);
     const size_t lane_off = (size_t)sub * 64 + lane;
-    const T *Qt = static_cast<const T *>(a.Q) + (size_t)tile * (size_t)a.E * F + lane_off;
+    const T *Qt = FIRST ? static_cast<const T *>(g.chan) + (size_t)tile * (size_t)g.N * F + lane_off
+                        : static_cast<const T *>(a.Q) + (size_t)tile * (size_t)a.E * F + lane_off;
+    const int32_t *__restrict__ in_idx = FIRST ? a.edge_col : a.qpos;
     T *Qwt = static_cast<T *>(g.Qw) + (size_t)tile * (size_t)a.E * F + lane_off;
     T *Rt = static_cast<T *>(a.R) + (size_t)tile * (size_t)a.E * F + lane_off;
     const T *chan_t = static_cast<const T *>(g.chan) + (size_t)tile * (size_t)g.N * F + lane_off;
@@ -891,7 +1091,7 @@
     auto load_row = [&](float (&dst)[D], int r) {
         const int e = a.cls_e0[r];
 #pragma unroll
-        for (int k = 0; k < D; ++k) { float t[1]; vload<1>(t, Qt + (size_t)edge_slot(a.qpos, e + k) * F); dst[k] = t[0]; }
+        for (int k = 0; k < D; ++k) { float t[1]; vload<1>(t, Qt + (size_t)edge_slot(in_idx, e + k) * F); dst[k] = t[0]; }
     };
     if (r_begin < r_end) load_row(b0, r_begin);
     if (r_begin + 1 < r_end) load_row(b1, r_begin + 1);
@@ -910,7 +1110,7 @@
         if (r + 2 < r_end) load_row(pre, r + 2);
         float xx[D][1], out[D][1];
 #pragma unroll
-        for (int k = 0; k < D; ++k) xx[k][0] = x[k];
+        for (int k = 0; k < D; ++k) xx[k][0] = FIRST ? first_q<ALGO>(x[k]) : x[k];
         if (ALGO == kAlgoSP) check_sp<D, 1>(xx, out); else if (ALGO == kAlgoMS) check_ms<D, 1>(xx, out); else check_ms<D, 1, true, T>(xx, out, ms_corr_of(a));
 #pragma unroll
         for (int k = 0; k < D; ++k)
diff --git a/myldpccppapi_amd/csrc/flood_tables.hpp b/myldpccppapi_amd/csrc/flood_tables.hpp
--- a/myldpccppapi_amd/csrc/flood_tables.hpp
+++ b/myldpccppapi_amd/csrc/flood_tables.hpp
@@ -28,6 +28,13 @@
     VarGroupFn var_group[kVarBuckets] = {};
     InitFn init = nullptr;
     int max_check_unrolled = kMaxUnrolledDegree;
+    CheckFn check_first[kMaxUnrolledCheckDegreeMS + 1] = {};
+    CheckFn check_wide_first[kMaxUnrolledCheckDegreeMS + 1] = {};
+    LinkFn link_first[kMaxUnrolledDegree + 1] = {};
+    LinkFn link_narrow_first[kMaxUnrolledDegree + 1] = {};
+    LinkFn link_deep_first[kMaxUnrolledDegree + 1] = {};
+    LinkFn link_half_first[kMaxUnrolledDegree + 1] = {};
+    CheckGroupFn check_group_first[kCheckBuckets] = {};
 };
 
 void fill_flood_sp(int V, FloodFns *f);
diff --git a/myldpccppapi_amd/csrc/flood_tables_impl.hpp b/myldpccppapi_amd/csrc/flood_tables_impl.hpp
--- a/myldpccppapi_amd/csrc/flood_tables_impl.hpp
+++ b/myldpccppapi_amd/csrc/flood_tables_impl.hpp
@@ -53,6 +53,54 @@
     static void fill(LinkFn *, LinkFn *, LinkFn *, LinkFn *) {}
 };
 
+template <int ALGO, int V, typename T, int D> struct FirstCheckTable {
+    static void fill(CheckFn *c, CheckFn *cw)
+    {
+        c[D] = check_kernel<ALGO, D, V, 1, T, true>;
+        cw[D] = check_kernel<ALGO, D, V, V, T, true>;
+        FirstCheckTable<ALGO, V, T, D - 1>::fill(c, cw);
+    }
+};
+template <int ALGO, int V, typename T> struct FirstCheckTable<ALGO, V, T, 0> {
+    static void fill(CheckFn *, CheckFn *) {}
+};
+template <int ALGO, int V, typename T, int D> struct FirstLinkHalf {
+    static LinkFn get() { return nullptr; }
+};
+template <int ALGO, typename T, int D> struct FirstLinkHalf<ALGO, 4, T, D> {
+    static LinkFn get() { return check_link_narrow_kernel<ALGO, D, 4, T, 2, true>; }
+};
+template <int ALGO, int V, typename T, int D> struct FirstLinkTable {
+    static void fill(LinkFn *t, LinkFn *tn, LinkFn *td, LinkFn *th)
+    {
+        t[D] = check_link_kernel<ALGO, D, V, T, true>;
+        tn[D] = check_link_narrow_kernel<ALGO, D, V, T, 1, true>;
+        td[D] = check_link_narrow2_kernel<ALGO, D, V, T, true>;
+        th[D] = FirstLinkHalf<ALGO, V, T, D>::get();
+        FirstLinkTable<ALGO, V, T, D - 1>::fill(t, tn, td, th);
+    }
+};
+template <int ALGO, int V, typename T> struct FirstLinkTable<ALGO, V, T, 1> {
+    static void fill(LinkFn *, LinkFn *, LinkFn *, LinkFn *) {}
+};
+template <int ALGO, int V, typename T> void fill_first_round(FloodFns *f)
+{
+    if constexpr (ALGO != kAlgoSP) {
+        for (int d = 1; d <= f->max_check_unrolled; ++d) { f->check_first[d] = f->check[d]; f->check_wide_first[d] = f->check_wide[d]; }
+        for (int k = 0; k < kCheckBuckets; ++k) f->check_group_first[k] = f->check_group[k];
+    }
+#ifndef LDPC_NO_FIRST_ROUND
+    if constexpr (ALGO == kAlgoSP) {
+        constexpr int GW = (sizeof(T) == 2 && V == 4) ? 2 : 1;
+        FirstCheckTable<ALGO, V, T, kMaxUnrolledDegree>::fill(f->check_first, f->check_wide_first);
+        f->check_group_first[0] = check_group_kernel<ALGO, V, T, 1, 8, GW, true>;
+        f->check_group_first[1] = check_group_kernel<ALGO, V, T, 9, 16, GW, true>;
+    }
+    if constexpr (ALGO != kAlgoMSC)
+        FirstLinkTable<ALGO, V, T, kMaxUnrolledDegree>::fill(f->link_first, f->link_narrow_first, f->link_deep_first, f->link_half_first);
+#endif
+}
+
 template <int ALGO, int V, typename T> void fill_v(FloodFns *f)
 {
     constexpr int DM = kMaxUnrolledDegree;
@@ -74,6 +122,7 @@
         f->check_group[3] = check_group_kernel<ALGO, V, T, 25, 32, GW>;
         f->max_check_unrolled = kMaxUnrolledCheckDegreeMS;
     }
+    fill_first_round<ALGO, V, T>(f);
 }
 
 template <int ALGO, typename T> void fill(int V, FloodFns *f)
diff --git a/myldpccppapi_amd/csrc/ldpc_hip.hip b/myldpccppapi_amd/csrc/ldpc_hip.hip
--- a/myldpccppapi_amd/csrc/ldpc_hip.hip
+++ b/myldpccppapi_amd/csrc/ldpc_hip.hip
@@ -215,6 +215,7 @@
     d->h_cols = g->cols;
     const ldpc::Tune tune = d->tune = ldpc::tune_from_config(*cfg);
     d->flood.syn_xcd = ldpc::tune_pick(tune.syn_xcd, true);
+    d->flood.lean = !ldpc::tune_forced_off(tune.lean);
     d->flood.check_wide = ldpc::tune_pick(tune.check_wide, false);
     d->flood.link_form = ldpc::tune_pick(tune.link_half, false) ? 2 : (ldpc::tune_pick(tune.link_narrow, true) ? 1 : 0);
     d->flood.link_deep = ldpc::tune_pick(tune.link_deep, false);
@@ -242,7 +243,7 @@
     d->flood.TA = d->T + d->flood.TO;
     const size_t TF = (size_t)d->flood.TA * d->F;
     LDPC_HIP_TRY(d->hard.alloc((size_t)d->flood.TA * d->N * d->V));
-    LDPC_HIP_TRY(d->failw.alloc((size_t)(cfg->max_iter + 2) * d->flood.TA * d->V));
+    LDPC_HIP_TRY(d->failw.alloc((size_t)(cfg->max_iter + 2) * d->flood.TA * d->V + ((size_t)(cfg->max_iter + 2) * d->flood.TA + 1) / 2));
     LDPC_HIP_TRY(d->done.alloc((size_t)d->flood.TA * d->V));
     LDPC_HIP_TRY(d->iters.alloc(TF));
     LDPC_HIP_TRY(d->active.alloc(1));
diff --git a/myldpccppapi_amd/csrc/tune.hpp b/myldpccppapi_amd/csrc/tune.hpp
--- a/myldpccppapi_amd/csrc/tune.hpp
+++ b/myldpccppapi_amd/csrc/tune.hpp
@@ -13,6 +13,7 @@
     int ldsp_grid = 0, ldsp_per_cu = 0, ldsp_waves = 0;
     int place = 0;
     int q_order = 0;
+    int lean = 0;
 };
 
 inline Tune tune_from_config(const ldpc_decoder_config &c)
@@ -34,6 +35,7 @@
     t.link_half = f(LDPC_TUNE_LINK_HALF);
     t.link_guided = f(LDPC_TUNE_LINK_GUIDED);
     t.tiles_first = f(LDPC_TUNE_TILES_FIRST);
+    t.lean = f(LDPC_TUNE_LEAN_ROUNDS);
     t.rows_per_wave = c.tune_rows_per_wave;
     t.cols_per_wave = c.tune_cols_per_wave;
     t.link_rows = c.tune_link_rows;
@@ -54,7 +56,8 @@
 {
     for (int field = 0; field <= LDPC_TUNE_TILES_FIRST; field += 2)
         if (((c.tune_flags >> field) & 3) == 3) return false;
-    if (c.tune_flags >> (LDPC_TUNE_TILES_FIRST + 2)) return false;
+    const int lean = (c.tune_flags >> LDPC_TUNE_LEAN_ROUNDS) & 3;
+    if (lean != 0 && lean != 2) return false;
     return c.tune_rows_per_wave >= 0 && c.tune_rows_per_wave <= 4096 && c.tune_cols_per_wave >= 0 &&
            c.tune_cols_per_wave <= 4096 && c.tune_link_rows >= -1 && c.tune_link_rows <= 4096 &&
            c.tune_compact >= -1 && c.tune_ldsp_grid >= 0 && c.tune_ldsp_shape >= 0 && c.tune_ldsp_shape < 65536 &&
```

After: 1126 Mbit/s. About the same (-0.1%).
